# mynameisfiber/baton

Measured on NVIDIA H100. Metric: federated local samples/sec (whole box), ResNet-18 FedAvg, synthetic non-IID 32x32 shards, higher is better.
Workload: dtype bf16

## Files before the change

baton_b200/csrc/bindings.cpp:

```cpp
#include <ATen/cuda/CUDAContext.h>
#include <c10/cuda/CUDAGuard.h>
#include <torch/extension.h>

#include <optional>
#include <vector>

#include "launch.h"

namespace {

inline cudaStream_t cur_stream() { return at::cuda::getCurrentCUDAStream().stream(); }
inline void check(int rc, const char* what) {
  TORCH_CHECK(rc == 0, "baton_b200::", what, " failed with code ", rc,
              rc > 0 ? std::string(" (") + cudaGetErrorString(static_cast<cudaError_t>(rc)) + ")" : std::string());
}
inline const void* cptr(const at::Tensor& t) { return t.data_ptr(); }
inline void* ptr(at::Tensor& t) { return t.data_ptr(); }
template <class T>
inline T* opt_ptr(const std::optional<at::Tensor>& t) {
  return (t.has_value() && t->defined()) ? reinterpret_cast<T*>(t->data_ptr()) : nullptr;
}
#define CHECK_CUDA(x) TORCH_CHECK((x).is_cuda(), #x " must be a CUDA tensor")

inline std::optional<B200SgdEpilogue> sgd_epilogue(const std::optional<at::Tensor>& theta,
                                                   const std::optional<at::Tensor>& theta_bf16,
                                                   const std::optional<at::Tensor>& mom,
                                                   const std::optional<at::Tensor>& hyper, bool nesterov) {
  if (!hyper.has_value() || !hyper->defined()) return std::nullopt;
  TORCH_CHECK(theta.has_value() && theta->scalar_type() == at::kFloat && hyper->scalar_type() == at::kFloat &&
                  (!theta_bf16.has_value() || theta_bf16->scalar_type() == at::kBFloat16) &&
                  (!mom.has_value() || mom->scalar_type() == at::kFloat),
              "sgd epilogue: fp32 theta / momentum / hyper, bf16 shadow");
  return B200SgdEpilogue{theta->data_ptr<float>(), opt_ptr<void>(theta_bf16), opt_ptr<float>(mom),
                         hyper->data_ptr<float>(), nesterov ? 1 : 0};
}

extern "C" {
#define B200_TRACE_TUS(X) X(gemm_wgmma) X(gemm_fp8) X(quant) X(attention) X(im2col_tma) X(gemm_simt) X(fedavg) \
  X(elementwise) X(conv) X(norm) X(loss)
#define B200_DECL(tu) int b200_trace_set_##tu(unsigned long long* p);
B200_TRACE_TUS(B200_DECL)
#undef B200_DECL
}
bool trace_set(const std::optional<at::Tensor>& buf) {
  unsigned long long* p = nullptr;
  if (buf.has_value() && buf->defined()) {
    CHECK_CUDA(*buf);
    TORCH_CHECK(buf->scalar_type() == at::kLong && buf->is_contiguous() && buf->numel() >= 4, "trace buffer: int64 [2+2n]");
    p = reinterpret_cast<unsigned long long*>(buf->data_ptr());
  }
  int rc = 0;
#define B200_SET(tu) rc |= b200_trace_set_##tu(p);
  B200_TRACE_TUS(B200_SET)
#undef B200_SET
  return rc == 0;
}

bool gemm(const at::Tensor& a, const at::Tensor& b, at::Tensor d, const std::optional<at::Tensor>& bias, int64_t M,
          int64_t N, int64_t K, int64_t lda, int64_t ldb, int64_t ldd, bool a_mn, bool b_mn, int64_t act,
          int64_t split_k, bool accumulate, double alpha, const std::optional<at::Tensor>& flags, int64_t flag_epoch,
          int64_t flag_elem_off, int64_t flag_tile_elems, int64_t flag_bias_off, int64_t force_bn, bool simt,
          const std::optional<at::Tensor>& col_stats, const std::optional<at::Tensor>& flag_epoch_word,
          const std::optional<at::Tensor>& sgd_theta, const std::optional<at::Tensor>& sgd_theta_bf16,
          const std::optional<at::Tensor>& sgd_mom, const std::optional<at::Tensor>& sgd_hyper, bool sgd_nesterov) {
  CHECK_CUDA(a); CHECK_CUDA(b); CHECK_CUDA(d);
  TORCH_CHECK(a.scalar_type() == at::kBFloat16 && b.scalar_type() == at::kBFloat16, "gemm operands must be bf16");
  TORCH_CHECK(d.scalar_type() == at::kBFloat16 || d.scalar_type() == at::kFloat, "gemm output must be bf16/fp32");
  const c10::cuda::CUDAGuard guard(a.device());
  const int out_fp32 = d.scalar_type() == at::kFloat;
  const float* bp = opt_ptr<const float>(bias);
  TORCH_CHECK(!col_stats.has_value() || (!simt && col_stats->scalar_type() == at::kFloat && col_stats->numel() >= 2 * N),
              "col_stats needs the tensor-core path and a [2N] fp32 buffer");
  if (simt) {
    TORCH_CHECK(!sgd_hyper.has_value(), "the SIMT GEMM has no optimizer epilogue");
    check(b200_gemm_simt(cptr(a), cptr(b), ptr(d), bp, M, N, K, lda, ldb, ldd, a_mn, b_mn, out_fp32, act, accumulate,
                         static_cast<float>(alpha), cur_stream()),
          "gemm_simt");
    return true;
  }
  const std::optional<B200SgdEpilogue> sgd = sgd_epilogue(sgd_theta, sgd_theta_bf16, sgd_mom, sgd_hyper, sgd_nesterov);
  const int rc = b200_gemm_bf16(cptr(a), cptr(b), ptr(d), bp, M, N, K, lda, ldb, ldd, a_mn, b_mn, out_fp32, act, split_k,
                                accumulate, static_cast<float>(alpha), opt_ptr<const uint32_t>(flags),
                                static_cast<uint32_t>(flag_epoch), flag_elem_off, static_cast<int>(flag_tile_elems),
                                flag_bias_off, static_cast<int>(force_bn), opt_ptr<float>(col_stats),
                                opt_ptr<const uint32_t>(flag_epoch_word), sgd ? &*sgd : nullptr, cur_stream());
  if (rc == B200_SGD_EPILOGUE_DECLINED) return false;
  check(rc, "gemm_bf16");
  return true;
}

void gemm_batched(const at::Tensor& a, const at::Tensor& b, at::Tensor d, int64_t M, int64_t N, int64_t K, int64_t lda,
                  int64_t ldb, int64_t ldd, bool a_mn, bool b_mn, int64_t act, double alpha, int64_t n_outer,
                  int64_t n_inner, int64_t a_outer, int64_t a_inner, int64_t b_outer, int64_t b_inner, int64_t d_outer,
                  int64_t d_inner, bool accumulate) {
  CHECK_CUDA(a); CHECK_CUDA(b); CHECK_CUDA(d);
  TORCH_CHECK(a.scalar_type() == at::kBFloat16 && b.scalar_type() == at::kBFloat16, "gemm operands must be bf16");
  const c10::cuda::CUDAGuard guard(a.device());
  check(b200_gemm_bf16_batched(cptr(a), cptr(b), ptr(d), M, N, K, lda, ldb, ldd, a_mn, b_mn,
                               d.scalar_type() == at::kFloat, act, static_cast<float>(alpha), n_outer, n_inner, a_outer,
                               a_inner, b_outer, b_inner, d_outer, d_inner, accumulate, cur_stream()),
        "gemm_bf16_batched");
}

bool attention_fwd(const at::Tensor& qkv, at::Tensor out, at::Tensor probs, int64_t B, int64_t S, int64_t H, int64_t dh,
                   double scale) {
  CHECK_CUDA(qkv); CHECK_CUDA(out); CHECK_CUDA(probs);
  TORCH_CHECK(qkv.scalar_type() == at::kBFloat16 && out.scalar_type() == at::kBFloat16 &&
              probs.scalar_type() == at::kBFloat16 && qkv.is_contiguous() && out.is_contiguous() && probs.is_contiguous());
  const c10::cuda::CUDAGuard guard(qkv.device());
  const int rc = b200_attention_fwd(cptr(qkv), ptr(out), ptr(probs), static_cast<int>(B), static_cast<int>(S),
                                    static_cast<int>(H), static_cast<int>(dh), static_cast<float>(scale), cur_stream());
  if (rc == -2) return false;
  check(rc, "attention_fwd");
  return true;
}

bool im2col_tma_probe(const at::Tensor& x, at::Tensor col, int64_t kh, int64_t kw, int64_t stride, int64_t pad,
                      int64_t ho, int64_t wo) {
  CHECK_CUDA(x); CHECK_CUDA(col);
  TORCH_CHECK(x.scalar_type() == at::kBFloat16 && col.scalar_type() == at::kBFloat16 && x.dim() == 4 && x.is_contiguous() &&
              col.is_contiguous());
  const c10::cuda::CUDAGuard guard(x.device());
  const int rc = b200_im2col_tma_probe(cptr(x), ptr(col), static_cast<int>(x.size(0)), static_cast<int>(x.size(1)),
                                       static_cast<int>(x.size(2)), static_cast<int>(x.size(3)), static_cast<int>(kh),
                                       static_cast<int>(kw), static_cast<int>(stride), static_cast<int>(pad),
                                       static_cast<int>(ho), static_cast<int>(wo), cur_stream());
  if (rc == -2) return false;
  check(rc, "im2col_tma_probe");
  return true;
}

bool attention_bwd(const at::Tensor& qkv, const at::Tensor& dout, const at::Tensor& probs, at::Tensor dqkv, int64_t B,
                   int64_t S, int64_t H, int64_t dh, double scale) {
  CHECK_CUDA(qkv); CHECK_CUDA(dout); CHECK_CUDA(probs); CHECK_CUDA(dqkv);
  TORCH_CHECK(qkv.scalar_type() == at::kBFloat16 && dout.scalar_type() == at::kBFloat16 &&
              probs.scalar_type() == at::kBFloat16 && dqkv.scalar_type() == at::kBFloat16 && qkv.is_contiguous() &&
              dout.is_contiguous() && probs.is_contiguous() && dqkv.is_contiguous());
  const c10::cuda::CUDAGuard guard(qkv.device());
  const int rc = b200_attention_bwd(cptr(qkv), cptr(dout), cptr(probs), ptr(dqkv), static_cast<int>(B), static_cast<int>(S),
                                    static_cast<int>(H), static_cast<int>(dh), static_cast<float>(scale), cur_stream());
  if (rc == -2) return false;
  check(rc, "attention_bwd");
  return true;
}

bool conv_igemm_fwd(const at::Tensor& x, const at::Tensor& w, at::Tensor y, int64_t kh, int64_t kw, int64_t stride,
                    int64_t pad, int64_t ho, int64_t wo, int64_t cluster_k, int64_t force_bn,
                    const std::optional<at::Tensor>& col_stats) {
  CHECK_CUDA(x); CHECK_CUDA(w); CHECK_CUDA(y);
  TORCH_CHECK(x.scalar_type() == at::kBFloat16 && w.scalar_type() == at::kBFloat16 && y.scalar_type() == at::kBFloat16 &&
              x.dim() == 4 && x.is_contiguous() && w.is_contiguous() && y.is_contiguous());
  const c10::cuda::CUDAGuard guard(x.device());
  const int rc = b200_conv_igemm_fwd(cptr(x), cptr(w), ptr(y), static_cast<int>(x.size(0)), static_cast<int>(x.size(1)),
                                     static_cast<int>(x.size(2)), static_cast<int>(x.size(3)), static_cast<int>(w.size(0)),
                                     static_cast<int>(kh), static_cast<int>(kw), static_cast<int>(stride),
                                     static_cast<int>(pad), static_cast<int>(ho), static_cast<int>(wo),
                                     static_cast<int>(cluster_k), static_cast<int>(force_bn), opt_ptr<float>(col_stats),
                                     cur_stream());
  if (rc == -2) return false;
  check(rc, "conv_igemm_fwd");
  return true;
}
bool conv_igemm_dgrad(const at::Tensor& dy, const at::Tensor& w, at::Tensor dx, int64_t kh, int64_t kw, int64_t pad,
                      int64_t cluster_k, int64_t force_bn) {
  CHECK_CUDA(dy); CHECK_CUDA(w); CHECK_CUDA(dx);
  TORCH_CHECK(dy.scalar_type() == at::kBFloat16 && w.scalar_type() == at::kBFloat16 && dx.scalar_type() == at::kBFloat16 &&
              dy.dim() == 4 && dx.dim() == 4 && dy.is_contiguous() && w.is_contiguous() && dx.is_contiguous());
  const c10::cuda::CUDAGuard guard(dy.device());
  const int rc = b200_conv_igemm_dgrad(cptr(dy), cptr(w), ptr(dx), static_cast<int>(dx.size(0)), static_cast<int>(dx.size(1)),
                                       static_cast<int>(dx.size(2)), static_cast<int>(dx.size(3)), static_cast<int>(dy.size(3)),
                                       static_cast<int>(kh), static_cast<int>(kw), static_cast<int>(pad),
                                       static_cast<int>(dy.size(1)), static_cast<int>(dy.size(2)),
                                       static_cast<int>(cluster_k), static_cast<int>(force_bn), cur_stream());
  if (rc == -2) return false;
  check(rc, "conv_igemm_dgrad");
  return true;
}
bool conv_igemm_wgrad(const at::Tensor& dy, const at::Tensor& x, at::Tensor dw, int64_t cout, int64_t kh, int64_t kw,
                      int64_t stride, int64_t pad, int64_t ho, int64_t wo, int64_t split_k, int64_t force_bn,
                      const std::optional<at::Tensor>& sgd_theta, const std::optional<at::Tensor>& sgd_theta_bf16,
                      const std::optional<at::Tensor>& sgd_mom, const std::optional<at::Tensor>& sgd_hyper,
                      bool sgd_nesterov) {
  CHECK_CUDA(dy); CHECK_CUDA(x); CHECK_CUDA(dw);
  TORCH_CHECK(x.scalar_type() == at::kBFloat16 && dy.scalar_type() == at::kBFloat16 && dw.scalar_type() == at::kFloat &&
              x.dim() == 4 && x.is_contiguous() && dy.is_contiguous());
  const c10::cuda::CUDAGuard guard(x.device());
  const std::optional<B200SgdEpilogue> sgd = sgd_epilogue(sgd_theta, sgd_theta_bf16, sgd_mom, sgd_hyper, sgd_nesterov);
  const int rc = b200_conv_igemm_wgrad(cptr(dy), cptr(x), dw.data_ptr<float>(), static_cast<int>(x.size(0)),
                                       static_cast<int>(x.size(1)), static_cast<int>(x.size(2)), static_cast<int>(x.size(3)),
                                       static_cast<int>(cout), static_cast<int>(kh), static_cast<int>(kw),
                                       static_cast<int>(stride), static_cast<int>(pad), static_cast<int>(ho),
                                       static_cast<int>(wo), static_cast<int>(split_k), static_cast<int>(force_bn),
                                       sgd ? &*sgd : nullptr, cur_stream());
  if (rc == -2 || rc == B200_SGD_EPILOGUE_DECLINED) return false;
  check(rc, "conv_igemm_wgrad");
  return true;
}

void gemm_fp8(const at::Tensor& a, const at::Tensor& b, at::Tensor d, const std::optional<at::Tensor>& bias,
              const std::optional<at::Tensor>& sfa, const std::optional<at::Tensor>& sfb, int64_t M, int64_t N, int64_t K,
              int64_t lda, int64_t ldb, int64_t ldd, int64_t act, int64_t split_k, bool accumulate, double alpha) {
  CHECK_CUDA(a); CHECK_CUDA(b); CHECK_CUDA(d);
  TORCH_CHECK(a.element_size() == 1 && b.element_size() == 1, "gemm_fp8 operands must be 1-byte (e4m3)");
  const c10::cuda::CUDAGuard guard(a.device());
  check(b200_gemm_fp8(cptr(a), cptr(b), ptr(d), opt_ptr<const float>(bias), opt_ptr<const void>(sfa),
                      opt_ptr<const void>(sfb), M, N, K, lda, ldb, ldd, d.scalar_type() == at::kFloat, act, split_k,
                      accumulate, static_cast<float>(alpha), cur_stream()),
        "gemm_fp8");
}
void quant_mx_rows(const at::Tensor& x, at::Tensor q, at::Tensor sf, int64_t R, int64_t C, int64_t ld_in, int64_t Cp) {
  CHECK_CUDA(x);
  const c10::cuda::CUDAGuard guard(x.device());
  check(b200_quant_mx_rows(x.data_ptr(), q.data_ptr(), sf.data_ptr(), R, C, ld_in, Cp, cur_stream()), "quant_mx_rows");
}
void quant_mx_cols(const at::Tensor& x, at::Tensor q, at::Tensor sf, int64_t R, int64_t C, int64_t ld_in, int64_t Rp) {
  CHECK_CUDA(x);
  const c10::cuda::CUDAGuard guard(x.device());
  check(b200_quant_mx_cols(x.data_ptr(), q.data_ptr(), sf.data_ptr(), R, C, ld_in, Rp, cur_stream()), "quant_mx_cols");
}
void dequant_mx(const at::Tensor& q, const at::Tensor& sf, at::Tensor out, int64_t R, int64_t C, int64_t Cp) {
  CHECK_CUDA(q);
  const c10::cuda::CUDAGuard guard(q.device());
  check(b200_dequant_mx(q.data_ptr(), sf.data_ptr(), out.data_ptr<float>(), R, C, Cp, cur_stream()), "dequant_mx");
}

void fused_sgd(at::Tensor w, at::Tensor g, const std::optional<at::Tensor>& mom, const std::optional<at::Tensor>& wb,
               const at::Tensor& hyper, bool zero_grad, bool nesterov, const std::optional<at::Tensor>& wire_slot,
               const std::optional<at::Tensor>& pack_global, const std::optional<at::Tensor>& pack_scale, int64_t n_pack,
               bool wire_fp32) {
  CHECK_CUDA(w);
  TORCH_CHECK(w.scalar_type() == at::kFloat && g.scalar_type() == at::kFloat && hyper.scalar_type() == at::kFloat);
  TORCH_CHECK(w.is_contiguous() && g.is_contiguous() && w.numel() == g.numel());
  const c10::cuda::CUDAGuard guard(w.device());
  check(b200_fused_sgd(w.data_ptr<float>(), g.data_ptr<float>(), opt_ptr<float>(mom), opt_ptr<void>(wb), w.numel(),
                       hyper.data_ptr<float>(), zero_grad, nesterov,
                       reinterpret_cast<const unsigned long long*>(opt_ptr<const int64_t>(wire_slot)),
                       opt_ptr<const float>(pack_global), opt_ptr<const float>(pack_scale), n_pack, wire_fp32, cur_stream()),
        "fused_sgd");
}

void fused_sgd_segments(at::Tensor w, at::Tensor g, const std::optional<at::Tensor>& mom,
                        const std::optional<at::Tensor>& wb, const at::Tensor& segments, const at::Tensor& hyper,
                        bool nesterov) {
  CHECK_CUDA(w); CHECK_CUDA(segments);
  TORCH_CHECK(w.scalar_type() == at::kFloat && g.scalar_type() == at::kFloat && hyper.scalar_type() == at::kFloat);
  TORCH_CHECK(segments.scalar_type() == at::kLong && segments.dim() == 2 && segments.size(1) == 3 &&
              segments.is_contiguous(), "segments: contiguous int64 [n, 3]");
  const c10::cuda::CUDAGuard guard(w.device());
  check(b200_fused_sgd_segments(w.data_ptr<float>(), g.data_ptr<float>(), opt_ptr<float>(mom), opt_ptr<void>(wb),
                                reinterpret_cast<const long long*>(segments.data_ptr<int64_t>()),
                                static_cast<int>(segments.size(0)), hyper.data_ptr<float>(), nesterov, cur_stream()),
        "fused_sgd_segments");
}

void fold_client(at::Tensor acc, at::Tensor theta, const at::Tensor& global_w, const std::optional<at::Tensor>& wb,
                 const std::optional<at::Tensor>& mom, double nk, int64_t mode, bool reset) {
  CHECK_CUDA(acc);
  TORCH_CHECK(acc.scalar_type() == at::kFloat && theta.scalar_type() == at::kFloat && global_w.scalar_type() == at::kFloat);
  TORCH_CHECK(acc.numel() == theta.numel() && theta.numel() == global_w.numel());
  const c10::cuda::CUDAGuard guard(acc.device());
  check(b200_fold_client(acc.data_ptr<float>(), theta.data_ptr<float>(), global_w.data_ptr<float>(), opt_ptr<void>(wb),
                         opt_ptr<float>(mom), mom.has_value() && mom->defined() ? mom->numel() : 0, theta.numel(),
                         static_cast<float>(nk), static_cast<int>(mode), reset, cur_stream()),
        "fold_client");
}

void weighted_sum(at::Tensor dst, const std::vector<at::Tensor>& srcs, const std::vector<double>& weights) {
  CHECK_CUDA(dst);
  TORCH_CHECK(srcs.size() == weights.size() && !srcs.empty() && srcs.size() <= B200_MAX_RANKS);
  TORCH_CHECK(dst.is_contiguous());
  const c10::cuda::CUDAGuard guard(dst.device());
  std::vector<const void*> ps;
  std::vector<float> ws;
  for (size_t i = 0; i < srcs.size(); ++i) {
    TORCH_CHECK(srcs[i].is_cuda() && srcs[i].is_contiguous() && srcs[i].scalar_type() == dst.scalar_type() &&
                srcs[i].numel() == dst.numel());
    ps.push_back(srcs[i].data_ptr());
    ws.push_back(static_cast<float>(weights[i]));
  }
  const int dt = dst.scalar_type() == at::kBFloat16 ? 1 : 0;
  TORCH_CHECK(dt == 1 || dst.scalar_type() == at::kFloat, "weighted_sum supports fp32/bf16");
  check(b200_weighted_sum(dst.data_ptr(), ps.data(), ws.data(), static_cast<int>(ps.size()), dst.numel(), dt,
                          cur_stream()),
        "weighted_sum");
}

void cast(const at::Tensor& src, at::Tensor dst) {
  CHECK_CUDA(src);
  TORCH_CHECK(src.is_contiguous() && dst.is_contiguous() && src.numel() == dst.numel());
  const c10::cuda::CUDAGuard guard(src.device());
  if (src.scalar_type() == at::kFloat && dst.scalar_type() == at::kBFloat16)
    check(b200_cast_f32_bf16(src.data_ptr<float>(), dst.data_ptr(), src.numel(), cur_stream()), "cast");
  else if (src.scalar_type() == at::kBFloat16 && dst.scalar_type() == at::kFloat)
    check(b200_cast_bf16_f32(src.data_ptr(), dst.data_ptr<float>(), src.numel(), cur_stream()), "cast");
  else
    TORCH_CHECK(false, "cast: unsupported dtype pair");
}

void gather_rows(const at::Tensor& src, const at::Tensor& idx, at::Tensor dst) {
  CHECK_CUDA(src);
  TORCH_CHECK(idx.scalar_type() == at::kLong && src.is_contiguous() && dst.is_contiguous());
  const c10::cuda::CUDAGuard guard(src.device());
  const int64_t n = idx.numel();
  if (src.scalar_type() == at::kLong && src.dim() == 1) {
    check(b200_gather_rows_i64(src.data_ptr<int64_t>() ? reinterpret_cast<const long long*>(src.data_ptr<int64_t>()) : nullptr,
                               reinterpret_cast<const long long*>(idx.data_ptr<int64_t>()),
                               reinterpret_cast<long long*>(dst.data_ptr<int64_t>()), n, cur_stream()),
          "gather_i64");
    return;
  }
  const int64_t row_bytes = src.numel() / src.size(0) * src.element_size();
  check(b200_gather_rows(src.data_ptr(), reinterpret_cast<const long long*>(idx.data_ptr<int64_t>()), dst.data_ptr(), n,
                         row_bytes, cur_stream()),
        "gather_rows");
}

void colsum(const at::Tensor& x, at::Tensor out, int64_t rows, int64_t cols, bool accumulate) {
  CHECK_CUDA(x);
  const c10::cuda::CUDAGuard guard(x.device());
  check(b200_colsum(x.data_ptr(), out.data_ptr<float>(), rows, cols, accumulate, cur_stream()), "colsum");
}
void add_bf16(const at::Tensor& a, const at::Tensor& b, at::Tensor o, bool relu) {
  CHECK_CUDA(a);
  const c10::cuda::CUDAGuard guard(a.device());
  check(b200_add_bf16(a.data_ptr(), b.data_ptr(), o.data_ptr(), a.numel(), relu, cur_stream()), "add_bf16");
}
void relu_bwd(const at::Tensor& y, const at::Tensor& dy, at::Tensor dx) {
  CHECK_CUDA(y);
// ... 157 lines not shown
                      opt_ptr<float>(rvar), save_mean.data_ptr<float>(), save_rstd.data_ptr<float>(),
                      opt_ptr<long long>(nbt), rows, C,
                      static_cast<float>(eps), static_cast<float>(momentum), relu, training, cur_stream()),
        "bn_apply");
}
void bn_bwd_reduce(const at::Tensor& x, const at::Tensor& y, const at::Tensor& dy, const at::Tensor& mean,
                   const at::Tensor& rstd, at::Tensor sums, int64_t rows, int64_t C, bool relu) {
  CHECK_CUDA(x);
  const c10::cuda::CUDAGuard guard(x.device());
  check(b200_bn_bwd_reduce(x.data_ptr(), y.data_ptr(), dy.data_ptr(), mean.data_ptr<float>(), rstd.data_ptr<float>(),
                           sums.data_ptr<float>(), rows, C, relu, cur_stream()),
        "bn_bwd_reduce");
}
void bn_bwd_apply(const at::Tensor& x, const at::Tensor& y, const at::Tensor& dy, at::Tensor dx,
                  const std::optional<at::Tensor>& dres, const std::optional<at::Tensor>& gamma, const at::Tensor& mean,
                  const at::Tensor& rstd, at::Tensor sums, const std::optional<at::Tensor>& dgamma,
                  const std::optional<at::Tensor>& dbeta, int64_t rows, int64_t C, bool relu) {
  CHECK_CUDA(x);
  const c10::cuda::CUDAGuard guard(x.device());
  check(b200_bn_bwd_apply(x.data_ptr(), y.data_ptr(), dy.data_ptr(), dx.data_ptr(), opt_ptr<void>(dres),
                          opt_ptr<const float>(gamma), mean.data_ptr<float>(), rstd.data_ptr<float>(),
                          sums.data_ptr<float>(), opt_ptr<float>(dgamma), opt_ptr<float>(dbeta), rows, C, relu,
                          cur_stream()),
        "bn_bwd_apply");
}
bool bn_relu_maxpool(const at::Tensor& z, at::Tensor p, at::Tensor arg, at::Tensor sums,
                     const std::optional<at::Tensor>& gamma, const std::optional<at::Tensor>& beta,
                     const std::optional<at::Tensor>& rmean, const std::optional<at::Tensor>& rvar, at::Tensor save_mean,
                     at::Tensor save_rstd, const std::optional<at::Tensor>& nbt, int64_t N, int64_t H, int64_t W, int64_t C,
                     int64_t k, int64_t stride, int64_t pad, int64_t Ho, int64_t Wo, double eps, double momentum) {
  CHECK_CUDA(z);
  const c10::cuda::CUDAGuard guard(z.device());
  const int rc = b200_bn_relu_maxpool(z.data_ptr(), p.data_ptr(), arg.data_ptr(), sums.data_ptr<float>(),
                                      opt_ptr<const float>(gamma), opt_ptr<const float>(beta), opt_ptr<float>(rmean),
                                      opt_ptr<float>(rvar), save_mean.data_ptr<float>(), save_rstd.data_ptr<float>(),
                                      opt_ptr<long long>(nbt), static_cast<int>(N), static_cast<int>(H), static_cast<int>(W),
                                      static_cast<int>(C), static_cast<int>(k), static_cast<int>(stride),
                                      static_cast<int>(pad), static_cast<int>(Ho), static_cast<int>(Wo),
                                      static_cast<float>(eps), static_cast<float>(momentum), cur_stream());
  if (rc == -2) return false;
  check(rc, "bn_relu_maxpool");
  return true;
}
bool bn_maxpool_bwd(const at::Tensor& z, const at::Tensor& p, const at::Tensor& arg, const at::Tensor& dy_a,
                    const std::optional<at::Tensor>& dy_b, at::Tensor dz, const std::optional<at::Tensor>& gamma,
                    const at::Tensor& mean, const at::Tensor& rstd, at::Tensor sums, const std::optional<at::Tensor>& dgamma,
                    const std::optional<at::Tensor>& dbeta, int64_t N, int64_t H, int64_t W, int64_t C, int64_t k,
                    int64_t stride, int64_t pad, int64_t Ho, int64_t Wo) {
  CHECK_CUDA(z);
  const c10::cuda::CUDAGuard guard(z.device());
  const int rc = b200_bn_maxpool_bwd(z.data_ptr(), p.data_ptr(), arg.data_ptr(), dy_a.data_ptr(), opt_ptr<const void>(dy_b),
                                     dz.data_ptr(), opt_ptr<const float>(gamma), mean.data_ptr<float>(),
                                     rstd.data_ptr<float>(), sums.data_ptr<float>(), opt_ptr<float>(dgamma),
                                     opt_ptr<float>(dbeta), static_cast<int>(N), static_cast<int>(H), static_cast<int>(W),
                                     static_cast<int>(C), static_cast<int>(k), static_cast<int>(stride),
                                     static_cast<int>(pad), static_cast<int>(Ho), static_cast<int>(Wo), cur_stream());
  if (rc == -2) return false;
  check(rc, "bn_maxpool_bwd");
  return true;
}
bool bn_bwd_cluster(const at::Tensor& x, const at::Tensor& y, const at::Tensor& dy_a, const std::optional<at::Tensor>& dy_b,
                    at::Tensor dx, const std::optional<at::Tensor>& dres, const std::optional<at::Tensor>& gamma,
                    const at::Tensor& mean, const at::Tensor& rstd, const std::optional<at::Tensor>& dgamma,
                    const std::optional<at::Tensor>& dbeta, int64_t rows, int64_t C, bool relu, int64_t max_cluster) {
  CHECK_CUDA(x);
  const c10::cuda::CUDAGuard guard(x.device());
  const int rc = b200_bn_bwd_cluster(x.data_ptr(), y.data_ptr(), dy_a.data_ptr(), opt_ptr<const void>(dy_b), dx.data_ptr(),
                                     opt_ptr<void>(dres), opt_ptr<const float>(gamma), mean.data_ptr<float>(),
                                     rstd.data_ptr<float>(), opt_ptr<float>(dgamma), opt_ptr<float>(dbeta), rows, C, relu,
                                     static_cast<int>(max_cluster), cur_stream());
  if (rc == -2) return false;
  check(rc, "bn_bwd_cluster");
  return true;
}
void layernorm_fwd(const at::Tensor& x, const std::optional<at::Tensor>& res, at::Tensor y, const at::Tensor& gamma,
                   const at::Tensor& beta, at::Tensor mean, at::Tensor rstd, int64_t rows, int64_t C, double eps) {
  CHECK_CUDA(x);
  const c10::cuda::CUDAGuard guard(x.device());
  check(b200_layernorm_fwd(x.data_ptr(), opt_ptr<const void>(res), y.data_ptr(), gamma.data_ptr<float>(),
                           beta.data_ptr<float>(), mean.data_ptr<float>(), rstd.data_ptr<float>(), rows, C,
                           static_cast<float>(eps), cur_stream()),
        "layernorm_fwd");
}
void layernorm_bwd(const at::Tensor& x, const at::Tensor& dy, at::Tensor dx, const at::Tensor& gamma,
                   const at::Tensor& mean, const at::Tensor& rstd, at::Tensor dgamma, at::Tensor dbeta, int64_t rows,
                   int64_t C) {
  CHECK_CUDA(x);
  const c10::cuda::CUDAGuard guard(x.device());
  check(b200_layernorm_bwd(x.data_ptr(), dy.data_ptr(), dx.data_ptr(), gamma.data_ptr<float>(), mean.data_ptr<float>(),
                           rstd.data_ptr<float>(), dgamma.data_ptr<float>(), dbeta.data_ptr<float>(), rows, C,
                           cur_stream()),
        "layernorm_bwd");
}
void softmax_fwd(const at::Tensor& x, at::Tensor y, int64_t rows, int64_t C, double scale) {
  CHECK_CUDA(x);
  const c10::cuda::CUDAGuard guard(x.device());
  check(b200_softmax_fwd(x.data_ptr(), y.data_ptr(), rows, C, static_cast<float>(scale), cur_stream()), "softmax_fwd");
}
void softmax_bwd(const at::Tensor& y, const at::Tensor& dy, at::Tensor dx, int64_t rows, int64_t C, double scale) {
  CHECK_CUDA(y);
  const c10::cuda::CUDAGuard guard(y.device());
  check(b200_softmax_bwd(y.data_ptr(), dy.data_ptr(), dx.data_ptr(), rows, C, static_cast<float>(scale), cur_stream()),
        "softmax_bwd");
}

void softmax_xent(const at::Tensor& logits, const at::Tensor& target, const std::optional<at::Tensor>& dlogits,
                  at::Tensor loss_acc, int64_t rows, int64_t C, int64_t ld, double grad_scale) {
  CHECK_CUDA(logits);
  TORCH_CHECK(target.scalar_type() == at::kLong && loss_acc.scalar_type() == at::kFloat && loss_acc.numel() >= 2);
  const c10::cuda::CUDAGuard guard(logits.device());
  const int in32 = logits.scalar_type() == at::kFloat;
  const int out32 = dlogits.has_value() && dlogits->defined() && dlogits->scalar_type() == at::kFloat;
  check(b200_softmax_xent(logits.data_ptr(), in32, reinterpret_cast<const long long*>(target.data_ptr<int64_t>()),
                          opt_ptr<void>(dlogits), out32, loss_acc.data_ptr<float>(), rows, C, ld,
                          static_cast<float>(grad_scale), cur_stream()),
        "softmax_xent");
}
bool linear_xent_head(const at::Tensor& x, const at::Tensor& w, const std::optional<at::Tensor>& bias, const at::Tensor& target,
                      const std::optional<at::Tensor>& dx, at::Tensor dw, const std::optional<at::Tensor>& db,
                      at::Tensor loss_acc, const std::optional<at::Tensor>& logits_out, double grad_scale) {
  CHECK_CUDA(x);
  TORCH_CHECK(x.scalar_type() == at::kBFloat16 && w.scalar_type() == at::kBFloat16 && x.dim() == 2 && w.dim() == 2 &&
              x.is_contiguous() && w.is_contiguous() && x.size(1) == w.size(1));
  TORCH_CHECK(target.scalar_type() == at::kLong && dw.scalar_type() == at::kFloat && dw.is_contiguous() &&
              dw.numel() == w.numel() && loss_acc.scalar_type() == at::kFloat && loss_acc.numel() >= 2);
  const c10::cuda::CUDAGuard guard(x.device());
  const int rc = b200_linear_xent_head(x.data_ptr(), w.data_ptr(), opt_ptr<const float>(bias),
                                       reinterpret_cast<const long long*>(target.data_ptr<int64_t>()), opt_ptr<void>(dx),
                                       dw.data_ptr<float>(), opt_ptr<float>(db), loss_acc.data_ptr<float>(),
                                       opt_ptr<float>(logits_out), static_cast<int>(x.size(0)), static_cast<int>(x.size(1)),
                                       static_cast<int>(w.size(0)), static_cast<float>(grad_scale), cur_stream());
  if (rc == -2) return false;
  check(rc, "linear_xent_head");
  return true;
}
void mse(const at::Tensor& pred, const at::Tensor& target, const std::optional<at::Tensor>& dpred, at::Tensor loss_acc,
         double grad_scale) {
  CHECK_CUDA(pred);
  TORCH_CHECK(target.scalar_type() == at::kFloat && target.numel() == pred.numel());
  const c10::cuda::CUDAGuard guard(pred.device());
  const int in32 = pred.scalar_type() == at::kFloat;
  const int out32 = dpred.has_value() && dpred->defined() && dpred->scalar_type() == at::kFloat;
  check(b200_mse(pred.data_ptr(), in32, target.data_ptr<float>(), opt_ptr<void>(dpred), out32,
                 loss_acc.data_ptr<float>(), pred.numel(), static_cast<float>(grad_scale), cur_stream()),
        "mse");
}

}

PYBIND11_MODULE(TORCH_EXTENSION_NAME, m) {
  m.doc() = "baton_b200 sm_90a kernels";
  m.attr("MAX_RANKS") = B200_MAX_RANKS;
  m.def("gemm", &gemm);
  m.def("trace_set", &trace_set);
  m.def("attention_fwd", &attention_fwd);
  m.def("attention_bwd", &attention_bwd);
  m.def("bn_bwd_cluster", &bn_bwd_cluster);
  m.def("im2col_tma_probe", &im2col_tma_probe);
  m.def("conv_igemm_fwd", &conv_igemm_fwd);
  m.def("conv_igemm_wgrad", &conv_igemm_wgrad);
  m.def("conv_igemm_dgrad", &conv_igemm_dgrad);
  m.def("gemm_batched", &gemm_batched);
  m.def("gemm_fp8", &gemm_fp8);
  m.def("quant_mx_rows", &quant_mx_rows);
  m.def("quant_mx_cols", &quant_mx_cols);
  m.def("dequant_mx", &dequant_mx);
  m.def("fused_sgd", &fused_sgd);
  m.def("fused_sgd_segments", &fused_sgd_segments);
  m.def("weighted_sum", &weighted_sum);
  m.def("fold_client", &fold_client);
  m.def("cast", &cast);
  m.def("gather_rows", &gather_rows);
  m.def("colsum", &colsum);
  m.def("add_bf16", &add_bf16);
  m.def("relu_bwd", &relu_bwd);
  m.def("gelu", &gelu);
  m.def("gelu_bwd", &gelu_bwd);
  m.def("pad_rows", &pad_rows);
  m.def("embedding_bwd", &embedding_bwd);
  m.def("fedavg_allreduce", &fedavg_allreduce);
  m.def("flag_barrier", &flag_barrier);
  m.def("im2col", &im2col);
  m.def("col2im", &col2im);
  m.def("maxpool", &maxpool);
  m.def("maxpool_bwd", &maxpool_bwd);
  m.def("avgpool", &avgpool);
  m.def("avgpool_bwd", &avgpool_bwd);
  m.def("bn_stats", &bn_stats);
  m.def("bn_apply", &bn_apply);
  m.def("bn_bwd_reduce", &bn_bwd_reduce);
  m.def("bn_bwd_apply", &bn_bwd_apply);
  m.def("bn_relu_maxpool", &bn_relu_maxpool);
  m.def("bn_maxpool_bwd", &bn_maxpool_bwd);
  m.def("layernorm_fwd", &layernorm_fwd);
  m.def("layernorm_bwd", &layernorm_bwd);
  m.def("softmax_fwd", &softmax_fwd);
  m.def("softmax_bwd", &softmax_bwd);
  m.def("softmax_xent", &softmax_xent);
  m.def("mse", &mse);
  m.def("linear_xent_head", &linear_xent_head);
}
```

baton_b200/csrc/gemm_wgmma.cu:

```cuda
#define B200_TU_TAG 1
#include "ptx.cuh"
#include "launch.h"
#include "pdl.cuh"
#include "sgd.cuh"

namespace b200 {

constexpr int BM = 128;
constexpr int BK = 64;
constexpr int WG_K = 16;
constexpr int GEMM_THREADS = 384;
constexpr int CONSUMER_WARPS = 8;
constexpr int CONSUMER_THREADS = 32 * CONSUMER_WARPS;
constexpr int MAX_STAGES = 8;

struct GemmParams {
  int M, N, K;
  void* D;
  long long ldd;
  const float* bias;
  int out_fp32;
  int act;
  float* col_stats;
  int a_mn, b_mn;
  int k_tiles_per_split;
  int atomic_out;
  int cluster_k;
  int stages;
  const uint32_t* tile_flags;
  uint32_t flag_epoch;
  long long flag_elem_off;
  int flag_tile_elems;
  long long flag_bias_off;
  long long ldb;
  float alpha;
  int batched, batch_inner;
  int batch_count;
  long long d_outer, d_inner;
  int conv_ho, conv_wo;
  int conv_stride, conv_pad;
  int conv_kw;
  int conv_cin;
  int conv_taps;
  int conv_ncol;
  const uint32_t* flag_epoch_ptr;
  const float* sgd_hyper = nullptr;
  float* sgd_theta = nullptr;
  __nv_bfloat16* sgd_wb = nullptr;
  float* sgd_mom = nullptr;
  int sgd_nesterov = 0;
};

__device__ __forceinline__ void wait_arrival_flags(const uint32_t* flags, long long e0, long long e1, int granule,
                                                   uint32_t need) {
  for (long long t = e0 / granule; t <= e1 / granule; ++t) {
    unsigned long long spins = 0;
    while (static_cast<int32_t>(ld_acquire_sys(flags + t) - need) < 0) {
      if (++spins > (1ull << 26)) break;
    }
  }
}

template <int BN>
struct SmemLayout {
  static constexpr int A_BYTES = BM * BK * 2;
  static constexpr int B_BYTES = BN * BK * 2;
  static constexpr int STAGE_BYTES = A_BYTES + B_BYTES;
  static constexpr int PART_PITCH = BN + 4;
  static constexpr int PART_BYTES = BM * PART_PITCH * 4;
};

__device__ __forceinline__ float apply_act(float v, int act) {
  if (act == 1) return fmaxf(v, 0.f);
  if (act == 2) {
    const float k0 = 0.7978845608028654f, k1 = 0.044715f;
    float t = tanhf(k0 * (v + k1 * v * v * v));
    return 0.5f * v * (1.f + t);
  }
  return v;
}

__device__ __forceinline__ uint32_t cluster_ctarank() {
  uint32_t r;
  asm volatile("mov.u32 %0, %%cluster_ctarank;" : "=r"(r));
  return r;
}
__device__ __forceinline__ void cluster_sync_all() {
  asm volatile("barrier.cluster.arrive.release.aligned;" ::: "memory");
  asm volatile("barrier.cluster.wait.acquire.aligned;" ::: "memory");
}
__device__ __forceinline__ float4 ld_dsmem_f4(uint32_t local_smem_addr, uint32_t cta_rank) {
  uint32_t remote;
  asm volatile("mapa.shared::cluster.u32 %0, %1, %2;" : "=r"(remote) : "r"(local_smem_addr), "r"(cta_rank));
  float4 v;
  asm volatile("ld.shared::cluster.v4.f32 {%0, %1, %2, %3}, [%4];"
               : "=f"(v.x), "=f"(v.y), "=f"(v.z), "=f"(v.w)
               : "r"(remote)
               : "memory");
  return v;
}

#define COLSUM_STEP(OFF, HALF)                                                  \
  {                                                                             \
    const bool upper = (lane & (OFF)) != 0;                                     \
    _Pragma("unroll") for (int i = 0; i < (HALF); ++i) {                        \
      const float keep = upper ? t[i + (HALF)] : t[i];                          \
      const float send = upper ? t[i] : t[i + (HALF)];                          \
      t[i] = keep + __shfl_xor_sync(0xffffffffu, send, (OFF));                  \
    }                                                                           \
  }
__device__ __forceinline__ float warp_colsum32(float (&t)[32]) {
  const uint32_t lane = lane_id();
  COLSUM_STEP(16, 16) COLSUM_STEP(8, 8) COLSUM_STEP(4, 4) COLSUM_STEP(2, 2) COLSUM_STEP(1, 1)
  return t[0];
}
#undef COLSUM_STEP
__device__ __forceinline__ void accumulate_col_stats(const GemmParams& p, int col0, const float (&v)[32]) {
  float s[32], q[32];
#pragma unroll
  for (int j = 0; j < 32; ++j) {
    const float r = __bfloat162float(__float2bfloat16_rn(v[j]));
    s[j] = r;
    q[j] = r * r;
  }
  const float cs = warp_colsum32(s), cq = warp_colsum32(q);
  const int col = col0 + static_cast<int>(lane_id());
  if (col < p.N) {
    atomicAdd(p.col_stats + col, cs);
    atomicAdd(p.col_stats + p.N + col, cq);
  }
}

__device__ __forceinline__ void stage_col_stats(float* sbuf, int BNv, int c, const float (&v)[32]) {
  float s[32], q[32];
#pragma unroll
  for (int j = 0; j < 32; ++j) {
    const float r = __bfloat162float(__float2bfloat16_rn(v[j]));
    s[j] = r;
    q[j] = r * r;
  }
  const float cs = warp_colsum32(s), cq = warp_colsum32(q);
  const int lane = static_cast<int>(lane_id());
  sbuf[c + lane] = cs;
  sbuf[BNv + c + lane] = cq;
}

template <int NV, int ACT, bool BIAS>
__device__ __forceinline__ void transform_chunk_t(const GemmParams& p, int col0, float (&v)[NV]) {
  float b[NV];
  if (BIAS) {
    if (col0 + NV <= p.N && ((reinterpret_cast<uintptr_t>(p.bias + col0) & 15) == 0)) {
#pragma unroll
      for (int j = 0; j < NV; j += 4) {
        const float4 t = __ldg(reinterpret_cast<const float4*>(p.bias + col0 + j));
        b[j] = t.x; b[j + 1] = t.y; b[j + 2] = t.z; b[j + 3] = t.w;
      }
    } else {
#pragma unroll
      for (int j = 0; j < NV; ++j) b[j] = (col0 + j) < p.N ? __ldg(p.bias + col0 + j) : 0.f;
    }
  }
  const float alpha = p.alpha;
#pragma unroll
  for (int j = 0; j < NV; ++j) {
    float x = v[j] * alpha;
    if (BIAS) x += b[j];
    if (ACT == 1) x = fmaxf(x, 0.f);
    if (ACT == 2) {
      const float k0 = 0.7978845608028654f, k1 = 0.044715f;
      x = 0.5f * x * (1.f + tanhf(k0 * (x + k1 * x * x * x)));
    }
    v[j] = x;
  }
}
template <int NV>
__device__ __forceinline__ void transform_chunk(const GemmParams& p, int col0, float (&v)[NV]) {
  if (p.bias == nullptr) {
    if (p.act == 0) transform_chunk_t<NV, 0, false>(p, col0, v);
    else if (p.act == 1) transform_chunk_t<NV, 1, false>(p, col0, v);
    else transform_chunk_t<NV, 2, false>(p, col0, v);
  } else {
    if (p.act == 0) transform_chunk_t<NV, 0, true>(p, col0, v);
    else if (p.act == 1) transform_chunk_t<NV, 1, true>(p, col0, v);
    else transform_chunk_t<NV, 2, true>(p, col0, v);
  }
}

template <int NV>
__device__ __forceinline__ void store_row_chunk(const GemmParams& p, int row, int col0, float (&v)[NV], bool vec_ok,
                                                size_t d_off = 0) {
  transform_chunk<NV>(p, col0, v);
  const bool full = (col0 + NV <= p.N);
  if (p.out_fp32) {
    float* d = reinterpret_cast<float*>(p.D) + d_off + static_cast<size_t>(row) * p.ldd + col0;
    if (p.atomic_out) {
      if (full && vec_ok) {
#pragma unroll
        for (int j = 0; j < NV; j += 4)
          asm volatile("red.global.add.v4.f32 [%0], {%1, %2, %3, %4};" ::"l"(d + j), "f"(v[j]), "f"(v[j + 1]),
                       "f"(v[j + 2]), "f"(v[j + 3])
                       : "memory");
      } else {
        _Pragma("unroll") for (int j = 0; j < NV; ++j) if (col0 + j < p.N) atomicAdd(d + j, v[j]);
      }
    } else if (full && vec_ok) {
#pragma unroll
      for (int j = 0; j < NV; j += 4) *reinterpret_cast<float4*>(d + j) = make_float4(v[j], v[j + 1], v[j + 2], v[j + 3]);
    } else {
      _Pragma("unroll") for (int j = 0; j < NV; ++j) if (col0 + j < p.N) d[j] = v[j];
    }
  } else {
    __nv_bfloat16* d = reinterpret_cast<__nv_bfloat16*>(p.D) + d_off + static_cast<size_t>(row) * p.ldd + col0;
    if (full && vec_ok) {
#pragma unroll
      for (int j = 0; j < NV; j += 8) {
        uint4 o;
        o.x = pack_bf16x2(v[j], v[j + 1]);
        o.y = pack_bf16x2(v[j + 2], v[j + 3]);
        o.z = pack_bf16x2(v[j + 4], v[j + 5]);
        o.w = pack_bf16x2(v[j + 6], v[j + 7]);
        *reinterpret_cast<uint4*>(d + j) = o;
      }
    } else {
      _Pragma("unroll") for (int j = 0; j < NV; ++j) if (col0 + j < p.N) d[j] = __float2bfloat16_rn(v[j]);
    }
  }
}

__device__ __forceinline__ void sgd_epilogue_chunk(const GemmParams& p, size_t e, int col0, const float (&v)[32],
                                                   bool vec) {
  const SgdHyper h = load_sgd_hyper(p.sgd_hyper);
  float* w = p.sgd_theta + e;
  float* m = p.sgd_mom != nullptr ? p.sgd_mom + e : nullptr;
  __nv_bfloat16* wb = p.sgd_wb != nullptr ? p.sgd_wb + e : nullptr;
  const bool nest = p.sgd_nesterov != 0;
  if (vec && col0 + 32 <= p.N) {
#pragma unroll
    for (int j = 0; j < 32; j += 4) {
      float4 mv = m != nullptr ? *reinterpret_cast<const float4*>(m + j) : make_float4(0.f, 0.f, 0.f, 0.f);
      const float4 gv = make_float4(__fadd_rn(0.f, v[j]), __fadd_rn(0.f, v[j + 1]), __fadd_rn(0.f, v[j + 2]),
                                    __fadd_rn(0.f, v[j + 3]));
      const float4 wv = sgd_update4(h, *reinterpret_cast<const float4*>(w + j), gv, mv, m != nullptr, nest);
      *reinterpret_cast<float4*>(w + j) = wv;
      if (m != nullptr) *reinterpret_cast<float4*>(m + j) = mv;
      if (wb != nullptr) *reinterpret_cast<uint2*>(wb + j) = make_uint2(pack_bf16x2(wv.x, wv.y), pack_bf16x2(wv.z, wv.w));
    }
  } else {
#pragma unroll
    for (int j = 0; j < 32; ++j) {
      if (col0 + j < p.N) {
        float mv = m != nullptr ? m[j] : 0.f;
        const float wv = sgd_update(h, w[j], __fadd_rn(0.f, v[j]), mv, m != nullptr, nest);
// ... 279 lines not shown
#pragma unroll
      for (int j = 0; j < 32; ++j) v[j] = __uint_as_float(r[j]);
      if (p.col_stats != nullptr) accumulate_col_stats(p, col0, v);
      if (row >= p.M) continue;
      store_row_chunk<32>(p, row, col0, v, vec_ok, d_off);
    }
    return;
  }
  const int W = 128 / elt;
  uint8_t* srow = stage + lane * EPI_PITCH;
#pragma unroll 1
  for (int c0 = half * W; c0 < BN; c0 += 2 * W) {
    if (n0 + c0 >= p.N) break;
    for (int cc = 0; cc < W; cc += 32) {
      uint32_t r[32];
      acc_ld_row32(arow + c0 + cc, r);
      const int col0 = n0 + c0 + cc;
      float v[32];
#pragma unroll
      for (int j = 0; j < 32; ++j) v[j] = __uint_as_float(r[j]);
      transform_chunk<32>(p, col0, v);
      if (p.col_stats != nullptr) accumulate_col_stats(p, col0, v);
      if (p.out_fp32) {
#pragma unroll
        for (int j = 0; j < 32; j += 4)
          *reinterpret_cast<float4*>(srow + (cc + j) * 4) = make_float4(v[j], v[j + 1], v[j + 2], v[j + 3]);
      } else {
#pragma unroll
        for (int j = 0; j < 32; j += 8)
          *reinterpret_cast<uint4*>(srow + (cc + j) * 2) =
              make_uint4(pack_bf16x2(v[j], v[j + 1]), pack_bf16x2(v[j + 2], v[j + 3]), pack_bf16x2(v[j + 4], v[j + 5]),
                         pack_bf16x2(v[j + 6], v[j + 7]));
      }
    }
    __syncwarp();
    const int per16 = 16 / elt;
#pragma unroll
    for (int it = 0; it < 8; ++it) {
      const int idx = it * 32 + lane;
      const int r = idx >> 3, ch = idx & 7;
      const int grow = m0 + q * 32 + r;
      const int col = n0 + c0 + ch * per16;
      if (grow < p.M && col < p.N) {
        const uint4 val = *reinterpret_cast<const uint4*>(stage + r * EPI_PITCH + ch * 16);
        *reinterpret_cast<uint4*>(reinterpret_cast<uint8_t*>(p.D) +
                                  (d_off + static_cast<size_t>(grow) * p.ldd + col) * elt) = val;
      }
    }
    __syncwarp();
  }
}

template <int BN, int STAGES>
__global__ void __launch_bounds__(GEMM_THREADS, 1)
gemm_bf16_persistent_kernel(const __grid_constant__ CUtensorMap tmA, const __grid_constant__ CUtensorMap tmB,
                            const GemmParams p) {
  using L = SmemLayout<BN>;
  extern __shared__ __align__(1024) uint8_t smem_raw[];
  uint8_t* smem = reinterpret_cast<uint8_t*>((reinterpret_cast<uintptr_t>(smem_raw) + 1023) & ~uintptr_t(1023));
  float* acc_tile = reinterpret_cast<float*>(smem + STAGES * L::STAGE_BYTES);
  uint64_t* full_bar = reinterpret_cast<uint64_t*>(smem + STAGES * L::STAGE_BYTES + L::PART_BYTES);
  uint64_t* empty_bar = full_bar + STAGES;
  uint8_t* epi_stage = reinterpret_cast<uint8_t*>(empty_bar + STAGES);

  griddep_launch_dependents();
  const int warp = threadIdx.x >> 5;
  const int tiles_m = (p.M + BM - 1) / BM;
  const int tiles_n = (p.N + BN - 1) / BN;
  const int tiles_per_z = tiles_m * tiles_n;
  const int num_tiles = tiles_per_z * (p.batched ? p.batch_count : 1);
  const int num_kt = (p.K + BK - 1) / BK;

  if (warp == 0 && elect_one()) {
    tma_prefetch_desc(&tmA);
    tma_prefetch_desc(&tmB);
    for (int s = 0; s < STAGES; ++s) {
      mbar_init(&full_bar[s], 1);
      mbar_init(&empty_bar[s], CONSUMER_WARPS);
    }
    fence_barrier_init();
  }
  __syncthreads();
  griddep_wait();

  if (warp == 0) {
    if (elect_one()) {
      int s = 0;
      uint32_t ph = 0;
      for (int tile = blockIdx.x; tile < num_tiles; tile += gridDim.x) {
        const int z = tile / tiles_per_z, rem = tile - z * tiles_per_z;
        const int m0 = (rem % tiles_m) * BM, n0 = (rem / tiles_m) * BN;
        const int zo = p.batched ? z / p.batch_inner : 0, zi = p.batched ? z % p.batch_inner : 0;
        for (int kt = 0; kt < num_kt; ++kt) {
          mbar_wait(&empty_bar[s], ph ^ 1);
          uint8_t* sa = smem + s * L::STAGE_BYTES;
          uint8_t* sb = sa + L::A_BYTES;
          const int k0 = kt * BK;
          mbar_expect_tx(&full_bar[s], L::STAGE_BYTES);
          if (p.batched) {
            if (!p.a_mn) {
              tma_load_4d(sa, &tmA, &full_bar[s], k0, m0, zi, zo);
            } else {
#pragma unroll
              for (int j = 0; j < BM / 64; ++j) tma_load_4d(sa + j * 8192, &tmA, &full_bar[s], m0 + j * 64, k0, zi, zo);
            }
            if (!p.b_mn) {
              tma_load_4d(sb, &tmB, &full_bar[s], k0, n0, zi, zo);
            } else {
#pragma unroll
              for (int j = 0; j < BN / 64; ++j) tma_load_4d(sb + j * 8192, &tmB, &full_bar[s], n0 + j * 64, k0, zi, zo);
            }
          } else {
            if (!p.a_mn) {
              tma_load_2d(sa, &tmA, &full_bar[s], k0, m0);
            } else {
#pragma unroll
              for (int j = 0; j < BM / 64; ++j) tma_load_2d(sa + j * 8192, &tmA, &full_bar[s], m0 + j * 64, k0);
            }
            if (!p.b_mn) {
              tma_load_2d(sb, &tmB, &full_bar[s], k0, n0);
            } else {
#pragma unroll
              for (int j = 0; j < BN / 64; ++j) tma_load_2d(sb + j * 8192, &tmB, &full_bar[s], n0 + j * 64, k0);
            }
          }
          if (++s == STAGES) { s = 0; ph ^= 1; }
        }
      }
    }
  } else if (warp >= 4) {
    const int ew = warp - 4;
    const size_t elt = p.out_fp32 ? 4 : 2;
    const bool vec_ok = ((reinterpret_cast<uintptr_t>(p.D) & 15) == 0) && ((p.ldd * elt) % 16 == 0);
    int s = 0;
    uint32_t ph = 0;
    float acc[BN / 2];
    for (int tile = blockIdx.x; tile < num_tiles; tile += gridDim.x) {
      const int z = tile / tiles_per_z, rem = tile - z * tiles_per_z;
      const int m0 = (rem % tiles_m) * BM, n0 = (rem / tiles_m) * BN;
      size_t d_off = 0;
      if (p.batched)
        d_off = static_cast<size_t>(z / p.batch_inner) * p.d_outer + static_cast<size_t>(z % p.batch_inner) * p.d_inner;
      consume_ktiles<BN>(acc, smem, STAGES, full_bar, empty_bar, s, ph, num_kt, p.a_mn, p.b_mn, ew >> 2);
      named_bar_sync(1, CONSUMER_THREADS);
      wg_store_acc<BN>(acc, acc_tile, L::PART_PITCH, 64 * (ew >> 2));
      named_bar_sync(1, CONSUMER_THREADS);
      epilogue_tile<BN>(p, acc_tile, ew & 3, ew >> 2, m0, n0, epi_stage + ew * EPI_WARP_BYTES,
                        vec_ok && ((d_off * elt) & 15) == 0, d_off);
    }
  }
}


template <int BN, bool CLUSTER, int CONV = 0>
__global__ void __launch_bounds__(GEMM_THREADS, 1)
gemm_bf16_splitk_kernel(const __grid_constant__ CUtensorMap tmA, const __grid_constant__ CUtensorMap tmB,
                        const GemmParams p) {
  using L = SmemLayout<BN>;
  extern __shared__ __align__(1024) uint8_t smem_raw[];
  uint8_t* smem = reinterpret_cast<uint8_t*>((reinterpret_cast<uintptr_t>(smem_raw) + 1023) & ~uintptr_t(1023));
  const int STAGES = p.stages;
  const int ring_bytes = STAGES * L::STAGE_BYTES;
  const int data_bytes = L::PART_BYTES > ring_bytes ? L::PART_BYTES : ring_bytes;
  uint64_t* full_bar = reinterpret_cast<uint64_t*>(smem + data_bytes);
  uint64_t* empty_bar = full_bar + MAX_STAGES;
  float* cstat = reinterpret_cast<float*>(empty_bar + MAX_STAGES);

  griddep_launch_dependents();
  const int warp = threadIdx.x >> 5;
  const int m0 = blockIdx.y * BM;
  const int n0 = blockIdx.x * BN;
  const int k_tiles_total = (p.K + BK - 1) / BK;
  const int kt_begin = blockIdx.z * p.k_tiles_per_split;
  int kt_end = kt_begin + p.k_tiles_per_split;
  if (kt_end > k_tiles_total) kt_end = k_tiles_total;
  const int num_kt = kt_end - kt_begin;

  if (warp == 0 && elect_one()) {
    tma_prefetch_desc(&tmA);
    tma_prefetch_desc(&tmB);
    for (int s = 0; s < STAGES; ++s) {
      mbar_init(&full_bar[s], 1);
      mbar_init(&empty_bar[s], CONSUMER_WARPS);
    }
    fence_barrier_init();
  }
  __syncthreads();
  griddep_wait();

  if (warp == 0) {
    if (elect_one()) {
      if (p.tile_flags != nullptr) {
        const int rows_here = (p.N - n0) < BN ? (p.N - n0) : BN;
        const uint32_t need = p.flag_epoch_ptr != nullptr ? *reinterpret_cast<const volatile uint32_t*>(p.flag_epoch_ptr)
                                                          : p.flag_epoch;
        wait_arrival_flags(p.tile_flags, p.flag_elem_off + static_cast<long long>(n0) * p.ldb,
                           p.flag_elem_off + static_cast<long long>(n0 + rows_here) * p.ldb - 1, p.flag_tile_elems, need);
        if (p.flag_bias_off >= 0)
          wait_arrival_flags(p.tile_flags, p.flag_bias_off + n0, p.flag_bias_off + n0 + rows_here - 1,
                             p.flag_tile_elems, need);
        fence_proxy_async_all();
      }
      int s = 0;
      uint32_t ph = 0;
      for (int i = 0; i < num_kt; ++i) {
        mbar_wait(&empty_bar[s], ph ^ 1);
        uint8_t* sa = smem + s * L::STAGE_BYTES;
        uint8_t* sb = sa + L::A_BYTES;
        const int k0 = (kt_begin + i) * BK;
        mbar_expect_tx(&full_bar[s], L::STAGE_BYTES);
        if constexpr (CONV == 1 || CONV == 3) {
          const int kt = kt_begin + i;
          const int cblocks = p.conv_cin >> 6;
          const int tap = kt / cblocks, cb = kt - tap * cblocks;
          const int fr = tap / p.conv_kw, fs = tap - fr * p.conv_kw;
          const int q0 = m0 % p.conv_wo, t0 = m0 / p.conv_wo;
          tma_load_im2col_4d(sa, &tmA, &full_bar[s], cb * 64, q0 * p.conv_stride - p.conv_pad,
                             (t0 % p.conv_ho) * p.conv_stride - p.conv_pad, t0 / p.conv_ho, fs, fr);
        } else if (!p.a_mn) {
          tma_load_2d(sa, &tmA, &full_bar[s], k0, m0);
        } else {
#pragma unroll
          for (int j = 0; j < BM / 64; ++j)
            tma_load_2d(sa + j * 8192, &tmA, &full_bar[s], m0 + j * 64, k0);
        }
        if constexpr (CONV == 3) {
          const int kt = kt_begin + i;
          const int cblocks = p.conv_cin >> 6;
          const int tap = kt / cblocks, cb = kt - tap * cblocks;
          const int wcol = (p.conv_taps - 1 - tap) * p.conv_ncol + n0;
#pragma unroll
          for (int j = 0; j < BN / 64; ++j) tma_load_2d(sb + j * 8192, &tmB, &full_bar[s], wcol + j * 64, cb * 64);
        } else if (!p.b_mn) {
          tma_load_2d(sb, &tmB, &full_bar[s], k0, n0);
        } else {
#pragma unroll
          for (int j = 0; j < BN / 64; ++j) tma_load_2d(sb + j * 8192, &tmB, &full_bar[s], n0 + j * 64, k0);
        }
        if (++s == STAGES) { s = 0; ph ^= 1; }
      }
    }
  } else if (warp >= 4) {
    const int ew = warp - 4;
    float acc[BN / 2];
    int s = 0;
    uint32_t ph = 0;
    consume_ktiles<BN>(acc, smem, STAGES, full_bar, empty_bar, s, ph, num_kt, p.a_mn, p.b_mn, ew >> 2);
    named_bar_sync(1, CONSUMER_THREADS);
    float* part = reinterpret_cast<float*>(smem);
    wg_store_acc<BN>(acc, part, L::PART_PITCH, 64 * (ew >> 2));
    if constexpr (!CLUSTER) {
      named_bar_sync(1, CONSUMER_THREADS);
      const int q = ew & 3;
      constexpr int NCHUNK = BN / 32;
      const int c_begin = (ew < 4 ? 0 : (NCHUNK + 1) / 2) * 32, c_end = (ew < 4 ? (NCHUNK + 1) / 2 : NCHUNK) * 32;
      const int lrow = q * 32 + static_cast<int>(lane_id());
      const int row = m0 + lrow;
      const size_t elt = p.out_fp32 ? 4 : 2;
      const bool vec_ok = ((reinterpret_cast<uintptr_t>(p.D) & 15) == 0) && ((p.ldd * elt) % 16 == 0);
#pragma unroll 1
      for (int c = c_begin; c < c_end; c += 32) {
        const int col0 = n0 + c;
        if (row >= p.M || col0 >= p.N) continue;
        uint32_t r[32];
        acc_ld_row32(part + lrow * L::PART_PITCH + c, r);
        float v[32];
#pragma unroll
        for (int j = 0; j < 32; ++j) v[j] = __uint_as_float(r[j]);
        store_row_chunk<32>(p, row, col0, v, vec_ok);
      }
    }
  }

  if constexpr (CLUSTER) {
    const int S = p.cluster_k;
    cluster_sync_all();
    if (warp >= 4 && warp < 8) {
      const uint32_t me = cluster_ctarank();
      const int rows_per = BM / S;
      constexpr int CG = BN / 8;
      const int t = threadIdx.x - 128;
      const size_t elt = p.out_fp32 ? 4 : 2;
      const bool vec_ok = ((reinterpret_cast<uintptr_t>(p.D) & 15) == 0) && ((p.ldd * elt) % 16 == 0);
      const bool want_stats = p.col_stats != nullptr;
      float cs[8] = {0.f, 0.f, 0.f, 0.f, 0.f, 0.f, 0.f, 0.f}, cq[8] = {0.f, 0.f, 0.f, 0.f, 0.f, 0.f, 0.f, 0.f};
      for (int item = t; item < rows_per * CG; item += 128) {
        const int lrow = static_cast<int>(me) * rows_per + item / CG;
        const int c = (item % CG) * 8;
        const uint32_t laddr = smem_u32(smem) + static_cast<uint32_t>((lrow * L::PART_PITCH + c) * 4);
        float v[8] = {0.f, 0.f, 0.f, 0.f, 0.f, 0.f, 0.f, 0.f};
        for (int r = 0; r < S; ++r) {
          const float4 a = ld_dsmem_f4(laddr, r), b = ld_dsmem_f4(laddr + 16, r);
          v[0] += a.x; v[1] += a.y; v[2] += a.z; v[3] += a.w;
          v[4] += b.x; v[5] += b.y; v[6] += b.z; v[7] += b.w;
        }
        const int row = m0 + lrow, col0 = n0 + c;
        if (want_stats) {
#pragma unroll
          for (int j = 0; j < 8; ++j) {
            const float rnd = __bfloat162float(__float2bfloat16_rn(v[j]));
            cs[j] += rnd;
            cq[j] = fmaf(rnd, rnd, cq[j]);
          }
        }
        if (row < p.M && col0 < p.N) store_row_chunk<8>(p, row, col0, v, vec_ok);
      }
      if (want_stats) {
#pragma unroll
        for (int j = 0; j < 8; ++j) {
#pragma unroll
          for (int o = CG; o < 32; o <<= 1) {
            cs[j] += __shfl_xor_sync(0xffffffffu, cs[j], o);
            cq[j] += __shfl_xor_sync(0xffffffffu, cq[j], o);
          }
        }
        const int wq = t >> 5, ln = t & 31;
        if (ln < CG) {
#pragma unroll
          for (int j = 0; j < 8; ++j) {
            cstat[wq * 2 * BN + ln * 8 + j] = cs[j];
            cstat[wq * 2 * BN + BN + ln * 8 + j] = cq[j];
          }
        }
        named_bar_sync(2, 128);
        for (int i = t; i < 2 * BN; i += 128) {
          const int col = i < BN ? i : i - BN;
          if (n0 + col < p.N) {
            const float v = cstat[i] + cstat[2 * BN + i] + cstat[4 * BN + i] + cstat[6 * BN + i];
            atomicAdd(p.col_stats + (i < BN ? 0 : p.N) + n0 + col, v);
          }
        }
      }
    }
    cluster_sync_all();
  }
}


typedef CUresult (*EncodeTiledFn)(CUtensorMap*, CUtensorMapDataType, cuuint32_t, void*, const cuuint64_t*,
                                  const cuuint64_t*, const cuuint32_t*, const cuuint32_t*, CUtensorMapInterleave,
                                  CUtensorMapSwizzle, CUtensorMapL2promotion, CUtensorMapFloatOOBfill);

static EncodeTiledFn get_encode_fn() {
  static thread_local bool ctx_bound = false;
  if (!ctx_bound) {
    cudaFree(nullptr);
    ctx_bound = true;
  }
  static EncodeTiledFn fn = nullptr;
  if (fn == nullptr) {
    void* ptr = nullptr;
    cudaDriverEntryPointQueryResult qres;
    cudaError_t e = cudaGetDriverEntryPoint("cuTensorMapEncodeTiled", &ptr, cudaEnableDefault, &qres);
    if (e != cudaSuccess || qres != cudaDriverEntryPointSuccess || ptr == nullptr) return nullptr;
    fn = reinterpret_cast<EncodeTiledFn>(ptr);
  }
  return fn;
}

static int make_map(CUtensorMap* map, const void* base, long long rows, long long cols, long long ld, int box_cols,
                    int box_rows) {
  EncodeTiledFn fn = get_encode_fn();
  if (fn == nullptr) return -1;
  cuuint64_t gdim[2] = {static_cast<cuuint64_t>(cols), static_cast<cuuint64_t>(rows)};
  cuuint64_t gstr[1] = {static_cast<cuuint64_t>(ld) * 2};
  cuuint32_t box[2] = {static_cast<cuuint32_t>(box_cols), static_cast<cuuint32_t>(box_rows)};
  cuuint32_t estr[2] = {1, 1};
  CUresult r = fn(map, CU_TENSOR_MAP_DATA_TYPE_BFLOAT16, 2, const_cast<void*>(base), gdim, gstr, box, estr,
                  CU_TENSOR_MAP_INTERLEAVE_NONE, CU_TENSOR_MAP_SWIZZLE_128B, CU_TENSOR_MAP_L2_PROMOTION_L2_256B,
                  CU_TENSOR_MAP_FLOAT_OOB_FILL_NONE);
  return r == CUDA_SUCCESS ? 0 : static_cast<int>(r);
}

static int make_map4(CUtensorMap* map, const void* base, long long rows, long long cols, long long ld, long long inner,
                     long long s_inner, long long outer, long long s_outer, int box_cols, int box_rows) {
  EncodeTiledFn fn = get_encode_fn();
  if (fn == nullptr) return -1;
  cuuint64_t gdim[4] = {static_cast<cuuint64_t>(cols), static_cast<cuuint64_t>(rows), static_cast<cuuint64_t>(inner),
                        static_cast<cuuint64_t>(outer)};
  cuuint64_t gstr[3] = {static_cast<cuuint64_t>(ld) * 2, static_cast<cuuint64_t>(s_inner) * 2,
                        static_cast<cuuint64_t>(s_outer) * 2};
  cuuint32_t box[4] = {static_cast<cuuint32_t>(box_cols), static_cast<cuuint32_t>(box_rows), 1, 1};
  cuuint32_t estr[4] = {1, 1, 1, 1};
  CUresult r = fn(map, CU_TENSOR_MAP_DATA_TYPE_BFLOAT16, 4, const_cast<void*>(base), gdim, gstr, box, estr,
                  CU_TENSOR_MAP_INTERLEAVE_NONE, CU_TENSOR_MAP_SWIZZLE_128B, CU_TENSOR_MAP_L2_PROMOTION_L2_256B,
                  CU_TENSOR_MAP_FLOAT_OOB_FILL_NONE);
  return r == CUDA_SUCCESS ? 0 : static_cast<int>(r);
}

static int clamp_bn(int bn) { return bn > 128 ? 128 : bn; }

static void set_sgd_epilogue(GemmParams& p, const B200SgdEpilogue& s) {
  p.sgd_hyper = s.hyper; p.sgd_theta = s.theta; p.sgd_wb = reinterpret_cast<__nv_bfloat16*>(s.theta_bf16);
  p.sgd_mom = s.mom; p.sgd_nesterov = s.nesterov;
}

template <int BN, int STAGES, int CONV = 0, bool SGD = false>
static int launch_fixed(const CUtensorMap& ta, const CUtensorMap& tb, const GemmParams& p, dim3 grid,
                      cudaStream_t stream) {
  constexpr int smem = STAGES * SmemLayout<BN>::STAGE_BYTES + 2 * STAGES * 8 + 8 * BN * 4 + 1024;
  static bool configured = false;
  if (!configured) {
    cudaError_t e = cudaFuncSetAttribute(gemm_bf16_fixed_kernel<BN, STAGES, CONV, SGD>,
                                         cudaFuncAttributeMaxDynamicSharedMemorySize, smem);
    if (e != cudaSuccess) return static_cast<int>(e);
    configured = true;
  }
  cudaError_t le = launch_pdl(gemm_bf16_fixed_kernel<BN, STAGES, CONV, SGD>, grid, GEMM_THREADS, smem, stream, ta, tb, p);
  if (le != cudaSuccess) return static_cast<int>(le);
  return static_cast<int>(cudaGetLastError());
}

template <int BN, int STAGES>
static int launch_persistent(const CUtensorMap& ta, const CUtensorMap& tb, const GemmParams& p, int num_tiles,
                             cudaStream_t stream) {
  constexpr int smem = STAGES * SmemLayout<BN>::STAGE_BYTES + SmemLayout<BN>::PART_BYTES + 2 * STAGES * 8 +
                       CONSUMER_WARPS * EPI_WARP_BYTES + 1024;
  static_assert(smem <= 227 * 1024, "persistent GEMM exceeds the 227 KB of shared memory a block may use");
  static bool configured = false;
  if (!configured) {
    cudaError_t e = cudaFuncSetAttribute(gemm_bf16_persistent_kernel<BN, STAGES>,
                                         cudaFuncAttributeMaxDynamicSharedMemorySize, smem);
    if (e != cudaSuccess) return static_cast<int>(e);
    configured = true;
  }
  const int grid = num_tiles < device_sm_count() ? num_tiles : device_sm_count();
  cudaError_t le = launch_pdl(gemm_bf16_persistent_kernel<BN, STAGES>, dim3(grid), GEMM_THREADS, smem, stream, ta, tb, p);
  if (le != cudaSuccess) return static_cast<int>(le);
  return static_cast<int>(cudaGetLastError());
}

template <int BN, int CONV = 0>
static int launch_cfg(const CUtensorMap& ta, const CUtensorMap& tb, const GemmParams& p, dim3 grid,
                      cudaStream_t stream) {
  using L = SmemLayout<BN>;
  constexpr int max_stages = BN == 128 ? 6 : 8;
  constexpr int max_smem = max_stages * L::STAGE_BYTES + 2 * MAX_STAGES * 8 + 8 * BN * 4 + 1024;
  static bool configured = false;
  if (!configured) {
    const int cap = max_smem > L::PART_BYTES + 4096 ? max_smem : L::PART_BYTES + 4096;
    cudaError_t e = cudaFuncSetAttribute(gemm_bf16_splitk_kernel<BN, false, CONV>,
                                         cudaFuncAttributeMaxDynamicSharedMemorySize, cap);
    if (e == cudaSuccess)
      e = cudaFuncSetAttribute(gemm_bf16_splitk_kernel<BN, true, CONV>, cudaFuncAttributeMaxDynamicSharedMemorySize, cap);
    if (e != cudaSuccess) return static_cast<int>(e);
    configured = true;
  }
  int ring = p.stages * L::STAGE_BYTES;
  if (L::PART_BYTES > ring) ring = L::PART_BYTES;
  int smem = ring + 2 * MAX_STAGES * 8 + 8 * BN * 4 + 1024;
  constexpr int max_ctas = 2;
  const int ctas_here = p.atomic_out ? 1 : max_ctas;
  const int floor_smem = (227 * 1024) / (ctas_here + 1) + 1024;
  if (smem < floor_smem && floor_smem <= max_smem) smem = floor_smem;
  cudaLaunchConfig_t cfg = {};
  cfg.gridDim = grid;
  cfg.blockDim = dim3(GEMM_THREADS);
  cfg.dynamicSmemBytes = smem;
  cfg.stream = stream;
  cudaLaunchAttribute attr[2];
  int na = 0;
  if (pdl_enabled()) {
    attr[na].id = cudaLaunchAttributeProgrammaticStreamSerialization;
    attr[na].val.programmaticStreamSerializationAllowed = 1;
    ++na;
  }
  if (p.cluster_k > 1) {
    attr[na].id = cudaLaunchAttributeClusterDimension;
    attr[na].val.clusterDim.x = 1;
    attr[na].val.clusterDim.y = 1;
    attr[na].val.clusterDim.z = p.cluster_k;
    ++na;
  }
  cfg.attrs = attr;
  cfg.numAttrs = na;
  cudaError_t le = p.cluster_k > 1 ? cudaLaunchKernelEx(&cfg, gemm_bf16_splitk_kernel<BN, true, CONV>, ta, tb, p)
                                   : cudaLaunchKernelEx(&cfg, gemm_bf16_splitk_kernel<BN, false, CONV>, ta, tb, p);
  if (le != cudaSuccess) return static_cast<int>(le);
  return static_cast<int>(cudaGetLastError());
}

}

extern "C" int b200_encode_map2_bf16(void* map, const void* base, long long rows, long long cols, long long ld,
                                     int box_cols, int box_rows) {
  return b200::make_map(reinterpret_cast<CUtensorMap*>(map), base, rows, cols, ld, box_cols, box_rows);
}
extern "C" int b200_encode_map4_bf16(void* map, const void* base, long long rows, long long cols, long long ld,
                                     long long inner, long long s_inner, long long outer, long long s_outer,
                                     int box_cols, int box_rows) {
  return b200::make_map4(reinterpret_cast<CUtensorMap*>(map), base, rows, cols, ld, inner, s_inner, outer, s_outer,
                         box_cols, box_rows);
}

extern "C" int b200_gemm_bf16(const void* a, const void* b, void* d, const float* bias, int M, int N, int K,
                              long long lda, long long ldb, long long ldd, int a_mn, int b_mn, int out_fp32, int act,
                              int split_k, int accumulate, float alpha, const uint32_t* tile_flags,
                              uint32_t flag_epoch, long long flag_elem_off, int flag_tile_elems,
                              long long flag_bias_off, int force_bn, float* col_stats, const uint32_t* flag_epoch_ptr,
                              const B200SgdEpilogue* sgd, cudaStream_t stream) {
  using namespace b200;
  if (M <= 0 || N <= 0 || K <= 0) return 0;
  if (sgd != nullptr && (!accumulate || !out_fp32 || !a_mn || !b_mn || bias != nullptr || act != 0 || alpha != 1.0f ||
                         col_stats != nullptr || tile_flags != nullptr))
    return B200_SGD_EPILOGUE_DECLINED;
  if (col_stats != nullptr && (split_k > 1 || bias != nullptr || act != 0 || alpha != 1.0f || accumulate)) return -3;
  if ((lda % 8) || (ldb % 8) || (reinterpret_cast<uintptr_t>(a) & 15) || (reinterpret_cast<uintptr_t>(b) & 15))
    return -2;
  const int bn = clamp_bn(force_bn > 0 ? force_bn : (N > 64 ? 128 : 64));
  if (tile_flags != nullptr && (b_mn || flag_tile_elems <= 0)) return -4;
  CUtensorMap ta, tb;
  int rc;
  if (!a_mn)
    rc = make_map(&ta, a, M, K, lda, BK, BM);
  else
    rc = make_map(&ta, a, K, M, lda, 64, BK);
  if (rc) return rc;
  if (!b_mn)
    rc = make_map(&tb, b, N, K, ldb, BK, bn);
  else
    rc = make_map(&tb, b, K, N, ldb, 64, BK);
  if (rc) return rc;

  const int k_tiles = (K + BK - 1) / BK;
  int cluster_k = 1;
  if (split_k < 0) {
    cluster_k = -split_k;
    if (cluster_k != 2 && cluster_k != 4 && cluster_k != 8) return -5;
    while (cluster_k > 1 && (cluster_k - 1) * ((k_tiles + cluster_k - 1) / cluster_k) >= k_tiles) cluster_k >>= 1;
    split_k = cluster_k;
  }
  if (split_k < 1) split_k = 1;
  if (split_k > k_tiles) split_k = k_tiles;
  int per = (k_tiles + split_k - 1) / split_k;
  if (cluster_k == 1) split_k = (k_tiles + per - 1) / per;
  GemmParams p;
  p.M = M; p.N = N; p.K = K; p.D = d; p.ldd = ldd; p.bias = bias; p.out_fp32 = out_fp32; p.act = act;
  p.a_mn = a_mn; p.b_mn = b_mn; p.k_tiles_per_split = per;
  p.cluster_k = cluster_k;
  p.atomic_out = (accumulate || (split_k > 1 && cluster_k == 1)) ? 1 : 0;
  p.col_stats = col_stats;
  p.tile_flags = tile_flags; p.flag_epoch = flag_epoch; p.alpha = alpha;
  p.flag_elem_off = flag_elem_off; p.flag_tile_elems = flag_tile_elems; p.ldb = ldb;
  p.flag_bias_off = (tile_flags != nullptr && bias != nullptr) ? flag_bias_off : -1;
  p.flag_epoch_ptr = tile_flags != nullptr ? flag_epoch_ptr : nullptr;
  p.batched = 0; p.batch_inner = 1; p.batch_count = 1; p.d_outer = 0; p.d_inner = 0;
  if (p.atomic_out && (!out_fp32 || bias != nullptr || act != 0)) return -3;
  const int max_stages = bn == 128 ? 6 : 8;
  p.stages = per < max_stages ? (per < 2 ? 2 : per) : max_stages;
  dim3 grid((N + bn - 1) / bn, (M + BM - 1) / BM, split_k);
  const int num_tiles = static_cast<int>(grid.x * grid.y);
  const bool persistent = split_k == 1 && tile_flags == nullptr && num_tiles >= device_sm_count() && bn == 128;
  if (sgd != nullptr) {
    if (split_k != 1 || cluster_k != 1 || persistent) return B200_SGD_EPILOGUE_DECLINED;
    set_sgd_epilogue(p, *sgd);
  }
  if (cluster_k > 1) {
    if (bn == 128) return launch_cfg<128>(ta, tb, p, grid, stream);
    return launch_cfg<64>(ta, tb, p, grid, stream);
  }
  if (persistent) return launch_persistent<128, 3>(ta, tb, p, num_tiles, stream);
  const bool shallow = per <= 4 && !p.batched;
  if (sgd != nullptr) {
    if (bn == 128)
      return shallow ? launch_fixed<128, 3, 0, true>(ta, tb, p, grid, stream) : launch_fixed<128, 6, 0, true>(ta, tb, p, grid, stream);
    return shallow ? launch_fixed<64, 4, 0, true>(ta, tb, p, grid, stream) : launch_fixed<64, 8, 0, true>(ta, tb, p, grid, stream);
  }
  if (bn == 128) return shallow ? launch_fixed<128, 3>(ta, tb, p, grid, stream) : launch_fixed<128, 6>(ta, tb, p, grid, stream);
  return shallow ? launch_fixed<64, 4>(ta, tb, p, grid, stream) : launch_fixed<64, 8>(ta, tb, p, grid, stream);
}

extern "C" int b200_gemm_bf16_batched(const void* a, const void* b, void* d, int M, int N, int K, long long lda,
                                      long long ldb, long long ldd, int a_mn, int b_mn, int out_fp32, int act,
                                      float alpha, int n_outer, int n_inner, long long a_outer, long long a_inner,
                                      long long b_outer, long long b_inner, long long d_outer, long long d_inner,
                                      int accumulate, cudaStream_t stream) {
  using namespace b200;
  if (M <= 0 || N <= 0 || K <= 0 || n_outer <= 0 || n_inner <= 0) return 0;
  if ((lda % 8) || (ldb % 8) || (a_outer % 8) || (a_inner % 8) || (b_outer % 8) || (b_inner % 8) ||
      (reinterpret_cast<uintptr_t>(a) & 15) || (reinterpret_cast<uintptr_t>(b) & 15))
    return -2;
  auto fix = [](long long s) { return s > 0 ? s : 8; };
  const int bn = N > 64 ? 128 : 64;
  CUtensorMap ta, tb;
  int rc;
  if (!a_mn)
    rc = make_map4(&ta, a, M, K, lda, n_inner, fix(a_inner), n_outer, fix(a_outer), BK, BM);
  else
    rc = make_map4(&ta, a, K, M, lda, n_inner, fix(a_inner), n_outer, fix(a_outer), 64, BK);
  if (rc) return rc;
  if (!b_mn)
    rc = make_map4(&tb, b, N, K, ldb, n_inner, fix(b_inner), n_outer, fix(b_outer), BK, bn);
  else
    rc = make_map4(&tb, b, K, N, ldb, n_inner, fix(b_inner), n_outer, fix(b_outer), 64, BK);
  if (rc) return rc;
  GemmParams p;
  p.M = M; p.N = N; p.K = K; p.D = d; p.ldd = ldd; p.bias = nullptr; p.out_fp32 = out_fp32; p.act = act;
  p.a_mn = a_mn; p.b_mn = b_mn; p.k_tiles_per_split = (K + BK - 1) / BK; p.cluster_k = 1;
  p.atomic_out = accumulate ? 1 : 0;
  p.col_stats = nullptr;
  p.tile_flags = nullptr; p.flag_epoch = 0; p.alpha = alpha; p.flag_elem_off = 0; p.flag_tile_elems = 0;
  p.ldb = ldb; p.flag_bias_off = -1; p.flag_epoch_ptr = nullptr; p.stages = 4;
  p.batched = 1; p.batch_inner = n_inner; p.d_outer = d_outer; p.d_inner = d_inner;
  if (p.atomic_out && !out_fp32) return -3;
  dim3 grid((N + bn - 1) / bn, (M + BM - 1) / BM, n_outer * n_inner);
  p.batch_count = n_outer * n_inner;
  const long long total_tiles = static_cast<long long>(grid.x) * grid.y * grid.z;
  if (total_tiles >= 2 * device_sm_count() && total_tiles < (1ll << 30)) {
    const int nt = static_cast<int>(total_tiles);
    if (bn == 128) return launch_persistent<128, 3>(ta, tb, p, nt, stream);
    return launch_persistent<64, 5>(ta, tb, p, nt, stream);
  }
  if (bn == 128) return launch_fixed<128, 6>(ta, tb, p, grid, stream);
  return launch_fixed<64, 8>(ta, tb, p, grid, stream);
}

extern "C" int b200_encode_map_im2col_bf16(void* map, const void* x, int N, int H, int W, int C, int KH, int KW,
                                            int stride, int pad, int channels, int pixels);

extern "C" int b200_conv_igemm_fwd(const void* x, const void* w, void* y, int N, int H, int W, int Cin, int Cout, int KH,
                                   int KW, int stride, int pad, int Ho, int Wo, int cluster_k, int force_bn,
                                   float* col_stats, cudaStream_t stream) {
  using namespace b200;
  const long long M = static_cast<long long>(N) * Ho * Wo;
  const int K = KH * KW * Cin;
  if (M <= 0 || Cout <= 0) return 0;
  if (Cin % 64 != 0 || Cout % 8 != 0 || M > (1ll << 30) || (reinterpret_cast<uintptr_t>(x) & 15) ||
      (reinterpret_cast<uintptr_t>(w) & 15) || (reinterpret_cast<uintptr_t>(y) & 15))
    return -2;
  const int bn = clamp_bn(force_bn > 0 ? force_bn : (Cout > 64 ? 128 : 64));
  CUtensorMap ta, tb;
  int rc = b200_encode_map_im2col_bf16(&ta, x, N, H, W, Cin, KH, KW, stride, pad, 64, BM);
  if (rc) return rc;
  rc = make_map(&tb, w, Cout, K, K, BK, bn);
  if (rc) return rc;
  const int k_tiles = K / BK;
  if (cluster_k != 1 && cluster_k != 2 && cluster_k != 4 && cluster_k != 8) return -5;
  while (cluster_k > 1 && (cluster_k - 1) * ((k_tiles + cluster_k - 1) / cluster_k) >= k_tiles) cluster_k >>= 1;
  const int per = (k_tiles + cluster_k - 1) / cluster_k;
  GemmParams p;
  p.M = static_cast<int>(M); p.N = Cout; p.K = K; p.D = y; p.ldd = Cout; p.bias = nullptr; p.out_fp32 = 0; p.act = 0;
  p.a_mn = 0; p.b_mn = 0; p.k_tiles_per_split = per; p.cluster_k = cluster_k; p.atomic_out = 0;
  p.col_stats = col_stats;
  p.tile_flags = nullptr; p.flag_epoch = 0; p.alpha = 1.0f; p.flag_elem_off = 0; p.flag_tile_elems = 0; p.ldb = K;
  p.flag_bias_off = -1; p.flag_epoch_ptr = nullptr;
  p.batched = 0; p.batch_inner = 1; p.batch_count = 1; p.d_outer = 0; p.d_inner = 0;
  const int max_stages = bn == 128 ? 6 : 8;
  p.stages = per < max_stages ? (per < 2 ? 2 : per) : max_stages;
  p.conv_ho = Ho; p.conv_wo = Wo; p.conv_stride = stride; p.conv_pad = pad; p.conv_kw = KW; p.conv_cin = Cin;
  p.conv_taps = KH * KW; p.conv_ncol = Cin;
  dim3 grid((Cout + bn - 1) / bn, static_cast<unsigned>((M + BM - 1) / BM), cluster_k);
  if (cluster_k > 1) {
    if (bn == 128) return launch_cfg<128, 1>(ta, tb, p, grid, stream);
    return launch_cfg<64, 1>(ta, tb, p, grid, stream);
  }
  const bool shallow = per <= 4;
  if (bn == 128) return shallow ? launch_fixed<128, 3, 1>(ta, tb, p, grid, stream) : launch_fixed<128, 6, 1>(ta, tb, p, grid, stream);
  return shallow ? launch_fixed<64, 4, 1>(ta, tb, p, grid, stream) : launch_fixed<64, 8, 1>(ta, tb, p, grid, stream);
}

extern "C" int b200_conv_igemm_dgrad(const void* dy, const void* w, void* dx, int N, int H, int W, int Cin, int Cout,
                                     int KH, int KW, int pad, int Ho, int Wo, int cluster_k, int force_bn,
                                     cudaStream_t stream) {
  using namespace b200;
  const long long M = static_cast<long long>(N) * H * W;
  const int K = KH * KW * Cout;
  if (M <= 0 || Cin <= 0) return 0;
  const int padp = KH - 1 - pad, padq = KW - 1 - pad;
  if (Cout % 64 != 0 || Cin % 64 != 0 || M > (1ll << 30) || padp < 0 || padq < 0 || padp != padq ||
      Ho + 2 * padp - (KH - 1) != H || Wo + 2 * padq - (KW - 1) != W || (reinterpret_cast<uintptr_t>(dy) & 15) ||
      (reinterpret_cast<uintptr_t>(w) & 15) || (reinterpret_cast<uintptr_t>(dx) & 15))
    return -2;
  const int bn = clamp_bn(force_bn > 0 ? force_bn : (Cin > 64 ? 128 : 64));
  CUtensorMap ta, tb;
  int rc = b200_encode_map_im2col_bf16(&ta, dy, N, Ho, Wo, Cout, KH, KW, 1, padp, 64, BM);
  if (rc) return rc;
  rc = make_map(&tb, w, Cout, static_cast<long long>(KH) * KW * Cin, static_cast<long long>(KH) * KW * Cin, 64, BK);
  if (rc) return rc;
  const int k_tiles = K / BK;
  if (cluster_k != 1 && cluster_k != 2 && cluster_k != 4 && cluster_k != 8) return -5;
  while (cluster_k > 1 && (cluster_k - 1) * ((k_tiles + cluster_k - 1) / cluster_k) >= k_tiles) cluster_k >>= 1;
  const int per = (k_tiles + cluster_k - 1) / cluster_k;
  GemmParams p;
  p.M = static_cast<int>(M); p.N = Cin; p.K = K; p.D = dx; p.ldd = Cin; p.bias = nullptr; p.out_fp32 = 0; p.act = 0;
  p.a_mn = 0; p.b_mn = 1; p.k_tiles_per_split = per; p.cluster_k = cluster_k; p.atomic_out = 0;
  p.col_stats = nullptr;
  p.tile_flags = nullptr; p.flag_epoch = 0; p.alpha = 1.0f; p.flag_elem_off = 0; p.flag_tile_elems = 0;
  p.ldb = static_cast<long long>(KH) * KW * Cin;
  p.flag_bias_off = -1; p.flag_epoch_ptr = nullptr;
  p.batched = 0; p.batch_inner = 1; p.batch_count = 1; p.d_outer = 0; p.d_inner = 0;
  const int max_stages = bn == 128 ? 6 : 8;
  p.stages = per < max_stages ? (per < 2 ? 2 : per) : max_stages;
  p.conv_ho = H; p.conv_wo = W; p.conv_stride = 1; p.conv_pad = padp; p.conv_kw = KW; p.conv_cin = Cout;
  p.conv_taps = KH * KW; p.conv_ncol = Cin;
  dim3 grid((Cin + bn - 1) / bn, static_cast<unsigned>((M + BM - 1) / BM), cluster_k);
  if (cluster_k > 1) {
    if (bn == 128) return launch_cfg<128, 3>(ta, tb, p, grid, stream);
    return launch_cfg<64, 3>(ta, tb, p, grid, stream);
  }
  if (bn == 128) return launch_fixed<128, 6, 3>(ta, tb, p, grid, stream);
  return launch_fixed<64, 8, 3>(ta, tb, p, grid, stream);
}

extern "C" int b200_conv_igemm_wgrad(const void* dy, const void* x, float* dw, int N, int H, int W, int Cin, int Cout,
                                     int KH, int KW, int stride, int pad, int Ho, int Wo, int split_k, int force_bn,
                                     const B200SgdEpilogue* sgd, cudaStream_t stream) {
  using namespace b200;
  const long long Mp = static_cast<long long>(N) * Ho * Wo;
  const int Kc = KH * KW * Cin;
  if (Mp <= 0 || Cout <= 0) return 0;
  if (Cin % 64 != 0 || Cout % 8 != 0 || Mp > (1ll << 30) || (reinterpret_cast<uintptr_t>(x) & 15) ||
      (reinterpret_cast<uintptr_t>(dy) & 15) || (reinterpret_cast<uintptr_t>(dw) & 15))
    return -2;
  const int bn = clamp_bn(force_bn > 0 ? force_bn : (Kc > 64 ? 128 : 64));
  CUtensorMap ta, tb;
  int rc = make_map(&ta, dy, Mp, Cout, Cout, 64, BK);
  if (rc) return rc;
  rc = b200_encode_map_im2col_bf16(&tb, x, N, H, W, Cin, KH, KW, stride, pad, 64, 64);
  if (rc) return rc;
  const int k_tiles = static_cast<int>((Mp + BK - 1) / BK);
  if (split_k < 1) split_k = 1;
  if (split_k > k_tiles) split_k = k_tiles;
  const int per = (k_tiles + split_k - 1) / split_k;
  split_k = (k_tiles + per - 1) / per;
  if (sgd != nullptr && split_k != 1) return B200_SGD_EPILOGUE_DECLINED;
  GemmParams p;
  if (sgd != nullptr) set_sgd_epilogue(p, *sgd);
  p.M = Cout; p.N = Kc; p.K = static_cast<int>(Mp); p.D = dw; p.ldd = Kc; p.bias = nullptr; p.out_fp32 = 1; p.act = 0;
  p.a_mn = 1; p.b_mn = 1; p.k_tiles_per_split = per; p.cluster_k = 1; p.atomic_out = 1;
  p.col_stats = nullptr;
  p.tile_flags = nullptr; p.flag_epoch = 0; p.alpha = 1.0f; p.flag_elem_off = 0; p.flag_tile_elems = 0; p.ldb = Kc;
  p.flag_bias_off = -1; p.flag_epoch_ptr = nullptr;
  p.batched = 0; p.batch_inner = 1; p.batch_count = 1; p.d_outer = 0; p.d_inner = 0;
  p.stages = 4;
  p.conv_ho = Ho; p.conv_wo = Wo; p.conv_stride = stride; p.conv_pad = pad; p.conv_kw = KW; p.conv_cin = Cin;
  p.conv_taps = KH * KW; p.conv_ncol = Cin;
  dim3 grid((Kc + bn - 1) / bn, (Cout + BM - 1) / BM, split_k);
  if (sgd != nullptr) {
    if (bn == 128) return launch_fixed<128, 6, 2, true>(ta, tb, p, grid, stream);
    return launch_fixed<64, 8, 2, true>(ta, tb, p, grid, stream);
  }
  if (bn == 128) return launch_fixed<128, 6, 2>(ta, tb, p, grid, stream);
  return launch_fixed<64, 8, 2>(ta, tb, p, grid, stream);
}

B200_TRACE_REGISTER(gemm_wgmma)
```

baton_b200/csrc/launch.h:

```cpp
#pragma once
#include <cuda_runtime.h>
#include <stdint.h>

#define B200_MAX_RANKS 16

extern "C" {

struct B200SgdEpilogue {
  float* theta;
  void* theta_bf16;
  float* mom;
  const float* hyper;
  int nesterov;
};
#define B200_SGD_EPILOGUE_DECLINED (-6)

int b200_gemm_bf16(const void* a, const void* b, void* d, const float* bias, int M, int N, int K, long long lda,
                   long long ldb, long long ldd, int a_mn, int b_mn, int out_fp32, int act, int split_k, int accumulate,
                   float alpha, const uint32_t* tile_flags, uint32_t flag_epoch, long long flag_elem_off, int flag_tile_elems,
                   long long flag_bias_off, int force_bn, float* col_stats, const uint32_t* flag_epoch_ptr,
                   const B200SgdEpilogue* sgd, cudaStream_t stream);
int b200_gemm_bf16_batched(const void* a, const void* b, void* d, int M, int N, int K, long long lda, long long ldb,
                           long long ldd, int a_mn, int b_mn, int out_fp32, int act, float alpha, int n_outer,
                           int n_inner, long long a_outer, long long a_inner, long long b_outer, long long b_inner,
                           long long d_outer, long long d_inner, int accumulate, cudaStream_t stream);
int b200_attention_fwd(const void* qkv, void* out, void* probs, int B, int S, int H, int dh, float scale,
                       cudaStream_t stream);
int b200_attention_bwd(const void* qkv, const void* dout, const void* probs, void* dqkv, int B, int S, int H, int dh,
                       float scale, cudaStream_t stream);
int b200_conv_igemm_fwd(const void* x, const void* w, void* y, int N, int H, int W, int Cin, int Cout, int KH, int KW,
                        int stride, int pad, int Ho, int Wo, int cluster_k, int force_bn, float* col_stats,
                        cudaStream_t stream);
int b200_conv_igemm_dgrad(const void* dy, const void* w, void* dx, int N, int H, int W, int Cin, int Cout, int KH, int KW,
                          int pad, int Ho, int Wo, int cluster_k, int force_bn, cudaStream_t stream);
int b200_conv_igemm_wgrad(const void* dy, const void* x, float* dw, int N, int H, int W, int Cin, int Cout, int KH, int KW,
                          int stride, int pad, int Ho, int Wo, int split_k, int force_bn, const B200SgdEpilogue* sgd,
                          cudaStream_t stream);
int b200_im2col_tma_probe(const void* x, void* col, int N, int H, int W, int C, int KH, int KW, int stride, int pad,
                          int Ho, int Wo, cudaStream_t stream);
int b200_gemm_fp8(const void* a, const void* b, void* d, const float* bias, const void* sfa, const void* sfb, int M, int N,
                  int K, long long lda, long long ldb, long long ldd, int out_fp32, int act, int split_k, int accumulate,
                  float alpha, cudaStream_t stream);
int b200_quant_mx_rows(const void* x, void* q, void* sf, long long R, int C, long long ld_in, int Cp, cudaStream_t stream);
int b200_quant_mx_cols(const void* x, void* q, void* sf, long long R, int C, long long ld_in, long long Rp,
                       cudaStream_t stream);
int b200_dequant_mx(const void* q, const void* sf, float* out, long long R, int C, int Cp, cudaStream_t stream);
int b200_gemm_simt(const void* a, const void* b, void* d, const float* bias, int M, int N, int K, long long lda,
                   long long ldb, long long ldd, int a_mn, int b_mn, int out_fp32, int act, int accumulate,
                   float alpha, cudaStream_t stream);

int b200_fused_sgd(float* w, float* g, float* mom, void* w_bf16, long long n, const float* hyper, int zero_grad,
                   int nesterov, const unsigned long long* wire_slot, const float* pack_global,
                   const float* pack_scale, long long n_pack, int wire_fp32, cudaStream_t stream);
int b200_fused_sgd_segments(float* w, float* g, float* mom, void* w_bf16, const long long* segments, int n_seg,
                            const float* hyper, int nesterov, cudaStream_t stream);
int b200_fold_client(float* acc, float* theta, const float* global_w, void* w_bf16, float* mom, long long n_mom, long long n,
                     float nk, int mode, int reset, cudaStream_t stream);
int b200_weighted_sum(void* dst, const void* const* srcs, const float* weights, int n_src, long long n, int dtype,
                      cudaStream_t stream);
int b200_cast_f32_bf16(const float* src, void* dst, long long n, cudaStream_t stream);
int b200_cast_bf16_f32(const void* src, float* dst, long long n, cudaStream_t stream);
int b200_gather_rows(const void* src, const long long* idx, void* dst, long long n_rows, long long row_bytes,
                     cudaStream_t stream);
int b200_gather_rows_i64(const long long* src, const long long* idx, long long* dst, long long n,
                         cudaStream_t stream);
int b200_colsum(const void* x, float* out, long long rows, int cols, int accumulate, cudaStream_t stream);
int b200_add_bf16(const void* a, const void* b, void* out, long long n, int relu, cudaStream_t stream);
int b200_relu_bwd_bf16(const void* y, const void* dy, void* dx, long long n, cudaStream_t stream);
int b200_gelu_bf16(const void* x, void* y, long long n, cudaStream_t stream);
int b200_gelu_bwd_bf16(const void* x, const void* dy, void* dx, long long n, cudaStream_t stream);
int b200_embedding_bwd(const void* dy, const long long* idx, float* grad, long long n_rows, int width,
                       cudaStream_t stream);
int b200_pad_rows_bf16(const void* src, void* dst, long long rows, int k, int kp, const uint32_t* flags,
                       const uint32_t* epoch_word, long long elem_off, int granule, cudaStream_t stream);

struct FedAvgArgs {
  void* wire[B200_MAX_RANKS];
  unsigned long long* pads[B200_MAX_RANKS];
  void* wire_mc;
  float* theta;
  float* global_w;
  void* theta_bf16;
  float* momentum;
  long long n_momentum;
  long long* int_local;
  long long* int_wire[B200_MAX_RANKS];
  float* loss_local;
  float* loss_wire[B200_MAX_RANKS];
  float* loss_out;
  int n_loss;
  float n_samples[B200_MAX_RANKS];
  int counts_from_flags;
  float nvls_prescale;
  uint32_t alive_mask;
  int rank, world;
  long long n;
  int n_int;
  int wire_kind;
  int delta;
  int use_nvls;
  uint32_t epoch;
  uint32_t* tile_flags;
  uint32_t flag_value;
  int tile_elems;
  int prepacked;
  int timeout_log2;
  int* status;
  unsigned long long* phase_ns;
};
int b200_fedavg_allreduce(const FedAvgArgs* args, int n_ctas, cudaStream_t stream);
int b200_flag_barrier(unsigned long long* const* pads, int rank, int world, uint32_t alive_mask, uint32_t epoch,
                      int slot, cudaStream_t stream);

int b200_im2col_nhwc(const void* x, void* col, int N, int H, int W, int C, int KH, int KW, int stride, int pad,
                     int Ho, int Wo, int kp, cudaStream_t stream);
int b200_col2im_nhwc(const void* col, void* dx, int N, int H, int W, int C, int KH, int KW, int stride, int pad,
                     int Ho, int Wo, int kp, cudaStream_t stream);
int b200_maxpool_nhwc(const void* x, void* y, int* argmax, int N, int H, int W, int C, int k, int stride, int pad,
                      int Ho, int Wo, int arg_u8, cudaStream_t stream);
int b200_maxpool_bwd_nhwc(const void* dy, const void* dy_b, const int* argmax, void* dx, int N, int H, int W, int C, int Ho,
                          int Wo, int k, int stride, int pad, int arg_u8, cudaStream_t stream);
int b200_avgpool_nhwc(const void* x, void* y, int N, int HW, int C, cudaStream_t stream);
int b200_avgpool_bwd_nhwc(const void* dy, void* dx, int N, int HW, int C, cudaStream_t stream);

int b200_bn_stats(const void* x, float* sums, long long rows, int C, cudaStream_t stream);
int b200_bn_apply(const void* x, const void* residual, void* y, float* sums, const float* gamma, const float* beta,
                  float* running_mean, float* running_var, float* save_mean, float* save_rstd, long long* nbt,
                  long long rows, int C, float eps, float momentum, int relu, int training, cudaStream_t stream);
int b200_bn_bwd_reduce(const void* x, const void* y, const void* dy, const float* save_mean, const float* save_rstd,
                       float* sums, long long rows, int C, int relu, cudaStream_t stream);
int b200_bn_bwd_apply(const void* x, const void* y, const void* dy, void* dx, void* dres, const float* gamma,
                      const float* save_mean, const float* save_rstd, float* sums, float* dgamma, float* dbeta,
                      long long rows, int C, int relu, cudaStream_t stream);
int b200_bn_relu_maxpool(const void* z, void* p, void* argmax, const float* sums, const float* gamma, const float* beta,
                         float* running_mean, float* running_var, float* save_mean, float* save_rstd, long long* nbt, int N,
                         int H, int W, int C, int k, int stride, int pad, int Ho, int Wo, float eps, float momentum,
                         cudaStream_t stream);
int b200_bn_maxpool_bwd(const void* z, const void* p, const void* argmax, const void* dy_a, const void* dy_b, void* dz,
                        const float* gamma, const float* save_mean, const float* save_rstd, float* sums, float* dgamma,
                        float* dbeta, int N, int H, int W, int C, int k, int stride, int pad, int Ho, int Wo,
                        cudaStream_t stream);
int b200_bn_bwd_cluster(const void* x, const void* y, const void* dy_a, const void* dy_b, void* dx, void* dres,
                        const float* gamma, const float* save_mean, const float* save_rstd, float* dgamma, float* dbeta,
                        long long rows, int C, int relu, int max_cluster, cudaStream_t stream);
int b200_layernorm_fwd(const void* x, const void* residual, void* y, const float* gamma, const float* beta,
                       float* mean, float* rstd, long long rows, int C, float eps, cudaStream_t stream);
int b200_layernorm_bwd(const void* x, const void* dy, void* dx, const float* gamma, const float* mean,
                       const float* rstd, float* dgamma, float* dbeta, long long rows, int C, cudaStream_t stream);
int b200_softmax_fwd(const void* x, void* y, long long rows, int C, float scale, cudaStream_t stream);
int b200_softmax_bwd(const void* y, const void* dy, void* dx, long long rows, int C, float scale,
                     cudaStream_t stream);

int b200_softmax_xent(const void* logits, int logits_fp32, const long long* target, void* dlogits, int dl_fp32,
                      float* loss_acc, long long rows, int C, long long ld, float grad_scale, cudaStream_t stream);
int b200_linear_xent_head(const void* x, const void* w, const float* bias, const long long* target, void* dx, float* dw,
                          float* db, float* loss_acc, float* logits_out, int rows, int K, int NC, float grad_scale,
                          cudaStream_t stream);
int b200_mse(const void* pred, int pred_fp32, const float* target, void* dpred, int dp_fp32, float* loss_acc,
             long long n, float grad_scale, cudaStream_t stream);
}
```

baton_b200/models/resnet.py:

```python
from __future__ import annotations

from typing import List, Optional, Sequence, Type

import torch
from torch import nn

from ..ops import nn as bnn
from .base import FederatedModule


def _conv_bn_fwd(conv: "bnn.Conv2d", bn: "bnn.BatchNorm2d", x, residual=None, after_conv=None):
    cc, cb = bnn.Ctx(), bnn.Ctx()
    stats = conv._fusable_stats(x)
    z = bnn._ConvFn.forward(cc, x, conv.weight, conv._w_bf16(), conv.kernel_size, conv.kernel_size, conv.stride,
                            conv.padding, None, stats, conv.flags_cfg)
    if after_conv is not None:
        after_conv()
    y = bnn._BNFn.forward(cb, z, residual, bn.weight, bn.bias, bn.running_mean, bn.running_var, bn.num_batches_tracked,
                          bn.eps, bn.momentum, bn.relu, True, bn.workspace, None, stats is not None)
    return y, (cc, cb)


def _conv_bn_bwd(ctxs, dy_a, dy_b=None, needs_dx=True):
    cc, cb = ctxs
    cc.needs_dx = needs_dx
    out = bnn._BNFn.backward(cb, dy_a, dy_b)
    dz, dres = out[0], out[1]
    dx = bnn._ConvFn.backward(cc, dz)[0]
    return dx, dres




def _stem_fwd(conv, bn, pool, x, after_conv=None):
    stats = conv._fusable_stats(x)
    if (stats is None or bn.workspace is None or not bn.relu or not bn.training or bn.num_features % 8
            or bnn._grad_target(bn.weight) is None or bnn._grad_target(bn.bias) is None):
        return None
    cc = bnn.Ctx()
    z = bnn._ConvFn.forward(cc, x, conv.weight, conv._w_bf16(), conv.kernel_size, conv.kernel_size, conv.stride,
                            conv.padding, None, stats, conv.flags_cfg)
    if after_conv is not None:
        after_conv()
    c = bn.num_features
    out = bnn.F.bn_relu_maxpool(z, bn.workspace[: 2 * c], bnn._unwrap(bn.weight), bnn._unwrap(bn.bias), bn.running_mean,
                                bn.running_var, bn.num_batches_tracked, bn.eps, bn.momentum, pool.k, pool.stride, pool.pad)
    if out is None:
        raise RuntimeError("bn_relu_maxpool rejected a shape _stem_fwd accepted")
    p, arg, mean, rstd = out
    return p, cc, z, arg, mean, rstd


def _stem_bwd(saved, bn, pool, dy_a, dy_b=None):
    p, cc, z, arg, mean, rstd = saved
    c = bn.num_features
    gamma = bnn._unwrap(bn.weight)
    tg, tb = bnn._grad_target(gamma), bnn._grad_target(bnn._unwrap(bn.bias))
    dz = bnn.F.bn_maxpool_bwd(z, p, arg, dy_a.contiguous(), dy_b.contiguous() if dy_b is not None else None, gamma, mean,
                              rstd, bn.workspace[2 * c:], tg, tb, pool.k, pool.stride, pool.pad)
    if dz is None:
        raise RuntimeError("bn_maxpool_bwd rejected a shape bn_relu_maxpool accepted")
    cc.needs_dx = False
    bnn._ConvFn.backward(cc, dz)


class BasicBlock(nn.Module):
    expansion = 1

    def __init__(self, inplanes: int, planes: int, stride: int = 1, downsample: Optional[nn.Module] = None):
        super().__init__()
        self.conv1 = bnn.Conv2d(inplanes, planes, 3, stride, 1)
        self.bn1 = bnn.BatchNorm2d(planes, relu=True)
        self.conv2 = bnn.Conv2d(planes, planes, 3, 1, 1)
        self.bn2 = bnn.BatchNorm2d(planes, relu=True)
        self.downsample = downsample

    def forward(self, x):
        identity = x if self.downsample is None else self.downsample(x)
        out = self.bn1(self.conv1(x))
        return self.bn2(self.conv2(out), identity)

    units = (("conv1", "bn1"), ("conv2", "bn2"))


class Bottleneck(nn.Module):
    expansion = 4

    def __init__(self, inplanes: int, planes: int, stride: int = 1, downsample: Optional[nn.Module] = None):
        super().__init__()
        self.conv1 = bnn.Conv2d(inplanes, planes, 1, 1, 0)
        self.bn1 = bnn.BatchNorm2d(planes, relu=True)
        self.conv2 = bnn.Conv2d(planes, planes, 3, stride, 1)
        self.bn2 = bnn.BatchNorm2d(planes, relu=True)
        self.conv3 = bnn.Conv2d(planes, planes * 4, 1, 1, 0)
        self.bn3 = bnn.BatchNorm2d(planes * 4, relu=True)
        self.downsample = downsample

    def forward(self, x):
        identity = x if self.downsample is None else self.downsample(x)
        out = self.bn1(self.conv1(x))
        out = self.bn2(self.conv2(out))
        return self.bn3(self.conv3(out), identity)

    units = (("conv1", "bn1"), ("conv2", "bn2"), ("conv3", "bn3"))


class _Downsample(nn.Sequential):

    def __init__(self, inplanes: int, outplanes: int, stride: int):
        super().__init__(bnn.Conv2d(inplanes, outplanes, 1, stride, 0), bnn.BatchNorm2d(outplanes, relu=False))


class ResNet(FederatedModule):
    loss_kind = "ce"
    default_lr = 0.05
    default_batch_size = 128

    def __init__(self, block: Type[nn.Module], layers: Sequence[int], num_classes: int = 1000,
                 in_channels: int = 3, name: Optional[str] = None):
        super().__init__()
        if name:
            self.name = name
        self.inplanes = 64
        self.conv1 = bnn.Conv2d(in_channels, 64, 7, 2, 3)
        self.bn1 = bnn.BatchNorm2d(64, relu=True)
        self.maxpool = bnn.MaxPool2d(3, 2, 1)
        self.layer1 = self._make_layer(block, 64, layers[0], 1)
        self.layer2 = self._make_layer(block, 128, layers[1], 2)
        self.layer3 = self._make_layer(block, 256, layers[2], 2)
        self.layer4 = self._make_layer(block, 512, layers[3], 2)
        self.avgpool = bnn.GlobalAvgPool()
        self.fc = bnn.Linear(512 * block.expansion, num_classes, out_fp32=True)
        self.stats_workspace = None
        self.zeroes_own_workspace = True
        for m in self.modules():
            if isinstance(m, BasicBlock):
                nn.init.zeros_(m.bn2.weight)
            elif isinstance(m, Bottleneck):
                nn.init.zeros_(m.bn3.weight)

    def _make_layer(self, block, planes: int, blocks: int, stride: int) -> nn.Sequential:
        downsample = None
        if stride != 1 or self.inplanes != planes * block.expansion:
            downsample = _Downsample(self.inplanes, planes * block.expansion, stride)
        layers: List[nn.Module] = [block(self.inplanes, planes, stride, downsample)]
        self.inplanes = planes * block.expansion
        for _ in range(1, blocks):
            layers.append(block(self.inplanes, planes))
        return nn.Sequential(*layers)

    def set_precision(self, dtype: str = "bf16") -> "ResNet":
        assert dtype in ("bf16", "fp8")
        for m in self.modules():
            if isinstance(m, bnn.Conv2d):
                m.fp8 = dtype == "fp8"
        self.compute_dtype = dtype
        return self

    def forward(self, x):
        if self.stats_workspace is not None and self.training:
            self.stats_workspace.zero_()
        x = self.maxpool(self.bn1(self.conv1(x)))
        x = self.layer4(self.layer3(self.layer2(self.layer1(x))))
        return self.fc(self.avgpool(x))

    def _block_fwd(self, blk, x, tape):
        ds_ctx = None
        identity = x
        if blk.downsample is not None:
            with bnn.BRANCH.fork(x):
                identity, ds_ctx = _conv_bn_fwd(blk.downsample[0], blk.downsample[1], x)
        out = x
        ctxs = []
        n = len(blk.units)
        for i, (cn, bnn_) in enumerate(blk.units):
            last = i == n - 1
            if last:
                bnn.BRANCH.join()
            out, c = _conv_bn_fwd(getattr(blk, cn), getattr(blk, bnn_), out, identity if last else None)
            ctxs.append(c)
        tape.append((ctxs, ds_ctx))
        return out

    def _block_bwd(self, entry, pieces):
        ctxs, ds_ctx = entry
        d, dres = _conv_bn_bwd(ctxs[-1], pieces[0], pieces[1] if len(pieces) > 1 else None)
        dx_ds = None
        if ds_ctx is not None:
            with bnn.BRANCH.fork(dres):
                dx_ds, _ = _conv_bn_bwd(ds_ctx, dres)
        for c in reversed(ctxs[:-1]):
            d, _ = _conv_bn_bwd(c, d)
        if ds_ctx is not None:
            bnn.BRANCH.join()
            return [d, dx_ds]
        return [d, dres]

    def explicit_step(self, x, target, loss_acc=None, after_first_gemm=None):
        F = bnn.F
        if self.stats_workspace is not None:
            self.stats_workspace.zero_()
        stem = cp = None
        fused_stem = _stem_fwd(self.conv1, self.bn1, self.maxpool, x, after_first_gemm)
        if fused_stem is not None:
            h = fused_stem[0]
        else:
            h, stem = _conv_bn_fwd(self.conv1, self.bn1, x, after_conv=after_first_gemm)
            cp = bnn.Ctx()
            h = bnn._MaxPoolFn.forward(cp, h, self.maxpool.k, self.maxpool.stride, self.maxpool.pad)
        tape = []
        for layer in (self.layer1, self.layer2, self.layer3, self.layer4):
            for blk in layer:
                h = self._block_fwd(blk, h, tape)
        ca = None
        if h.shape[1] == 1 and h.shape[2] == 1:
            feat = h.reshape(h.shape[0], h.shape[3])
        else:
            ca = bnn.Ctx()
            feat = bnn._AvgPoolFn.forward(ca, h)
        fc = self.fc
        head = None
        tw, tb = bnn._grad_target(fc.weight), bnn._grad_target(fc.bias)
        if fc.out_features <= 32 and tw is not None and (fc.bias is None or tb is not None) and fc.act == 0:
            head = F.linear_xent_head(feat.contiguous(), bnn._shadow(fc, "weight", fc.weight), fc.bias, target, tw, tb,
                                      acc=loss_acc)
        if head is not None:
            stats, d, _ = head
        else:
            cl = bnn.Ctx()
            logits = bnn._LinearFn.forward(cl, feat, fc.weight, fc.bias, bnn._shadow(fc, "weight", fc.weight), fc.act,
                                           fc.out_fp32, None, None)
            cl.needs_dx = True
            stats, dlogits = F.softmax_xent(logits.contiguous(), target, want_grad=True, acc=loss_acc)
            d = bnn._LinearFn.backward(cl, dlogits)[0]
        d = d.reshape(h.shape) if ca is None else bnn._AvgPoolFn.backward(ca, d)
        pieces = [d]
        for bi in range(len(tape) - 1, -1, -1):
            pieces = self._block_bwd(tape[bi], pieces)
        if fused_stem is not None:
            _stem_bwd(fused_stem, self.bn1, self.maxpool, pieces[0], pieces[1] if len(pieces) > 1 else None)
        else:
            d = bnn._MaxPoolFn.backward(cp, pieces[0], pieces[1] if len(pieces) > 1 else None)[0]
            _conv_bn_bwd(stem, d, needs_dx=False)
        bnn.WGRAD.join()
        return stats

    def build_workspace(self, device) -> torch.Tensor:
        bns = [m for m in self.modules() if isinstance(m, bnn.BatchNorm2d)]
        total = sum(4 * m.num_features for m in bns)
        ws = torch.zeros(total, dtype=torch.float32, device=device)
        off = 0
        for m in bns:
            m.workspace = ws[off: off + 4 * m.num_features]
            off += 4 * m.num_features
        self.stats_workspace = ws
        for parent in self.modules():
            for conv_name, bn_name in (("conv1", "bn1"), ("conv2", "bn2"), ("conv3", "bn3")):
                conv, bn = getattr(parent, conv_name, None), getattr(parent, bn_name, None)
                if isinstance(conv, bnn.Conv2d) and isinstance(bn, bnn.BatchNorm2d):
                    conv.bn_ws = bn.workspace
            if isinstance(parent, _Downsample):
                parent[0].bn_ws = parent[1].workspace
        return ws


def resnet18(num_classes: int = 10, **kw) -> ResNet:
    kw.setdefault("name", "resnet18")
    return ResNet(BasicBlock, [2, 2, 2, 2], num_classes=num_classes, **kw)


def resnet50(num_classes: int = 1000, **kw) -> ResNet:
    kw.setdefault("name", "resnet50")
    return ResNet(Bottleneck, [3, 4, 6, 3], num_classes=num_classes, **kw)
```

baton_b200/ops/functional.py:

```python
from __future__ import annotations

from typing import List, Optional, Sequence, Tuple

import torch

from ._ext import load

BF16 = torch.bfloat16
NUM_SMS = 132


def _pitch(t: torch.Tensor) -> int:
    assert t.dim() == 2 and (t.stride(1) == 1 or t.shape[1] == 1), "GEMM operand must have unit inner stride"
    return t.stride(0) if t.shape[0] > 1 else max(t.stride(0), t.shape[1])


def _tma_ok(t: torch.Tensor) -> bool:
    return t.dtype == BF16 and _pitch(t) % 8 == 0 and t.data_ptr() % 16 == 0


def pick_bn(M: int, N: int) -> int:
    m_tiles = (M + 127) // 128
    if N >= 128 and m_tiles * ((N + 127) // 128) >= NUM_SMS:
        return 128
    if N > 128 and m_tiles * ((N + 127) // 128) >= NUM_SMS // 2:
        return 128
    return 64


_WGRAD_MAX_CTAS = 64
_CLUSTER_MIN_KT = 4


def pick_split_k(M: int, N: int, K: int, bn: int) -> int:
    tiles = ((M + 127) // 128) * ((N + bn - 1) // bn)
    k_tiles = (K + 63) // 64
    if tiles >= NUM_SMS // 2 or k_tiles < 8:
        return 1
    return max(1, min(k_tiles // 4, max(1, _WGRAD_MAX_CTAS // tiles)))


def pick_cluster_k(M: int, N: int, K: int, bn: int) -> int:
    tiles = ((M + 127) // 128) * ((N + bn - 1) // bn)
    k_tiles = (K + 63) // 64
    if k_tiles < 16:
        return 1
    best = 1
    for s in (2, 4, 8):
        cap = NUM_SMS // 2 if s == 8 else 128
        if tiles * s <= cap and k_tiles >= _CLUSTER_MIN_KT * s:
            best = s
    return best


def gemm(a: torch.Tensor, b: torch.Tensor, *, a_mn: bool = False, b_mn: bool = False,
         out: Optional[torch.Tensor] = None, out_dtype: torch.dtype = BF16, bias: Optional[torch.Tensor] = None,
         act: int = 0, accumulate: bool = False, alpha: float = 1.0, split_k: Optional[int] = None,
         n_valid: Optional[int] = None, flags: Optional[torch.Tensor] = None, flag_epoch: int = 0,
         flag_elem_off: int = 0, flag_tile_elems: int = 0, flag_bias_off: int = -1, force_bn: int = 0,
         force_simt: bool = False, col_stats: Optional[torch.Tensor] = None,
         flag_epoch_word: Optional[torch.Tensor] = None, sgd: Optional[dict] = None) -> Optional[torch.Tensor]:
    C = load()
    M, K = (a.shape[1], a.shape[0]) if a_mn else (a.shape[0], a.shape[1])
    N, Kb = (b.shape[1], b.shape[0]) if b_mn else (b.shape[0], b.shape[1])
    assert K == Kb, "GEMM reduction dims differ: {} vs {}".format(K, Kb)
    if n_valid is not None:
        N = min(N, n_valid)
    if out is None:
        out = torch.empty((M, N), dtype=out_dtype, device=a.device)
        if accumulate:
            out.zero_()
    ldd = out.stride(0) if out.dim() == 2 else N
    lda, ldb = _pitch(a), _pitch(b)
    use_simt = force_simt or not (_tma_ok(a) and _tma_ok(b))
    if use_simt and sgd is not None:
        return None
    if use_simt:
        assert col_stats is None, "fused column statistics need the tensor-core path"
        C.gemm(a, b, out, bias, M, N, K, lda, ldb, ldd, a_mn, b_mn, act, 1, accumulate, alpha, None, 0, 0, 0, -1, 0,
               True, None, None, None, None, None, None, False)
        return out
    bn = force_bn or pick_bn(M, N)
    if col_stats is not None:
        assert not accumulate and bias is None and act == 0 and alpha == 1.0
    if split_k is None:
        if accumulate and out.dtype == torch.float32:
            split_k = pick_split_k(M, N, K, bn)
        else:
            split_k = -pick_cluster_k(M, N, K, bn)
            if split_k == -1:
                split_k = 1
    if split_k > 1:
        assert out.dtype == torch.float32 and bias is None and act == 0
    if sgd is not None and split_k != 1:
        return None
    sg = sgd or {}
    if not C.gemm(a, b, out, bias, M, N, K, lda, ldb, ldd, a_mn, b_mn, act, split_k, accumulate, alpha, flags, flag_epoch,
                  flag_elem_off, flag_tile_elems, flag_bias_off, bn, False, col_stats, flag_epoch_word, sg.get("theta"),
                  sg.get("theta_bf16"), sg.get("momentum"), sg.get("hyper"), bool(sg.get("nesterov", False))):
        return None
    return out


def gemm_stats_fusable(M: int, N: int, K: int) -> bool:
    return K % 8 == 0


def fused_sgd(w: torch.Tensor, g: torch.Tensor, hyper: torch.Tensor, momentum_buf: Optional[torch.Tensor] = None,
              w_bf16: Optional[torch.Tensor] = None, zero_grad: bool = True, nesterov: bool = False,
              pack: Optional[dict] = None) -> None:
    pk = pack or {}
    load().fused_sgd(w, g, momentum_buf, w_bf16, hyper, zero_grad, nesterov, pk.get("wire_slot"),
                     pk.get("global_w"), pk.get("scale"), int(pk.get("n_pack", 0)), bool(pk.get("wire_fp32", False)))


def sgd_epilogue_args(theta: torch.Tensor, grad: torch.Tensor, grad_view: torch.Tensor, hyper: torch.Tensor,
                      momentum: Optional[torch.Tensor] = None, theta_bf16: Optional[torch.Tensor] = None,
                      nesterov: bool = False) -> dict:
    off = (grad_view.data_ptr() - grad.data_ptr()) // grad.element_size()
    assert 0 <= off < grad.numel(), "the GEMM output is not a view of the gradient arena"
    return {"theta": theta[off:], "theta_bf16": theta_bf16[off:] if theta_bf16 is not None else None,
            "momentum": momentum[off:] if momentum is not None else None, "hyper": hyper, "nesterov": nesterov}


SGD_CHUNK = 8192


def sgd_segments(n: int, fused: Sequence[Tuple[int, int, int, int]], nograd: Sequence[Tuple[int, int]],
                 chunk: int = SGD_CHUNK) -> List[Tuple[int, int, int]]:
    pieces = sorted((o + r * ld, o + r * ld + cols) for o, rows, cols, ld in fused for r in range(rows))
    free, pos = [], 0
    for s, e in pieces:
        if s < pos or e > n:
            raise ValueError("fused blocks overlap or leave the arena: [{}, {})".format(s, e))
        if s > pos:
            free.append((pos, s))
        pos = e
    if pos < n:
        free.append((pos, n))
    ng = sorted((o, o + l) for o, l in nograd)
    out = []
    for s, e in free:
        cuts = sorted({s, e} | {b for r in ng for b in r if s < b < e})
        for a, b in zip(cuts, cuts[1:]):
            kind = 1 if any(lo <= a and b <= hi for lo, hi in ng) else 0
            out.extend((c, min(chunk, b - c), kind) for c in range(a, b, chunk))
    return out


def fused_sgd_segments(w: torch.Tensor, g: torch.Tensor, hyper: torch.Tensor, segments: torch.Tensor,
                       momentum_buf: Optional[torch.Tensor] = None, w_bf16: Optional[torch.Tensor] = None,
                       nesterov: bool = False) -> None:
    load().fused_sgd_segments(w, g, momentum_buf, w_bf16, segments, hyper, nesterov)


def weighted_sum_(dst: torch.Tensor, srcs: Sequence[torch.Tensor], weights: Sequence[float]) -> torch.Tensor:
    C = load()
    flat_dst = dst.view(-1) if dst.is_contiguous() else None
    if flat_dst is None or dst.dtype not in (torch.float32, BF16) or len(srcs) > C.MAX_RANKS:
        acc = torch.zeros_like(dst, dtype=torch.float32)
        for s, w in zip(srcs, weights):
            acc.add_(s.to(device=dst.device, dtype=torch.float32), alpha=float(w))
        dst.copy_(acc.to(dst.dtype))
        return dst
    ss = [s.to(device=dst.device, dtype=dst.dtype).contiguous().view(-1) for s in srcs]
    C.weighted_sum(flat_dst, ss, [float(w) for w in weights])
    return dst


def fold_client(acc: torch.Tensor, theta: torch.Tensor, global_w: torch.Tensor, nk: float, *, first: bool = False,
                reset: bool = False, w_bf16: Optional[torch.Tensor] = None, momentum: Optional[torch.Tensor] = None) -> None:
    load().fold_client(acc, theta, global_w, w_bf16, momentum, float(nk), 1 if first else 0, reset)


def fold_finish(acc: torch.Tensor, theta: torch.Tensor, global_w: torch.Tensor, total: float) -> None:
    load().fold_client(acc, theta, global_w, None, None, 1.0 / float(total), 2, False)


def cast(src: torch.Tensor, dtype: torch.dtype, out: Optional[torch.Tensor] = None) -> torch.Tensor:
    if out is None:
        out = torch.empty(src.shape, dtype=dtype, device=src.device)
    load().cast(src.contiguous(), out)
    return out


def gather_rows(src: torch.Tensor, idx: torch.Tensor, out: Optional[torch.Tensor] = None) -> torch.Tensor:
    if out is None:
        out = torch.empty((idx.numel(),) + tuple(src.shape[1:]), dtype=src.dtype, device=src.device)
    load().gather_rows(src, idx, out)
    return out


def colsum_(x2d: torch.Tensor, out: torch.Tensor, accumulate: bool = True) -> torch.Tensor:
    load().colsum(x2d, out, x2d.shape[0], x2d.shape[1], accumulate)
    return out


def add(a: torch.Tensor, b: torch.Tensor, relu: bool = False) -> torch.Tensor:
    out = torch.empty_like(a)
    load().add_bf16(a, b, out, relu)
    return out


def relu_bwd(y: torch.Tensor, dy: torch.Tensor) -> torch.Tensor:
    dx = torch.empty_like(dy)
    load().relu_bwd(y, dy, dx)
    return dx


def gelu(x: torch.Tensor) -> torch.Tensor:
    y = torch.empty_like(x)
    load().gelu(x, y)
    return y


def gelu_bwd(x: torch.Tensor, dy: torch.Tensor) -> torch.Tensor:
    dx = torch.empty_like(x)
    load().gelu_bwd(x, dy, dx)
    return dx


def pad_rows(src2d: torch.Tensor, kp: int, out: Optional[torch.Tensor] = None, gate: Optional[dict] = None) -> torch.Tensor:
    rows, k = src2d.shape
    if out is None:
        out = torch.empty((rows, kp), dtype=BF16, device=src2d.device)
    g = gate or {}
    load().pad_rows(src2d, out, rows, k, kp, g.get("flags"), g.get("epoch_word"), int(g.get("elem_off", 0)),
                    int(g.get("tile_elems", 0)))
    return out


def conv_out_size(h: int, k: int, stride: int, pad: int) -> int:
    return (h + 2 * pad - k) // stride + 1


def round_up(x: int, m: int) -> int:
    return (x + m - 1) // m * m


def im2col(x: torch.Tensor, kh: int, kw: int, stride: int, pad: int) -> Tuple[torch.Tensor, int, int, int]:
    n, h, w, c = x.shape
    ho, wo = conv_out_size(h, kh, stride, pad), conv_out_size(w, kw, stride, pad)
    kp = round_up(kh * kw * c, 8)
    col = torch.empty((n * ho * wo, kp), dtype=BF16, device=x.device)
    load().im2col(x, col, n, h, w, c, kh, kw, stride, pad, ho, wo, kp)
    return col, ho, wo, kp


def conv_igemm_fwd(x: torch.Tensor, w2d: torch.Tensor, kh: int, kw: int, stride: int, pad: int,
                   col_stats: Optional[torch.Tensor] = None) -> Optional[torch.Tensor]:
    n, h, w, c = x.shape
    cout = w2d.shape[0]
    if c % 64 or w2d.shape[1] != kh * kw * c or not x.is_contiguous() or not w2d.is_contiguous():
        return None
    ho, wo = conv_out_size(h, kh, stride, pad), conv_out_size(w, kw, stride, pad)
    M, K = n * ho * wo, kh * kw * c
    bn = pick_bn(M, cout)
    y = torch.empty((M, cout), dtype=BF16, device=x.device)
    ok = load().conv_igemm_fwd(x, w2d, y, kh, kw, stride, pad, ho, wo, pick_cluster_k(M, cout, K, bn), bn, col_stats)
    return y if ok else None


def conv_igemm_dgrad(dy: torch.Tensor, w2d: torch.Tensor, in_shape, kh: int, kw: int, pad: int) -> Optional[torch.Tensor]:
    n, h, w, c = in_shape
    cout = dy.shape[-1]
    if c % 64 or cout % 64 or w2d.shape[1] != kh * kw * c or not dy.is_contiguous() or not w2d.is_contiguous():
        return None
    M, K = n * h * w, kh * kw * cout
    bn = pick_bn(M, c)
    dx = torch.empty((n, h, w, c), dtype=BF16, device=dy.device)
    ok = load().conv_igemm_dgrad(dy, w2d, dx, kh, kw, pad, pick_cluster_k(M, c, K, bn), bn)
    return dx if ok else None


def conv_igemm_wgrad_(dy2d: torch.Tensor, x: torch.Tensor, dw2d: torch.Tensor, kh: int, kw: int, stride: int,
                      pad: int, sgd: Optional[dict] = None) -> bool:
    n, h, w, c = x.shape
    cout = dy2d.shape[1]
    if c % 64 or not x.is_contiguous() or not dy2d.is_contiguous() or not dw2d.is_contiguous():
        return False
    ho, wo = conv_out_size(h, kh, stride, pad), conv_out_size(w, kw, stride, pad)
    M, K = n * ho * wo, kh * kw * c
    bn = pick_bn(cout, K)
    split_k = pick_split_k(cout, K, M, bn)
    if sgd is not None and split_k != 1:
        return False
    sg = sgd or {}
    return bool(load().conv_igemm_wgrad(dy2d, x, dw2d, cout, kh, kw, stride, pad, ho, wo, split_k, bn,
                                        sg.get("theta"), sg.get("theta_bf16"), sg.get("momentum"), sg.get("hyper"),
                                        bool(sg.get("nesterov", False))))


def col2im(col: torch.Tensor, shape: Tuple[int, int, int, int], kh: int, kw: int, stride: int, pad: int,
           ho: int, wo: int) -> torch.Tensor:
    n, h, w, c = shape
    dx = torch.empty(shape, dtype=BF16, device=col.device)
    load().col2im(col, dx, n, h, w, c, kh, kw, stride, pad, ho, wo, col.shape[1])
    return dx


def maxpool(x: torch.Tensor, k: int, stride: int, pad: int) -> Tuple[torch.Tensor, torch.Tensor]:
    n, h, w, c = x.shape
    ho, wo = conv_out_size(h, k, stride, pad), conv_out_size(w, k, stride, pad)
    y = torch.empty((n, ho, wo, c), dtype=BF16, device=x.device)
    arg = torch.empty((n, ho, wo, c), dtype=torch.uint8 if (c % 8 == 0 and k * k <= 255) else torch.int32, device=x.device)
    load().maxpool(x, y, arg, n, h, w, c, k, stride, pad, ho, wo)
    return y, arg


def maxpool_bwd(dy: torch.Tensor, arg: torch.Tensor, in_shape, k: int, stride: int, pad: int,
                dy_b: Optional[torch.Tensor] = None) -> torch.Tensor:
    n, h, w, c = in_shape
    if dy_b is not None and arg.dtype != torch.uint8:
        dy, dy_b = add(dy, dy_b), None
    dx = torch.empty(in_shape, dtype=BF16, device=dy.device)
    load().maxpool_bwd(dy, dy_b, arg, dx, n, h, w, c, dy.shape[1], dy.shape[2], k, stride, pad)
    return dx


def bn_relu_maxpool(z: torch.Tensor, sums: torch.Tensor, gamma, beta, rmean, rvar, nbt, eps: float, momentum: float,
                    k: int, stride: int, pad: int):
    n, h, w, c = z.shape
    if c % 8 or k * k > 255:
        return None
    ho, wo = conv_out_size(h, k, stride, pad), conv_out_size(w, k, stride, pad)
    p = torch.empty((n, ho, wo, c), dtype=BF16, device=z.device)
    arg = torch.empty((n, ho, wo, c), dtype=torch.uint8, device=z.device)
    mean = torch.empty(c, dtype=torch.float32, device=z.device)
    rstd = torch.empty(c, dtype=torch.float32, device=z.device)
    if not load().bn_relu_maxpool(z, p, arg, sums, gamma, beta, rmean, rvar, mean, rstd, nbt, n, h, w, c, k, stride, pad,
                                  ho, wo, eps, momentum):
        return None
    return p, arg, mean, rstd


def bn_maxpool_bwd(z: torch.Tensor, p: torch.Tensor, arg: torch.Tensor, dy_a: torch.Tensor, dy_b: Optional[torch.Tensor],
                   gamma, mean: torch.Tensor, rstd: torch.Tensor, sums_b: torch.Tensor, dgamma, dbeta, k: int, stride: int,
                   pad: int) -> Optional[torch.Tensor]:
    n, h, w, c = z.shape
    dz = torch.empty_like(z)
    if not load().bn_maxpool_bwd(z, p, arg, dy_a, dy_b, dz, gamma, mean, rstd, sums_b, dgamma, dbeta, n, h, w, c, k, stride,
                                 pad, p.shape[1], p.shape[2]):
        return None
    return dz


def avgpool(x: torch.Tensor) -> torch.Tensor:
    n, h, w, c = x.shape
    y = torch.empty((n, c), dtype=BF16, device=x.device)
    load().avgpool(x, y, n, h * w, c)
    return y


def avgpool_bwd(dy: torch.Tensor, in_shape) -> torch.Tensor:
    n, h, w, c = in_shape
    dx = torch.empty(in_shape, dtype=BF16, device=dy.device)
    load().avgpool_bwd(dy, dx, n, h * w, c)
    return dx


def softmax_xent(logits: torch.Tensor, target: torch.Tensor, want_grad: bool = True,
                 grad_dtype: Optional[torch.dtype] = None, acc: Optional[torch.Tensor] = None):
    rows, c = logits.shape
    if acc is None:
        acc = torch.zeros(2, dtype=torch.float32, device=logits.device)
    dl = torch.empty_like(logits, dtype=grad_dtype or logits.dtype) if want_grad else None
    load().softmax_xent(logits, target, dl, acc, rows, c, logits.stride(0), 1.0 / rows)
    return acc, dl


def linear_xent_head(x: torch.Tensor, w_bf16: torch.Tensor, bias: Optional[torch.Tensor], target: torch.Tensor,
                     dw: torch.Tensor, db: Optional[torch.Tensor], acc: Optional[torch.Tensor] = None,
                     want_dx: bool = True, want_logits: bool = False):
    rows, K = x.shape
    if acc is None:
        acc = torch.zeros(2, dtype=torch.float32, device=x.device)
    dx = torch.empty((rows, K), dtype=BF16, device=x.device) if want_dx else None
    logits = torch.empty((rows, w_bf16.shape[0]), dtype=torch.float32, device=x.device) if want_logits else None
    ok = load().linear_xent_head(x, w_bf16, bias, target, dx, dw, db, acc, logits, 1.0 / rows)
    return (acc, dx, logits) if ok else None


def mse(pred: torch.Tensor, target: torch.Tensor, want_grad: bool = True):
    acc = torch.zeros(2, dtype=torch.float32, device=pred.device)
    dp = torch.empty_like(pred) if want_grad else None
    load().mse(pred.contiguous(), target.contiguous().float(), dp, acc, 1.0 / pred.numel())
    return acc, dp


def gemm_batched(a: torch.Tensor, b: torch.Tensor, out: torch.Tensor, *, M: int, N: int, K: int, lda: int, ldb: int,
                 ldd: int, a_mn: bool, b_mn: bool, n_outer: int, n_inner: int, a_strides, b_strides, d_strides,
                 alpha: float = 1.0, act: int = 0, accumulate: bool = False) -> torch.Tensor:
    load().gemm_batched(a, b, out, M, N, K, lda, ldb, ldd, a_mn, b_mn, act, alpha, n_outer, n_inner,
                        a_strides[0], a_strides[1], b_strides[0], b_strides[1], d_strides[0], d_strides[1], accumulate)
    return out


def embedding_bwd_(dy2d: torch.Tensor, idx: torch.Tensor, grad_table: torch.Tensor) -> None:
    load().embedding_bwd(dy2d, idx, grad_table)


def _sf_bytes(rows: int, k: int) -> int:
    return ((rows + 127) // 128) * ((k + 127) // 128) * 512


def quant_mx_rows(x2d: torch.Tensor):
    R, C = x2d.shape
    Cp = round_up(C, 16)
    q = torch.empty((R, Cp), dtype=torch.uint8, device=x2d.device)
    sf = torch.empty(_sf_bytes(R, C), dtype=torch.uint8, device=x2d.device)
    load().quant_mx_rows(x2d, q, sf, R, C, x2d.stride(0), Cp)
    return q, sf


def quant_mx_cols(x2d: torch.Tensor):
    R, C = x2d.shape
    Rp = round_up(R, 16)
    q = torch.zeros((C, Rp), dtype=torch.uint8, device=x2d.device) if Rp != R else \
        torch.empty((C, Rp), dtype=torch.uint8, device=x2d.device)
    sf = torch.empty(_sf_bytes(C, R), dtype=torch.uint8, device=x2d.device)
    load().quant_mx_cols(x2d, q, sf, R, C, x2d.stride(0), Rp)
    return q, sf


def dequant_mx(q: torch.Tensor, sf: torch.Tensor, cols: int) -> torch.Tensor:
# ... 19 lines not shown
```

baton_b200/ops/nn.py:

```python
from __future__ import annotations

import contextlib
import math
from typing import Optional

import torch
from torch import nn
from torch.nn import functional as TF

from . import functional as F
from ._ext import load

BF16 = torch.bfloat16


class _P:
    __slots__ = ("p",)

    def __init__(self, p):
        self.p = p


def _unwrap(v):
    return v.p if isinstance(v, _P) else v
# ... 106 lines not shown
BRANCH = _Branch()


class _SgdEpilogue:

    def __init__(self):
        self.arena = None

    @contextlib.contextmanager
    def open(self, arena, hyper, nesterov):
        self.arena, self.hyper, self.nesterov = arena, hyper, nesterov
        self.fused, self.nograd = [], []
        try:
            yield self
        finally:
            self.arena = None

    @property
    def active(self):
        return self.arena is not None

    def args(self, out2d):
        a = self.arena
        if a is None:
            return None
        return F.sgd_epilogue_args(a.theta, a.grad, out2d, self.hyper, a.momentum, a.theta_bf16, self.nesterov)

    def record(self, out2d, nograd_of=None):
        off = (out2d.data_ptr() - self.arena.grad.data_ptr()) // 4
        self.fused.append((off, out2d.shape[0], out2d.shape[1], out2d.stride(0)))
        if nograd_of is not None:
            self.nograd.append(((nograd_of.data_ptr() - self.arena.grad.data_ptr()) // 4, nograd_of.numel()))


SGD_EPI = _SgdEpilogue()


def _wgrad(fn, out2d, nograd_of=None):
    sgd = SGD_EPI.args(out2d)
    if sgd is not None and fn(sgd):
        SGD_EPI.record(out2d, nograd_of)
    else:
        fn(None)


def _grad_target(p: Optional[torch.Tensor]):
    if p is None or p.grad is None or p.grad.dtype != torch.float32:
        return None
    return p.grad


def _shadow(module: nn.Module, name: str, param: torch.Tensor, as2d: bool = True) -> torch.Tensor:
    sh = getattr(module, name + "_bf16", None)
    if sh is not None:
        return sh
    if param.dim() == 4:
        src = param.detach().permute(0, 2, 3, 1).contiguous()
        return F.cast(src.view(param.shape[0], -1), BF16)
    return F.cast(param.detach().contiguous(), BF16)


class _LinearFn(torch.autograd.Function):
    @staticmethod
    def forward(ctx, x, weight, bias, w_bf16, act, out_fp32, flags_cfg, anchor):
        weight, bias = _unwrap(weight), _unwrap(bias)
        x2 = x.reshape(-1, x.shape[-1])
        kw = {}
        if flags_cfg is not None:
            kw = dict(flags=flags_cfg["flags"], flag_epoch=flags_cfg.get("epoch", 0), flag_elem_off=flags_cfg["elem_off"],
                      flag_tile_elems=flags_cfg["tile_elems"], flag_bias_off=flags_cfg.get("bias_off", -1),
                      force_bn=128, flag_epoch_word=flags_cfg.get("epoch_word"))
        y = F.gemm(x2, w_bf16, bias=bias, act=act if act != 2 else 0,
                   out_dtype=torch.float32 if out_fp32 else BF16, **kw)
        ctx.act = act
        pre = None
        if act == 2:
            pre = y
            y = F.gelu(pre)
        ctx.save_for_backward(x2, w_bf16, y if act == 1 else pre)
        ctx.weight, ctx.bias = weight, bias
        ctx.x_shape = x.shape
        ctx.needs_dx = x.requires_grad
        return y.view(*x.shape[:-1], w_bf16.shape[0])

    @staticmethod
    def backward(ctx, dy):
        x2, w_bf16, aux = ctx.saved_tensors
        dy2 = dy.reshape(-1, dy.shape[-1])
        if dy2.dtype != BF16:
            dy2 = F.cast(dy2.contiguous(), BF16)
        elif not dy2.is_contiguous():
            dy2 = dy2.contiguous()
        if ctx.act == 1:
            dy2 = F.relu_bwd(aux, dy2)
        elif ctx.act == 2:
            dy2 = F.gelu_bwd(aux, dy2)
        weight, bias = ctx.weight, ctx.bias
        gw = gb = None
        tgt = _grad_target(weight)
        if tgt is not None:
            out2d = tgt.view(weight.shape[0], -1)
            WGRAD.run(lambda: F.gemm(dy2, x2, a_mn=True, b_mn=True, out=out2d, accumulate=True), dy2, x2)
        else:
            gw = F.gemm(dy2, x2, a_mn=True, b_mn=True, out_dtype=torch.float32, accumulate=True).view_as(weight)
        if bias is not None:
            tb = _grad_target(bias)
            if tb is not None:
                F.colsum_(dy2, tb, accumulate=True)
            else:
                gb = F.colsum_(dy2, torch.zeros_like(bias, dtype=torch.float32), accumulate=True)
        dx = None
        if ctx.needs_dx:
            dx = F.gemm(dy2, w_bf16, b_mn=True).view(ctx.x_shape)
        return dx, gw, gb, None, None, None, None, None


class Linear(nn.Module):

    def __init__(self, in_features: int, out_features: int, bias: bool = True, act: Optional[str] = None,
                 out_fp32: bool = False):
        super().__init__()
        self.in_features, self.out_features = in_features, out_features
        self.act = {None: 0, "relu": 1, "gelu": 2}[act]
        self.out_fp32 = out_fp32
        self.weight = nn.Parameter(torch.empty(out_features, in_features))
        self.bias = nn.Parameter(torch.empty(out_features)) if bias else None
        self.flags_cfg = None
        self.reset_parameters()

    def reset_parameters(self):
        nn.init.kaiming_uniform_(self.weight, a=math.sqrt(5))
        if self.bias is not None:
            bound = 1 / math.sqrt(self.in_features)
            nn.init.uniform_(self.bias, -bound, bound)

    def forward(self, x):
        if not x.is_cuda:
            y = TF.linear(x, self.weight.to(x.dtype), None if self.bias is None else self.bias.to(x.dtype))
            return TF.relu(y) if self.act == 1 else (TF.gelu(y, approximate="tanh") if self.act == 2 else y)
        if x.dtype != BF16:
            x = F.cast(x.contiguous(), BF16)
        if getattr(self, "fp8", False) and self.act == 0 and self.bias is None and not self.out_fp32:
            y = matmul_fp8(x.reshape(-1, x.shape[-1]), self, _shadow(self, "weight", self.weight), self.in_features)
            return y.view(*x.shape[:-1], self.out_features)
        cfg = self.flags_cfg
        if cfg is not None and cfg.get("epoch_word") is None:
            self.flags_cfg = None
        return _LinearFn.apply(x, _wrap(self.weight, x), _wrap(self.bias, x), _shadow(self, "weight", self.weight),
                               self.act, self.out_fp32, cfg, _anchor(x, self.weight))


class _ConvFn(torch.autograd.Function):
    @staticmethod
    def forward(ctx, x, weight, w_bf16, kh, kw, stride, pad, anchor, stats=None, gate=None):
        weight = _unwrap(weight)
        n, h, w, c = x.shape
        cout = w_bf16.shape[0]
        ctx.center = (h == 1 and w == 1 and kh == kw and kh % 2 == 1 and pad == kh // 2 and c % 8 == 0 and kh > 1)
        if ctx.center:
            col, ho, wo, kp = x.view(n, c), 1, 1, c
            wc = w_bf16.view(cout, kh * kw, c)[:, (kh // 2) * kw + kw // 2, :]
            y = F.gemm(col, wc, col_stats=stats)
        else:
            y = None
            ctx.igemm = False
            if kh == 1 and kw == 1 and stride == 1 and pad == 0 and c % 8 == 0:
                col, ho, wo, kp = x.view(n * h * w, c), h, w, c
            elif c % 64 == 0:
                ho, wo, kp = F.conv_out_size(h, kh, stride, pad), F.conv_out_size(w, kw, stride, pad), kh * kw * c
                y = F.conv_igemm_fwd(x, w_bf16, kh, kw, stride, pad, col_stats=stats)
                col, ctx.igemm = x, y is not None
            if y is None:
                if not (kh == 1 and kw == 1 and stride == 1 and pad == 0 and c % 8 == 0):
                    col, ho, wo, kp = F.im2col(x, kh, kw, stride, pad)
                gk = {}
                if gate is not None:
                    gk = dict(flags=gate["flags"], flag_epoch_word=gate["epoch_word"], flag_elem_off=gate["elem_off"],
                              flag_tile_elems=gate["tile_elems"], force_bn=F.pick_bn(col.shape[0], w_bf16.shape[0]))
                y = F.gemm(col, w_bf16, col_stats=stats, **gk)
        ctx.save_for_backward(col, w_bf16)
        ctx.weight = weight
        ctx.geom = (n, h, w, c, kh, kw, stride, pad, ho, wo, kp)
        ctx.needs_dx = x.requires_grad
        return y.view(n, ho, wo, cout)

    @staticmethod
    def backward(ctx, dy):
        col, w_bf16 = ctx.saved_tensors
        n, h, w, c, kh, kw, stride, pad, ho, wo, kp = ctx.geom
        cout = w_bf16.shape[0]
        dy2 = dy.reshape(n * ho * wo, cout)
        if not dy2.is_contiguous():
            dy2 = dy2.contiguous()
        weight = ctx.weight
        k_true = kh * kw * c
        gw = None
        tgt = _grad_target(weight)
        if ctx.center:
            tap = (kh // 2) * kw + kw // 2
            if tgt is None:
                gw = torch.zeros((cout, kh, kw, c), dtype=torch.float32, device=dy.device)
                g2d = gw.view(cout, kh * kw, c)[:, tap, :]
                gw = gw.permute(0, 3, 1, 2)
            else:
                full = tgt.permute(0, 2, 3, 1).reshape(cout, kh * kw, c)
                assert full.data_ptr() == tgt.data_ptr(), "conv weight grad must be channels_last in the arena"
                g2d = full[:, tap, :]
            if tgt is None:
                F.gemm(dy2, col, a_mn=True, b_mn=True, out=g2d, accumulate=True)
            tok = WGRAD.mark(dy2)
            dx = None
            if ctx.needs_dx:
                wc = w_bf16.view(cout, kh * kw, c)[:, tap, :]
                dx = F.gemm(dy2, wc, b_mn=True).view(n, 1, 1, c)
            if tgt is not None:
                WGRAD.run(lambda: _wgrad(lambda sgd: F.gemm(dy2, col, a_mn=True, b_mn=True, out=g2d, accumulate=True,
                                                            sgd=sgd) is not None, g2d, nograd_of=tgt),
                          dy2, col, after=None if SGD_EPI.active else tok)
            return dx, gw, None, None, None, None, None, None, None, None
        igemm = getattr(ctx, "igemm", False)
        tok = WGRAD.mark(dy2)
        dx = None
        if ctx.needs_dx:
            if stride == 1 and kh == kw and kh > 1 and kp == k_true and w_bf16.shape[1] == k_true:
                dx = F.conv_igemm_dgrad(dy2.view(n, ho, wo, cout), w_bf16, (n, h, w, c), kh, kw, pad)
            if dx is None:
                dcol = F.gemm(dy2, w_bf16, b_mn=True)
                if kh == 1 and kw == 1 and stride == 1 and pad == 0 and c % 8 == 0:
                    dx = dcol.view(n, h, w, c)
                else:
                    dx = F.col2im(dcol, (n, h, w, c), kh, kw, stride, pad, ho, wo)
        if tgt is not None:
            out2d = tgt.permute(0, 2, 3, 1).reshape(cout, k_true) if tgt.dim() == 4 else tgt.view(cout, k_true)
            assert out2d.data_ptr() == tgt.data_ptr(), "conv weight grad must be channels_last in the arena"
            if igemm:
                WGRAD.run(lambda: _wgrad(lambda sgd: F.conv_igemm_wgrad_(dy2, col, out2d, kh, kw, stride, pad, sgd=sgd),
                                         out2d),
                          dy2, col, after=None if SGD_EPI.active else tok)
            else:
                WGRAD.run(lambda: F.gemm(dy2, col, a_mn=True, b_mn=True, out=out2d, accumulate=True, n_valid=k_true),
                          dy2, col, after=tok)
        elif igemm:
            g2 = torch.zeros((cout, k_true), dtype=torch.float32, device=dy.device)
            F.conv_igemm_wgrad_(dy2, col, g2, kh, kw, stride, pad)
            gw = g2.view(cout, kh, kw, c).permute(0, 3, 1, 2)
        else:
            g2 = F.gemm(dy2, col, a_mn=True, b_mn=True, out_dtype=torch.float32, accumulate=True, n_valid=k_true)
            gw = g2.view(cout, kh, kw, c).permute(0, 3, 1, 2)
        return dx, gw, None, None, None, None, None, None, None, None


class Conv2d(nn.Module):

    def __init__(self, in_channels: int, out_channels: int, kernel_size: int, stride: int = 1, padding: int = 0):
        super().__init__()
        self.in_channels, self.out_channels = in_channels, out_channels
        self.kernel_size, self.stride, self.padding = kernel_size, stride, padding
        w = torch.empty(out_channels, in_channels, kernel_size, kernel_size)
        nn.init.kaiming_normal_(w, mode="fan_out", nonlinearity="relu")
        self.weight = nn.Parameter(w.contiguous(memory_format=torch.channels_last))
        self.k_true = kernel_size * kernel_size * in_channels
        self.kp = F.round_up(self.k_true, 8)
        self.flags_cfg = None

    def _w_bf16(self):
        sh = getattr(self, "weight_bf16", None)
        if sh is None:
            sh = _shadow(self, "weight", self.weight)
        sh = sh.view(self.out_channels, self.k_true)
        if self.kp != self.k_true:
            sh = F.pad_rows(sh, self.kp, gate=self.flags_cfg)
        return sh

    def forward(self, x):
        if not x.is_cuda:
            y = TF.conv2d(x.permute(0, 3, 1, 2), self.weight.to(x.dtype), None, self.stride, self.padding)
            return y.permute(0, 2, 3, 1)
        if getattr(self, "fp8", False):
            return conv2d_fp8(x, self)
        stats = self._fusable_stats(x)
        y = _ConvFn.apply(x, _wrap(self.weight, x), self._w_bf16(), self.kernel_size, self.kernel_size,
                          self.stride, self.padding, _anchor(x, self.weight), stats, self.flags_cfg)
        if stats is not None:
            y._bn_stats_ws = stats
        return y

    def _fusable_stats(self, x):
        ws = getattr(self, "bn_ws", None)
        if ws is None or not self.training or not torch.is_grad_enabled():
            return None
        n, h, w, c = x.shape
        k, s_, p_ = self.kernel_size, self.stride, self.padding
        ho, wo = (h + 2 * p_ - k) // s_ + 1, (w + 2 * p_ - k) // s_ + 1
        centre = h == 1 and w == 1 and k % 2 == 1 and p_ == k // 2 and c % 8 == 0 and k > 1
        kdim = c if (centre or (k == 1 and c % 8 == 0)) else F.round_up(k * k * c, 8)
        cout = self.weight.shape[0]
        return ws[: 2 * cout] if F.gemm_stats_fusable(n * ho * wo, cout, kdim) else None


class _BNFn(torch.autograd.Function):
    @staticmethod
    def forward(ctx, x, residual, gamma, beta, rmean, rvar, nbt, eps, momentum, relu, training, ws, anchor,
                stats_ready=False):
        gamma, beta = _unwrap(gamma), _unwrap(beta)
        C_ = load()
        c = x.shape[-1]
        rows = x.numel() // c
        y = torch.empty_like(x)
        if ws is None:
            ws = torch.zeros(4 * c, dtype=torch.float32, device=x.device)
        sums_f, sums_b = ws[: 2 * c], ws[2 * c:]
        save_mean = torch.empty(c, dtype=torch.float32, device=x.device)
        save_rstd = torch.empty(c, dtype=torch.float32, device=x.device)
        if training and not stats_ready:
            C_.bn_stats(x, sums_f, rows, c)
        C_.bn_apply(x, residual, y, sums_f, gamma, beta, rmean, rvar, save_mean, save_rstd, nbt, rows, c, eps,
                    momentum, relu, training)
        ctx.save_for_backward(x, y, save_mean, save_rstd)
        ctx.gamma, ctx.beta, ctx.sums_b = gamma, beta, sums_b
        ctx.relu, ctx.has_res, ctx.rows, ctx.c = relu, residual is not None, rows, c
        return y

    @staticmethod
    def backward(ctx, dy, dy_b=None):
        C_ = load()
        x, y, mean, rstd = ctx.saved_tensors
        if not dy.is_contiguous():
            dy = dy.contiguous()
        gamma, beta = ctx.gamma, ctx.beta
        dx = torch.empty_like(x)
        dres = torch.empty_like(x) if ctx.has_res else None
        tg, tb = _grad_target(gamma), _grad_target(beta)
        gg = gb = None
        if tg is None:
            gg = tg = torch.zeros(ctx.c, dtype=torch.float32, device=x.device)
        if tb is None:
            gb = tb = torch.zeros(ctx.c, dtype=torch.float32, device=x.device)
        if not C_.bn_bwd_cluster(x, y, dy, dy_b, dx, dres, gamma, mean, rstd, tg, tb, ctx.rows, ctx.c, ctx.relu, 16):
            if dy_b is not None:
                dy = F.add(dy, dy_b.contiguous())
            C_.bn_bwd_reduce(x, y, dy, mean, rstd, ctx.sums_b, ctx.rows, ctx.c, ctx.relu)
            C_.bn_bwd_apply(x, y, dy, dx, dres, gamma, mean, rstd, ctx.sums_b, tg, tb, ctx.rows, ctx.c, ctx.relu)
        if ctx.has_res and dres is None:
            dres = dy
        return dx, dres, gg, gb, None, None, None, None, None, None, None, None, None, None


class BatchNorm2d(nn.Module):

    def __init__(self, num_features: int, eps: float = 1e-5, momentum: float = 0.1, relu: bool = False):
        super().__init__()
        self.num_features, self.eps, self.momentum, self.relu = num_features, eps, momentum, relu
        self.weight = nn.Parameter(torch.ones(num_features))
        self.bias = nn.Parameter(torch.zeros(num_features))
        self.register_buffer("running_mean", torch.zeros(num_features))
        self.register_buffer("running_var", torch.ones(num_features))
        self.register_buffer("num_batches_tracked", torch.tensor(0, dtype=torch.long))
        self.workspace = None

    def forward(self, x, residual=None):
        if not x.is_cuda:
            xn = x.permute(0, 3, 1, 2)
            y = TF.batch_norm(xn, self.running_mean, self.running_var, self.weight, self.bias, self.training,
                              self.momentum, self.eps).permute(0, 2, 3, 1)
            if self.training:
                self.num_batches_tracked += 1
            if residual is not None:
                y = y + residual
            return TF.relu(y) if self.relu else y
        ws = self.workspace
        if ws is None:
            ws = torch.zeros(4 * self.num_features, dtype=torch.float32, device=x.device)
        fused = getattr(x, "_bn_stats_ws", None)
        ready = (fused is not None and self.workspace is not None and self.training
                 and fused.data_ptr() == self.workspace.data_ptr())
        return _BNFn.apply(x, residual, _wrap(self.weight, x), _wrap(self.bias, x), self.running_mean,
                           self.running_var, self.num_batches_tracked if self.training else None, self.eps,
                           self.momentum, self.relu, self.training, ws, _anchor(x, self.weight), ready)


class _MaxPoolFn(torch.autograd.Function):
    @staticmethod
    def forward(ctx, x, k, stride, pad):
        y, arg = F.maxpool(x, k, stride, pad)
        ctx.save_for_backward(arg)
        ctx.cfg = (tuple(x.shape), k, stride, pad)
        return y

    @staticmethod
    def backward(ctx, dy, dy_b=None):
        (arg,) = ctx.saved_tensors
        shape, k, stride, pad = ctx.cfg
        return F.maxpool_bwd(dy.contiguous(), arg, shape, k, stride, pad, dy_b=dy_b), None, None, None


class MaxPool2d(nn.Module):
    def __init__(self, kernel_size: int = 3, stride: int = 2, padding: int = 1):
        super().__init__()
        self.k, self.stride, self.pad = kernel_size, stride, padding

    def forward(self, x):
        if not x.is_cuda:
            return TF.max_pool2d(x.permute(0, 3, 1, 2), self.k, self.stride, self.pad).permute(0, 2, 3, 1)
        return _MaxPoolFn.apply(x, self.k, self.stride, self.pad)


class _AvgPoolFn(torch.autograd.Function):
    @staticmethod
    def forward(ctx, x):
        ctx.shape = tuple(x.shape)
        return F.avgpool(x)

    @staticmethod
    def backward(ctx, dy):
        return F.avgpool_bwd(dy.contiguous(), ctx.shape)


class GlobalAvgPool(nn.Module):

    def forward(self, x):
        if x.shape[1] == 1 and x.shape[2] == 1:
            return x.reshape(x.shape[0], x.shape[3])
        if not x.is_cuda:
            return x.mean(dim=(1, 2))
        return _AvgPoolFn.apply(x)


class _LNFn(torch.autograd.Function):
    @staticmethod
    def forward(ctx, x, residual, gamma, beta, eps, anchor):
        gamma, beta = _unwrap(gamma), _unwrap(beta)
        C_ = load()
        c = x.shape[-1]
        rows = x.numel() // c
        y = torch.empty_like(x)
        mean = torch.empty(rows, dtype=torch.float32, device=x.device)
        rstd = torch.empty(rows, dtype=torch.float32, device=x.device)
        C_.layernorm_fwd(x, residual, y, gamma, beta, mean, rstd, rows, c, eps)
        pre = x if residual is None else F.add(x, residual)
        ctx.save_for_backward(pre, mean, rstd)
        ctx.gamma, ctx.beta, ctx.has_res, ctx.rows, ctx.c = gamma, beta, residual is not None, rows, c
        return y

    @staticmethod
    def backward(ctx, dy):
        C_ = load()
        pre, mean, rstd = ctx.saved_tensors
        dy = dy.contiguous()
        dx = torch.empty_like(pre)
        tg, tb = _grad_target(ctx.gamma), _grad_target(ctx.beta)
        gg = gb = None
        if tg is None:
            gg = tg = torch.zeros(ctx.c, dtype=torch.float32, device=dy.device)
        if tb is None:
            gb = tb = torch.zeros(ctx.c, dtype=torch.float32, device=dy.device)
        C_.layernorm_bwd(pre, dy, dx, ctx.gamma, mean, rstd, tg, tb, ctx.rows, ctx.c)
        return dx, (dx if ctx.has_res else None), gg, gb, None, None


class LayerNorm(nn.Module):

    def __init__(self, normalized_shape: int, eps: float = 1e-12):
        super().__init__()
        self.c, self.eps = normalized_shape, eps
        self.weight = nn.Parameter(torch.ones(normalized_shape))
        self.bias = nn.Parameter(torch.zeros(normalized_shape))

    def forward(self, x, residual=None):
        if not x.is_cuda:
            if residual is not None:
                x = x + residual
            return TF.layer_norm(x, (self.c,), self.weight.to(x.dtype), self.bias.to(x.dtype), self.eps)
        return _LNFn.apply(x.contiguous(), None if residual is None else residual.contiguous(),
                           _wrap(self.weight, x), _wrap(self.bias, x), self.eps, _anchor(x, self.weight))


class _SoftmaxFn(torch.autograd.Function):
    @staticmethod
    def forward(ctx, x, scale):
        c = x.shape[-1]
        y = torch.empty_like(x)
        load().softmax_fwd(x, y, x.numel() // c, c, scale)
        ctx.save_for_backward(y)
        ctx.scale = scale
        return y

    @staticmethod
    def backward(ctx, dy):
        (y,) = ctx.saved_tensors
        c = y.shape[-1]
        dx = torch.empty_like(y)
        load().softmax_bwd(y, dy.contiguous(), dx, y.numel() // c, c, ctx.scale)
        return dx, None


def softmax(x: torch.Tensor, scale: float = 1.0) -> torch.Tensor:
    if not x.is_cuda:
        return torch.softmax(x * scale, dim=-1)
# ... 220 lines not shown
```

Baseline: 194,100.

## Fuse BatchNorm forward and backward into conv/GEMM epilogues via cluster reduction

Adds a BatchNorm epilogue to the wgmma GEMM and implicit-GEMM conv kernels. Forward mode computes per-channel statistics across the cluster through distributed shared memory, then normalizes, applies residual and ReLU, and updates running stats. Backward mode applies the BN gradient, ReLU mask and dgamma/dbeta inside the dgrad kernel. The aim is to remove the separate BN reduce/apply kernels and the extra activation round-trips through global memory. In exchange it adds cluster syncs, register pressure, more Python plumbing, and fallback paths when the epilogue is declined.

```diff
diff --git a/baton_b200/csrc/bindings.cpp b/baton_b200/csrc/bindings.cpp
--- a/baton_b200/csrc/bindings.cpp
+++ b/baton_b200/csrc/bindings.cpp
@@ -33,6 +33,43 @@
               "sgd epilogue: fp32 theta / momentum / hyper, bf16 shadow");
   return B200SgdEpilogue{theta->data_ptr<float>(), opt_ptr<void>(theta_bf16), opt_ptr<float>(mom),
                          hyper->data_ptr<float>(), nesterov ? 1 : 0};
+}
+
+inline B200BnEpilogue bn_epilogue(const std::vector<std::optional<at::Tensor>>& t, const std::vector<double>& s) {
+  TORCH_CHECK(t.size() == 15 && s.size() == 4, "bn epilogue: 15 tensors and 4 scalars");
+  const int mode = static_cast<int>(s[0]);
+  TORCH_CHECK(mode == 1 || mode == 2, "bn epilogue: mode 1 (forward) or 2 (backward)");
+  for (size_t i : {0, 1, 2, 3, 6, 7, 13, 14})
+    TORCH_CHECK(!t[i].has_value() || (t[i]->scalar_type() == at::kFloat && t[i]->is_contiguous()),
+                "bn epilogue: fp32 per-channel tensors");
+  for (size_t i : {4, 5, 9, 10, 11, 12})
+    TORCH_CHECK(!t[i].has_value() || (t[i]->scalar_type() == at::kBFloat16 && t[i]->is_contiguous()),
+                "bn epilogue: bf16 activations");
+  TORCH_CHECK(t[2].has_value() && t[3].has_value(), "bn epilogue: mean / rstd");
+  TORCH_CHECK(mode == 1 ? t[5].has_value() : (t[9].has_value() && (s[1] == 0 || t[10].has_value())),
+              "bn epilogue: forward needs y, backward needs x (and y for the ReLU mask)");
+  TORCH_CHECK(!t[8].has_value() || t[8]->scalar_type() == at::kLong, "bn epilogue: num_batches_tracked is int64");
+  B200BnEpilogue e{};
+  e.mode = mode;
+  e.relu = s[1] != 0 ? 1 : 0;
+  e.eps = static_cast<float>(s[2]);
+  e.momentum = static_cast<float>(s[3]);
+  e.gamma = opt_ptr<const float>(t[0]);
+  e.beta = opt_ptr<const float>(t[1]);
+  e.mean = opt_ptr<float>(t[2]);
+  e.rstd = opt_ptr<float>(t[3]);
+  e.residual = opt_ptr<const void>(t[4]);
+  e.y = opt_ptr<void>(t[5]);
+  e.running_mean = opt_ptr<float>(t[6]);
+  e.running_var = opt_ptr<float>(t[7]);
+  e.nbt = opt_ptr<long long>(t[8]);
+  e.x = opt_ptr<const void>(t[9]);
+  e.y_in = opt_ptr<const void>(t[10]);
+  e.dy_b = opt_ptr<const void>(t[11]);
+  e.dres = opt_ptr<void>(t[12]);
+  e.dgamma = opt_ptr<float>(t[13]);
+  e.dbeta = opt_ptr<float>(t[14]);
+  return e;
 }
 
 extern "C" {
@@ -83,9 +120,25 @@
                                 accumulate, static_cast<float>(alpha), opt_ptr<const uint32_t>(flags),
                                 static_cast<uint32_t>(flag_epoch), flag_elem_off, static_cast<int>(flag_tile_elems),
                                 flag_bias_off, static_cast<int>(force_bn), opt_ptr<float>(col_stats),
-                                opt_ptr<const uint32_t>(flag_epoch_word), sgd ? &*sgd : nullptr, cur_stream());
+                                opt_ptr<const uint32_t>(flag_epoch_word), sgd ? &*sgd : nullptr, nullptr, cur_stream());
   if (rc == B200_SGD_EPILOGUE_DECLINED) return false;
   check(rc, "gemm_bf16");
+  return true;
+}
+
+bool gemm_bn(const at::Tensor& a, const at::Tensor& b, at::Tensor d, int64_t M, int64_t N, int64_t K, int64_t lda,
+             int64_t ldb, int64_t ldd, bool b_mn, int64_t split_k, int64_t force_bn,
+             const std::vector<std::optional<at::Tensor>>& bn_t, const std::vector<double>& bn_s) {
+  CHECK_CUDA(a); CHECK_CUDA(b); CHECK_CUDA(d);
+  TORCH_CHECK(a.scalar_type() == at::kBFloat16 && b.scalar_type() == at::kBFloat16 && d.scalar_type() == at::kBFloat16,
+              "gemm_bn: bf16 operands and output");
+  const c10::cuda::CUDAGuard guard(a.device());
+  const B200BnEpilogue e = bn_epilogue(bn_t, bn_s);
+  const int rc = b200_gemm_bf16(cptr(a), cptr(b), ptr(d), nullptr, M, N, K, lda, ldb, ldd, 0, b_mn, 0, 0, split_k, 0, 1.0f,
+                                nullptr, 0, 0, 0, -1, static_cast<int>(force_bn), nullptr, nullptr, nullptr, &e,
+                                cur_stream());
+  if (rc == B200_BN_EPILOGUE_DECLINED || rc == -2) return false;
+  check(rc, "gemm_bn");
   return true;
 }
 
@@ -156,9 +209,26 @@
                                      static_cast<int>(kh), static_cast<int>(kw), static_cast<int>(stride),
                                      static_cast<int>(pad), static_cast<int>(ho), static_cast<int>(wo),
                                      static_cast<int>(cluster_k), static_cast<int>(force_bn), opt_ptr<float>(col_stats),
-                                     cur_stream());
+                                     nullptr, cur_stream());
   if (rc == -2) return false;
   check(rc, "conv_igemm_fwd");
+  return true;
+}
+bool conv_igemm_fwd_bn(const at::Tensor& x, const at::Tensor& w, at::Tensor y, int64_t kh, int64_t kw, int64_t stride,
+                       int64_t pad, int64_t ho, int64_t wo, int64_t cluster_k, int64_t force_bn,
+                       const std::vector<std::optional<at::Tensor>>& bn_t, const std::vector<double>& bn_s) {
+  CHECK_CUDA(x); CHECK_CUDA(w); CHECK_CUDA(y);
+  TORCH_CHECK(x.scalar_type() == at::kBFloat16 && w.scalar_type() == at::kBFloat16 && y.scalar_type() == at::kBFloat16 &&
+              x.dim() == 4 && x.is_contiguous() && w.is_contiguous() && y.is_contiguous());
+  const c10::cuda::CUDAGuard guard(x.device());
+  const B200BnEpilogue e = bn_epilogue(bn_t, bn_s);
+  const int rc = b200_conv_igemm_fwd(cptr(x), cptr(w), ptr(y), static_cast<int>(x.size(0)), static_cast<int>(x.size(1)),
+                                     static_cast<int>(x.size(2)), static_cast<int>(x.size(3)), static_cast<int>(w.size(0)),
+                                     static_cast<int>(kh), static_cast<int>(kw), static_cast<int>(stride),
+                                     static_cast<int>(pad), static_cast<int>(ho), static_cast<int>(wo),
+                                     static_cast<int>(cluster_k), static_cast<int>(force_bn), nullptr, &e, cur_stream());
+  if (rc == -2 || rc == B200_BN_EPILOGUE_DECLINED) return false;
+  check(rc, "conv_igemm_fwd_bn");
   return true;
 }
 bool conv_igemm_dgrad(const at::Tensor& dy, const at::Tensor& w, at::Tensor dx, int64_t kh, int64_t kw, int64_t pad,
@@ -171,9 +241,26 @@
                                        static_cast<int>(dx.size(2)), static_cast<int>(dx.size(3)), static_cast<int>(dy.size(3)),
                                        static_cast<int>(kh), static_cast<int>(kw), static_cast<int>(pad),
                                        static_cast<int>(dy.size(1)), static_cast<int>(dy.size(2)),
-                                       static_cast<int>(cluster_k), static_cast<int>(force_bn), cur_stream());
+                                       static_cast<int>(cluster_k), static_cast<int>(force_bn), nullptr, cur_stream());
   if (rc == -2) return false;
   check(rc, "conv_igemm_dgrad");
+  return true;
+}
+bool conv_igemm_dgrad_bn(const at::Tensor& dy, const at::Tensor& w, at::Tensor dx, int64_t kh, int64_t kw, int64_t pad,
+                         int64_t cluster_k, int64_t force_bn, const std::vector<std::optional<at::Tensor>>& bn_t,
+                         const std::vector<double>& bn_s) {
+  CHECK_CUDA(dy); CHECK_CUDA(w); CHECK_CUDA(dx);
+  TORCH_CHECK(dy.scalar_type() == at::kBFloat16 && w.scalar_type() == at::kBFloat16 && dx.scalar_type() == at::kBFloat16 &&
+              dy.dim() == 4 && dx.dim() == 4 && dy.is_contiguous() && w.is_contiguous() && dx.is_contiguous());
+  const c10::cuda::CUDAGuard guard(dy.device());
+  const B200BnEpilogue e = bn_epilogue(bn_t, bn_s);
+  const int rc = b200_conv_igemm_dgrad(cptr(dy), cptr(w), ptr(dx), static_cast<int>(dx.size(0)), static_cast<int>(dx.size(1)),
+                                       static_cast<int>(dx.size(2)), static_cast<int>(dx.size(3)), static_cast<int>(dy.size(3)),
+                                       static_cast<int>(kh), static_cast<int>(kw), static_cast<int>(pad),
+                                       static_cast<int>(dy.size(1)), static_cast<int>(dy.size(2)),
+                                       static_cast<int>(cluster_k), static_cast<int>(force_bn), &e, cur_stream());
+  if (rc == -2 || rc == B200_BN_EPILOGUE_DECLINED) return false;
+  check(rc, "conv_igemm_dgrad_bn");
   return true;
 }
 bool conv_igemm_wgrad(const at::Tensor& dy, const at::Tensor& x, at::Tensor dw, int64_t cout, int64_t kh, int64_t kw,
@@ -637,6 +724,9 @@
   m.doc() = "baton_b200 sm_90a kernels";
   m.attr("MAX_RANKS") = B200_MAX_RANKS;
   m.def("gemm", &gemm);
+  m.def("gemm_bn", &gemm_bn);
+  m.def("conv_igemm_fwd_bn", &conv_igemm_fwd_bn);
+  m.def("conv_igemm_dgrad_bn", &conv_igemm_dgrad_bn);
   m.def("trace_set", &trace_set);
   m.def("attention_fwd", &attention_fwd);
   m.def("attention_bwd", &attention_bwd);
diff --git a/baton_b200/csrc/gemm_wgmma.cu b/baton_b200/csrc/gemm_wgmma.cu
--- a/baton_b200/csrc/gemm_wgmma.cu
+++ b/baton_b200/csrc/gemm_wgmma.cu
@@ -49,6 +49,8 @@
   __nv_bfloat16* sgd_wb = nullptr;
   float* sgd_mom = nullptr;
   int sgd_nesterov = 0;
+  B200BnEpilogue bn = {};
+  int bn_m_tiles = 1;
 };
 
 __device__ __forceinline__ void wait_arrival_flags(const uint32_t* flags, long long e0, long long e1, int granule,
@@ -89,6 +91,8 @@
   asm volatile("barrier.cluster.arrive.release.aligned;" ::: "memory");
   asm volatile("barrier.cluster.wait.acquire.aligned;" ::: "memory");
 }
+__device__ __forceinline__ void cluster_arrive_only() { asm volatile("barrier.cluster.arrive.release.aligned;" ::: "memory"); }
+__device__ __forceinline__ void cluster_wait_only() { asm volatile("barrier.cluster.wait.acquire.aligned;" ::: "memory"); }
 __device__ __forceinline__ float4 ld_dsmem_f4(uint32_t local_smem_addr, uint32_t cta_rank) {
   uint32_t remote;
   asm volatile("mapa.shared::cluster.u32 %0, %1, %2;" : "=r"(remote) : "r"(local_smem_addr), "r"(cta_rank));
@@ -98,6 +102,25 @@
                : "r"(remote)
                : "memory");
   return v;
+}
+__device__ __forceinline__ float ld_dsmem_f1(uint32_t local_smem_addr, uint32_t cta_rank) {
+  uint32_t remote;
+  asm volatile("mapa.shared::cluster.u32 %0, %1, %2;" : "=r"(remote) : "r"(local_smem_addr), "r"(cta_rank));
+  float v;
+  asm volatile("ld.shared::cluster.f32 %0, [%1];" : "=f"(v) : "r"(remote) : "memory");
+  return v;
+}
+__device__ __forceinline__ void unpack8_bf16(const uint4 u, float (&f)[8]) {
+  const uint32_t w[4] = {u.x, u.y, u.z, u.w};
+#pragma unroll
+  for (int j = 0; j < 4; ++j) {
+    const float2 t = unpack_bf16x2(w[j]);
+    f[2 * j] = t.x;
+    f[2 * j + 1] = t.y;
+  }
+}
+__device__ __forceinline__ uint4 pack8_bf16(const float (&f)[8]) {
+  return make_uint4(pack_bf16x2(f[0], f[1]), pack_bf16x2(f[2], f[3]), pack_bf16x2(f[4], f[5]), pack_bf16x2(f[6], f[7]));
 }
 
 #define COLSUM_STEP(OFF, HALF)                                                  \
@@ -683,7 +706,292 @@
 }
 
 
-template <int BN, bool CLUSTER, int CONV = 0>
+constexpr int BN_EPI_SMEM_FLOATS_PER_COL = 20;
+template <int BN, int EPI>
+struct BnEpiOperands {
+  static constexpr int ITEMS = BM * (BN / 8) / CONSUMER_THREADS;
+  uint4 ax[ITEMS], ay[ITEMS], ab[ITEMS];
+  float mu[8], rs[8], gm8[8];
+  float pc[4];
+};
+template <int BN>
+struct BnEpiOperands<BN, 0> {};
+
+template <int BN, int EPI>
+__device__ __forceinline__ void bn_epi_load(const GemmParams& p, BnEpiOperands<BN, EPI>& op, int m0, int n0) {
+  constexpr int CG = BN / 8;
+  constexpr int ITEMS = BnEpiOperands<BN, EPI>::ITEMS;
+  const B200BnEpilogue& e = p.bn;
+  const int t = static_cast<int>(threadIdx.x) - 128;
+  const int rows_per = BM / p.cluster_k;
+  const int zb = static_cast<int>(blockIdx.z);
+  const int col0 = n0 + (t & (CG - 1)) * 8;
+  const bool col_ok = col0 < p.N;
+  const bool lead = blockIdx.y == 0 && zb == 0;
+  const auto bf = [](const void* base, size_t off) {
+    return *reinterpret_cast<const uint4*>(reinterpret_cast<const __nv_bfloat16*>(base) + off);
+  };
+#pragma unroll
+  for (int i = 0; i < ITEMS; ++i) {
+    const int item = t + i * CONSUMER_THREADS;
+    const int row = m0 + zb * rows_per + item / CG;
+    const size_t off = static_cast<size_t>(row) * p.ldd + col0;
+    op.ax[i] = op.ay[i] = op.ab[i] = make_uint4(0u, 0u, 0u, 0u);
+    if (item < rows_per * CG && row < p.M && col_ok) {
+      if (EPI == 1) {
+        if (e.residual != nullptr) op.ax[i] = bf(e.residual, off);
+      } else {
+        op.ax[i] = bf(e.x, off);
+        if (e.relu) op.ay[i] = bf(e.y_in, off);
+        if (e.dy_b != nullptr) op.ab[i] = bf(e.dy_b, off);
+      }
+    }
+  }
+  if (EPI == 2) {
+#pragma unroll
+    for (int j = 0; j < 8; ++j) {
+      op.mu[j] = col_ok ? e.mean[col0 + j] : 0.f;
+      op.rs[j] = col_ok ? e.rstd[col0 + j] : 0.f;
+      op.gm8[j] = (col_ok && e.gamma != nullptr) ? e.gamma[col0 + j] : 1.f;
+    }
+  }
+  op.pc[0] = op.pc[1] = op.pc[2] = op.pc[3] = 0.f;
+  const int col = n0 + t;
+  if (t < BN && col < p.N) {
+    if (EPI == 1) {
+      op.pc[0] = e.gamma != nullptr ? e.gamma[col] : 1.f;
+      op.pc[1] = e.beta != nullptr ? e.beta[col] : 0.f;
+      if (lead && e.running_mean != nullptr) {
+        op.pc[2] = e.running_mean[col];
+        op.pc[3] = e.running_var[col];
+      }
+    } else if (lead) {
+      op.pc[0] = e.dbeta != nullptr ? e.dbeta[col] : 0.f;
+      op.pc[1] = e.dgamma != nullptr ? e.dgamma[col] : 0.f;
+    }
+  }
+}
+
+template <int BN, int EPI>
+__device__ __forceinline__ void bn_cluster_epilogue(const GemmParams& p, const BnEpiOperands<BN, EPI>& op, float* cstat,
+                                                    int m0, int n0, int warp, uint8_t* smem) {
+  using L = SmemLayout<BN>;
+  constexpr int CG = BN / 8;
+  constexpr int ITEMS = BM * CG / CONSUMER_THREADS;
+  constexpr int DS_BATCH = 4, MAX_NR = 16;
+  const B200BnEpilogue& e = p.bn;
+  const int S = p.cluster_k, MT = p.bn_m_tiles, NR = MT * S;
+  const int yb = static_cast<int>(blockIdx.y), zb = static_cast<int>(blockIdx.z);
+  float* wpart = cstat;
+  float* cpart = cstat + 16 * BN;
+  float* coef = cpart + 2 * BN;
+  const bool worker = warp >= 4;
+  const int t = static_cast<int>(threadIdx.x) - 128;
+  const int rows_per = BM / S;
+  const int n_items = rows_per * CG;
+  const int cl = (t & (CG - 1)) * 8;
+  const int col0 = n0 + cl;
+  const bool col_ok = col0 < p.N;
+  const auto& ax = op.ax;
+  const auto& ay = op.ay;
+  const auto& ab = op.ab;
+  const auto& mu = op.mu;
+  const auto& rs = op.rs;
+  const auto& pc = op.pc;
+  size_t off[ITEMS];
+  bool ok[ITEMS];
+  const bool lead = yb == 0 && zb == 0;
+#pragma unroll
+  for (int i = 0; i < ITEMS; ++i) {
+    const int item = t + i * CONSUMER_THREADS;
+    const int row = m0 + zb * rows_per + item / CG;
+    ok[i] = worker && item < n_items && row < p.M && col_ok;
+    off[i] = static_cast<size_t>(row) * p.ldd + col0;
+  }
+  if (threadIdx.x == 128) TRACE_POINT();
+  cluster_sync_all();
+  if (threadIdx.x == 128) TRACE_POINT();
+  float g[ITEMS][8];
+  if (worker) {
+    float cs[8] = {0.f, 0.f, 0.f, 0.f, 0.f, 0.f, 0.f, 0.f}, cq[8] = {0.f, 0.f, 0.f, 0.f, 0.f, 0.f, 0.f, 0.f};
+#pragma unroll
+    for (int i = 0; i < ITEMS; ++i) {
+#pragma unroll
+      for (int j = 0; j < 8; ++j) g[i][j] = 0.f;
+      const int item = t + i * CONSUMER_THREADS;
+      if (item >= n_items) continue;
+      const int lrow = zb * rows_per + item / CG;
+      float v[8] = {0.f, 0.f, 0.f, 0.f, 0.f, 0.f, 0.f, 0.f};
+      if (S == 1) {
+        const float4* sp = reinterpret_cast<const float4*>(reinterpret_cast<const float*>(smem) + lrow * L::PART_PITCH + cl);
+        const float4 a = sp[0], b = sp[1];
+        v[0] += a.x; v[1] += a.y; v[2] += a.z; v[3] += a.w;
+        v[4] += b.x; v[5] += b.y; v[6] += b.z; v[7] += b.w;
+#pragma unroll
+        for (int j = 0; j < 8; ++j) g[i][j] = v[j];
+        continue;
+      }
+      const uint32_t laddr = smem_u32(smem) + static_cast<uint32_t>((lrow * L::PART_PITCH + cl) * 4);
+      for (int r0 = 0; r0 < S; r0 += DS_BATCH) {
+        float4 pa[DS_BATCH], pb[DS_BATCH];
+#pragma unroll
+        for (int r = 0; r < DS_BATCH; ++r) {
+          if (r0 + r < S) {
+            const uint32_t rank = static_cast<uint32_t>(yb + (r0 + r) * MT);
+            pa[r] = ld_dsmem_f4(laddr, rank);
+            pb[r] = ld_dsmem_f4(laddr + 16, rank);
+          }
+        }
+#pragma unroll
+        for (int r = 0; r < DS_BATCH; ++r) {
+          if (r0 + r < S) {
+            v[0] += pa[r].x; v[1] += pa[r].y; v[2] += pa[r].z; v[3] += pa[r].w;
+            v[4] += pb[r].x; v[5] += pb[r].y; v[6] += pb[r].z; v[7] += pb[r].w;
+          }
+        }
+      }
+#pragma unroll
+      for (int j = 0; j < 8; ++j) g[i][j] = v[j];
+    }
+#pragma unroll
+    for (int i = 0; i < ITEMS; ++i) {
+      if (!ok[i]) {
+#pragma unroll
+        for (int j = 0; j < 8; ++j) g[i][j] = 0.f;
+        continue;
+      }
+#pragma unroll
+      for (int j = 0; j < 8; ++j) g[i][j] = __bfloat162float(__float2bfloat16_rn(g[i][j]));
+      if (EPI == 1) {
+        *reinterpret_cast<uint4*>(reinterpret_cast<__nv_bfloat16*>(p.D) + off[i]) = pack8_bf16(g[i]);
+#pragma unroll
+        for (int j = 0; j < 8; ++j) {
+          cs[j] += g[i][j];
+          cq[j] = fmaf(g[i][j], g[i][j], cq[j]);
+        }
+      } else {
+        float xf[8], yv[8], d[8];
+        unpack8_bf16(ax[i], xf);
+        unpack8_bf16(ay[i], yv);
+        unpack8_bf16(ab[i], d);
+#pragma unroll
+        for (int j = 0; j < 8; ++j) {
+          if (e.dy_b != nullptr) g[i][j] += d[j];
+          if (e.relu && !(yv[j] > 0.f)) g[i][j] = 0.f;
+          cs[j] += g[i][j];
+          cq[j] = fmaf(g[i][j], (xf[j] - mu[j]) * rs[j], cq[j]);
+        }
+        if (e.dres != nullptr) *reinterpret_cast<uint4*>(reinterpret_cast<__nv_bfloat16*>(e.dres) + off[i]) = pack8_bf16(g[i]);
+      }
+    }
+#pragma unroll
+    for (int j = 0; j < 8; ++j) {
+#pragma unroll
+      for (int o = CG; o < 32; o <<= 1) {
+        cs[j] += __shfl_xor_sync(0xffffffffu, cs[j], o);
+        cq[j] += __shfl_xor_sync(0xffffffffu, cq[j], o);
+      }
+    }
+    const int wq = t >> 5, ln = t & 31;
+    if (ln < CG) {
+#pragma unroll
+      for (int j = 0; j < 8; ++j) {
+        wpart[wq * 2 * BN + ln * 8 + j] = cs[j];
+        wpart[wq * 2 * BN + BN + ln * 8 + j] = cq[j];
+      }
+    }
+    named_bar_sync(1, CONSUMER_THREADS);
+    for (int i = t; i < 2 * BN; i += CONSUMER_THREADS) {
+      float s = 0.f;
+#pragma unroll
+      for (int w = 0; w < CONSUMER_WARPS; ++w) s += wpart[w * 2 * BN + i];
+      cpart[i] = s;
+    }
+    if (t == 0) TRACE_POINT();
+  }
+  cluster_sync_all();
+  if (threadIdx.x == 128) TRACE_POINT();
+  if (worker) {
+    float* tot = wpart;
+    for (int i = t; i < 2 * BN; i += CONSUMER_THREADS) {
+      const uint32_t a = smem_u32(cpart + i);
+      float l[MAX_NR];
+#pragma unroll
+      for (int r = 0; r < MAX_NR; ++r)
+        if (r < NR) l[r] = ld_dsmem_f1(a, static_cast<uint32_t>(r));
+      float s = 0.f;
+#pragma unroll
+      for (int r = 0; r < MAX_NR; ++r)
+        if (r < NR) s += l[r];
+      tot[i] = s;
+    }
+    named_bar_sync(1, CONSUMER_THREADS);
+    const float inv_rows = 1.f / static_cast<float>(p.M);
+    const int col = n0 + t;
+    if (t < BN && col < p.N) {
+      const float s = tot[t], q = tot[BN + t];
+      if (EPI == 1) {
+        const float mean = s * inv_rows;
+        const float var = fmaxf(q * inv_rows - mean * mean, 0.f);
+        const float rstd = rsqrtf(var + e.eps);
+        coef[t] = pc[0] * rstd;
+        coef[BN + t] = pc[1] - mean * pc[0] * rstd;
+        if (lead) {
+          e.mean[col] = mean;
+          e.rstd[col] = rstd;
+          if (e.running_mean != nullptr) {
+            const float rows = static_cast<float>(p.M);
+            const float unbiased = p.M > 1 ? var * rows / static_cast<float>(p.M - 1) : var;
+            e.running_mean[col] = (1.f - e.momentum) * pc[2] + e.momentum * mean;
+            e.running_var[col] = (1.f - e.momentum) * pc[3] + e.momentum * unbiased;
+          }
+        }
+      } else {
+        coef[t] = s * inv_rows;
+        coef[BN + t] = q * inv_rows;
+        if (lead) {
+          if (e.dbeta != nullptr) e.dbeta[col] = pc[0] + s;
+          if (e.dgamma != nullptr) e.dgamma[col] = pc[1] + q;
+        }
+      }
+    }
+    if (EPI == 1 && lead && blockIdx.x == 0 && t == 0 && e.nbt != nullptr) *e.nbt += 1;
+    named_bar_sync(1, CONSUMER_THREADS);
+    if (t == 0) TRACE_POINT();
+  }
+  cluster_arrive_only();
+  if (worker && col_ok) {
+    float ka[8], kb[8], gr[8];
+#pragma unroll
+    for (int j = 0; j < 8; ++j) {
+      ka[j] = coef[cl + j];
+      kb[j] = coef[BN + cl + j];
+      if (EPI == 2) gr[j] = op.gm8[j] * rs[j];
+    }
+#pragma unroll
+    for (int i = 0; i < ITEMS; ++i) {
+      if (!ok[i]) continue;
+      float o[8], a[8];
+      unpack8_bf16(ax[i], a);
+      if (EPI == 1) {
+#pragma unroll
+        for (int j = 0; j < 8; ++j) {
+          o[j] = fmaf(g[i][j], ka[j], kb[j]) + a[j];
+          if (e.relu) o[j] = fmaxf(o[j], 0.f);
+        }
+        *reinterpret_cast<uint4*>(reinterpret_cast<__nv_bfloat16*>(e.y) + off[i]) = pack8_bf16(o);
+      } else {
+#pragma unroll
+        for (int j = 0; j < 8; ++j) o[j] = gr[j] * (g[i][j] - ka[j] - (a[j] - mu[j]) * rs[j] * kb[j]);
+        *reinterpret_cast<uint4*>(reinterpret_cast<__nv_bfloat16*>(p.D) + off[i]) = pack8_bf16(o);
+      }
+    }
+  }
+  if (threadIdx.x == 128) TRACE_POINT();
+  cluster_wait_only();
+}
+
+template <int BN, bool CLUSTER, int CONV = 0, int EPI = 0>
 __global__ void __launch_bounds__(GEMM_THREADS, 1)
 gemm_bf16_splitk_kernel(const __grid_constant__ CUtensorMap tmA, const __grid_constant__ CUtensorMap tmB,
                         const GemmParams p) {
@@ -718,6 +1026,7 @@
   }
   __syncthreads();
   griddep_wait();
+  BnEpiOperands<BN, EPI> bn_op;
 
   if (warp == 0) {
     if (elect_one()) {
@@ -773,6 +1082,7 @@
     }
   } else if (warp >= 4) {
     const int ew = warp - 4;
+    if constexpr (EPI != 0) bn_epi_load<BN, EPI>(p, bn_op, m0, n0);
     float acc[BN / 2];
     int s = 0;
     uint32_t ph = 0;
@@ -803,7 +1113,9 @@
     }
   }
 
-  if constexpr (CLUSTER) {
+  if constexpr (EPI != 0) {
+    bn_cluster_epilogue<BN, EPI>(p, bn_op, cstat, m0, n0, warp, smem);
+  } else if constexpr (CLUSTER) {
     const int S = p.cluster_k;
     cluster_sync_all();
     if (warp >= 4 && warp < 8) {
@@ -1011,6 +1323,65 @@
   return static_cast<int>(cudaGetLastError());
 }
 
+template <int CONV, int EPI>
+static int launch_bn_epi(const CUtensorMap& ta, const CUtensorMap& tb, GemmParams& p, int bn, dim3 grid,
+                         cudaStream_t stream) {
+  using L = SmemLayout<64>;
+  constexpr int max_smem = 8 * L::STAGE_BYTES + 2 * MAX_STAGES * 8 + BN_EPI_SMEM_FLOATS_PER_COL * 64 * 4 + 1024;
+  const int m_tiles = static_cast<int>(grid.y);
+  const int csize = m_tiles * p.cluster_k;
+  if (bn != 64 || p.N % 8 != 0 || p.ldd % 8 != 0 || (reinterpret_cast<uintptr_t>(p.D) & 15) || csize > 16)
+    return B200_BN_EPILOGUE_DECLINED;
+  static int np16 = -1;
+  if (np16 < 0) {
+    cudaError_t e = cudaFuncSetAttribute(gemm_bf16_splitk_kernel<64, true, CONV, EPI>,
+                                         cudaFuncAttributeMaxDynamicSharedMemorySize, max_smem);
+    if (e != cudaSuccess) return static_cast<int>(e);
+    np16 = cudaFuncSetAttribute(gemm_bf16_splitk_kernel<64, true, CONV, EPI>,
+                                cudaFuncAttributeNonPortableClusterSizeAllowed, 1) == cudaSuccess;
+    cudaGetLastError();
+  }
+  if (csize > 8 && !np16) return B200_BN_EPILOGUE_DECLINED;
+  p.bn_m_tiles = m_tiles;
+  int ring = p.stages * L::STAGE_BYTES;
+  if (L::PART_BYTES > ring) ring = L::PART_BYTES;
+  int smem = ring + 2 * MAX_STAGES * 8 + BN_EPI_SMEM_FLOATS_PER_COL * 64 * 4 + 1024;
+  const int floor_smem = (227 * 1024) / 3 + 1024;
+  if (smem < floor_smem) smem = floor_smem;
+  cudaLaunchConfig_t cfg = {};
+  cfg.gridDim = grid;
+  cfg.blockDim = dim3(GEMM_THREADS);
+  cfg.dynamicSmemBytes = smem;
+  cfg.stream = stream;
+  cudaLaunchAttribute attr[2];
+  int na = 0;
+  if (pdl_enabled()) {
+    attr[na].id = cudaLaunchAttributeProgrammaticStreamSerialization;
+    attr[na].val.programmaticStreamSerializationAllowed = 1;
+    ++na;
+  }
+  attr[na].id = cudaLaunchAttributeClusterDimension;
+  attr[na].val.clusterDim.x = 1;
+  attr[na].val.clusterDim.y = static_cast<unsigned>(m_tiles);
+  attr[na].val.clusterDim.z = static_cast<unsigned>(p.cluster_k);
+  ++na;
+  cfg.attrs = attr;
+  cfg.numAttrs = na;
+  cudaError_t le = cudaLaunchKernelEx(&cfg, gemm_bf16_splitk_kernel<64, true, CONV, EPI>, ta, tb, p);
+  if (le != cudaSuccess) return static_cast<int>(le);
+  return static_cast<int>(cudaGetLastError());
+}
+template <int CONV>
+static int launch_bn(const CUtensorMap& ta, const CUtensorMap& tb, GemmParams& p, const B200BnEpilogue& bn_epi, int bn,
+                     dim3 grid, cudaStream_t stream) {
+  p.bn = bn_epi;
+  if constexpr (CONV != 3)
+    if (bn_epi.mode == 1) return launch_bn_epi<CONV, 1>(ta, tb, p, bn, grid, stream);
+  if constexpr (CONV != 1)
+    if (bn_epi.mode == 2) return launch_bn_epi<CONV, 2>(ta, tb, p, bn, grid, stream);
+  return B200_BN_EPILOGUE_DECLINED;
+}
+
 }
 
 extern "C" int b200_encode_map2_bf16(void* map, const void* base, long long rows, long long cols, long long ld,
@@ -1029,9 +1400,12 @@
                               int split_k, int accumulate, float alpha, const uint32_t* tile_flags,
                               uint32_t flag_epoch, long long flag_elem_off, int flag_tile_elems,
                               long long flag_bias_off, int force_bn, float* col_stats, const uint32_t* flag_epoch_ptr,
-                              const B200SgdEpilogue* sgd, cudaStream_t stream) {
+                              const B200SgdEpilogue* sgd, const B200BnEpilogue* bn_epi, cudaStream_t stream) {
   using namespace b200;
   if (M <= 0 || N <= 0 || K <= 0) return 0;
+  if (bn_epi != nullptr && (M > 4 * BM || out_fp32 || accumulate || a_mn || split_k > 1 || bias != nullptr || act != 0 ||
+                            alpha != 1.0f || col_stats != nullptr || tile_flags != nullptr || sgd != nullptr))
+    return B200_BN_EPILOGUE_DECLINED;
   if (sgd != nullptr && (!accumulate || !out_fp32 || !a_mn || !b_mn || bias != nullptr || act != 0 || alpha != 1.0f ||
                          col_stats != nullptr || tile_flags != nullptr))
     return B200_SGD_EPILOGUE_DECLINED;
@@ -1086,6 +1460,7 @@
     if (split_k != 1 || cluster_k != 1 || persistent) return B200_SGD_EPILOGUE_DECLINED;
     set_sgd_epilogue(p, *sgd);
   }
+  if (bn_epi != nullptr) return launch_bn<0>(ta, tb, p, *bn_epi, bn, grid, stream);
   if (cluster_k > 1) {
     if (bn == 128) return launch_cfg<128>(ta, tb, p, grid, stream);
     return launch_cfg<64>(ta, tb, p, grid, stream);
@@ -1151,11 +1526,12 @@
 
 extern "C" int b200_conv_igemm_fwd(const void* x, const void* w, void* y, int N, int H, int W, int Cin, int Cout, int KH,
                                    int KW, int stride, int pad, int Ho, int Wo, int cluster_k, int force_bn,
-                                   float* col_stats, cudaStream_t stream) {
+                                   float* col_stats, const B200BnEpilogue* bn_epi, cudaStream_t stream) {
   using namespace b200;
   const long long M = static_cast<long long>(N) * Ho * Wo;
   const int K = KH * KW * Cin;
   if (M <= 0 || Cout <= 0) return 0;
+  if (bn_epi != nullptr && (M > 4 * BM || col_stats != nullptr)) return B200_BN_EPILOGUE_DECLINED;
   if (Cin % 64 != 0 || Cout % 8 != 0 || M > (1ll << 30) || (reinterpret_cast<uintptr_t>(x) & 15) ||
       (reinterpret_cast<uintptr_t>(w) & 15) || (reinterpret_cast<uintptr_t>(y) & 15))
     return -2;
@@ -1181,6 +1557,7 @@
   p.conv_ho = Ho; p.conv_wo = Wo; p.conv_stride = stride; p.conv_pad = pad; p.conv_kw = KW; p.conv_cin = Cin;
   p.conv_taps = KH * KW; p.conv_ncol = Cin;
   dim3 grid((Cout + bn - 1) / bn, static_cast<unsigned>((M + BM - 1) / BM), cluster_k);
+  if (bn_epi != nullptr) return launch_bn<1>(ta, tb, p, *bn_epi, bn, grid, stream);
   if (cluster_k > 1) {
     if (bn == 128) return launch_cfg<128, 1>(ta, tb, p, grid, stream);
     return launch_cfg<64, 1>(ta, tb, p, grid, stream);
@@ -1192,11 +1569,12 @@
 
 extern "C" int b200_conv_igemm_dgrad(const void* dy, const void* w, void* dx, int N, int H, int W, int Cin, int Cout,
                                      int KH, int KW, int pad, int Ho, int Wo, int cluster_k, int force_bn,
-                                     cudaStream_t stream) {
+                                     const B200BnEpilogue* bn_epi, cudaStream_t stream) {
   using namespace b200;
   const long long M = static_cast<long long>(N) * H * W;
   const int K = KH * KW * Cout;
   if (M <= 0 || Cin <= 0) return 0;
+  if (bn_epi != nullptr && M > 4 * BM) return B200_BN_EPILOGUE_DECLINED;
   const int padp = KH - 1 - pad, padq = KW - 1 - pad;
   if (Cout % 64 != 0 || Cin % 64 != 0 || M > (1ll << 30) || padp < 0 || padq < 0 || padp != padq ||
       Ho + 2 * padp - (KH - 1) != H || Wo + 2 * padq - (KW - 1) != W || (reinterpret_cast<uintptr_t>(dy) & 15) ||
@@ -1225,6 +1603,7 @@
   p.conv_ho = H; p.conv_wo = W; p.conv_stride = 1; p.conv_pad = padp; p.conv_kw = KW; p.conv_cin = Cout;
   p.conv_taps = KH * KW; p.conv_ncol = Cin;
   dim3 grid((Cin + bn - 1) / bn, static_cast<unsigned>((M + BM - 1) / BM), cluster_k);
+  if (bn_epi != nullptr) return launch_bn<3>(ta, tb, p, *bn_epi, bn, grid, stream);
   if (cluster_k > 1) {
     if (bn == 128) return launch_cfg<128, 3>(ta, tb, p, grid, stream);
     return launch_cfg<64, 3>(ta, tb, p, grid, stream);
diff --git a/baton_b200/csrc/launch.h b/baton_b200/csrc/launch.h
--- a/baton_b200/csrc/launch.h
+++ b/baton_b200/csrc/launch.h
@@ -15,11 +15,33 @@
 };
 #define B200_SGD_EPILOGUE_DECLINED (-6)
 
+struct B200BnEpilogue {
+  int mode;
+  int relu;
+  float eps, momentum;
+  const float* gamma;
+  const float* beta;
+  float* mean;
+  float* rstd;
+  const void* residual;
+  void* y;
+  float* running_mean;
+  float* running_var;
+  long long* nbt;
+  const void* x;
+  const void* y_in;
+  const void* dy_b;
+  void* dres;
+  float* dgamma;
+  float* dbeta;
+};
+#define B200_BN_EPILOGUE_DECLINED (-7)
+
 int b200_gemm_bf16(const void* a, const void* b, void* d, const float* bias, int M, int N, int K, long long lda,
                    long long ldb, long long ldd, int a_mn, int b_mn, int out_fp32, int act, int split_k, int accumulate,
                    float alpha, const uint32_t* tile_flags, uint32_t flag_epoch, long long flag_elem_off, int flag_tile_elems,
                    long long flag_bias_off, int force_bn, float* col_stats, const uint32_t* flag_epoch_ptr,
-                   const B200SgdEpilogue* sgd, cudaStream_t stream);
+                   const B200SgdEpilogue* sgd, const B200BnEpilogue* bn, cudaStream_t stream);
 int b200_gemm_bf16_batched(const void* a, const void* b, void* d, int M, int N, int K, long long lda, long long ldb,
                            long long ldd, int a_mn, int b_mn, int out_fp32, int act, float alpha, int n_outer,
                            int n_inner, long long a_outer, long long a_inner, long long b_outer, long long b_inner,
@@ -30,9 +52,10 @@
                        float scale, cudaStream_t stream);
 int b200_conv_igemm_fwd(const void* x, const void* w, void* y, int N, int H, int W, int Cin, int Cout, int KH, int KW,
                         int stride, int pad, int Ho, int Wo, int cluster_k, int force_bn, float* col_stats,
-                        cudaStream_t stream);
+                        const B200BnEpilogue* bn, cudaStream_t stream);
 int b200_conv_igemm_dgrad(const void* dy, const void* w, void* dx, int N, int H, int W, int Cin, int Cout, int KH, int KW,
-                          int pad, int Ho, int Wo, int cluster_k, int force_bn, cudaStream_t stream);
+                          int pad, int Ho, int Wo, int cluster_k, int force_bn, const B200BnEpilogue* bn,
+                          cudaStream_t stream);
 int b200_conv_igemm_wgrad(const void* dy, const void* x, float* dw, int N, int H, int W, int Cin, int Cout, int KH, int KW,
                           int stride, int pad, int Ho, int Wo, int split_k, int force_bn, const B200SgdEpilogue* sgd,
                           cudaStream_t stream);
diff --git a/baton_b200/models/resnet.py b/baton_b200/models/resnet.py
--- a/baton_b200/models/resnet.py
+++ b/baton_b200/models/resnet.py
@@ -12,21 +12,31 @@
 def _conv_bn_fwd(conv: "bnn.Conv2d", bn: "bnn.BatchNorm2d", x, residual=None, after_conv=None):
     cc, cb = bnn.Ctx(), bnn.Ctx()
     stats = conv._fusable_stats(x)
+    n, h, w, _ = x.shape
+    k, s, p = conv.kernel_size, conv.stride, conv.padding
+    shape = (n, bnn.F.conv_out_size(h, k, s, p), bnn.F.conv_out_size(w, k, s, p), conv.out_channels)
+    epi = bnn.bn_fwd_epilogue(bn, residual, shape, x.device)
     z = bnn._ConvFn.forward(cc, x, conv.weight, conv._w_bf16(), conv.kernel_size, conv.kernel_size, conv.stride,
-                            conv.padding, None, stats, conv.flags_cfg)
+                            conv.padding, None, stats, conv.flags_cfg, epi)
     if after_conv is not None:
         after_conv()
+    if cc.bn_fused:
+        return bnn._BNFn.fused(cb, z, residual, bn, epi), (cc, cb)
     y = bnn._BNFn.forward(cb, z, residual, bn.weight, bn.bias, bn.running_mean, bn.running_var, bn.num_batches_tracked,
                           bn.eps, bn.momentum, bn.relu, True, bn.workspace, None, stats is not None)
     return y, (cc, cb)
 
 
-def _conv_bn_bwd(ctxs, dy_a, dy_b=None, needs_dx=True):
+def _conv_bn_bwd(ctxs, dy_a, dy_b=None, needs_dx=True, below=None):
     cc, cb = ctxs
     cc.needs_dx = needs_dx
-    out = bnn._BNFn.backward(cb, dy_a, dy_b)
-    dz, dres = out[0], out[1]
-    dx = bnn._ConvFn.backward(cc, dz)[0]
+    if isinstance(dy_a, bnn.BNGrad):
+        dz, dres = dy_a.dz, dy_a.dres
+    else:
+        out = bnn._BNFn.backward(cb, dy_a, dy_b)
+        dz, dres = out[0], out[1]
+    epi = bnn.bn_bwd_epilogue(*below) if below is not None and needs_dx else None
+    dx = bnn._ConvFn.backward(cc, dz, epi)[0]
     return dx, dres
 
 
@@ -182,15 +192,19 @@
         tape.append((ctxs, ds_ctx))
         return out
 
-    def _block_bwd(self, entry, pieces):
+    def _block_bwd(self, entry, pieces, below=None):
         ctxs, ds_ctx = entry
-        d, dres = _conv_bn_bwd(ctxs[-1], pieces[0], pieces[1] if len(pieces) > 1 else None)
+        d, dres = _conv_bn_bwd(ctxs[-1], pieces[0], pieces[1] if len(pieces) > 1 else None, below=(ctxs[-2][1], None))
         dx_ds = None
         if ds_ctx is not None:
             with bnn.BRANCH.fork(dres):
                 dx_ds, _ = _conv_bn_bwd(ds_ctx, dres)
-        for c in reversed(ctxs[:-1]):
-            d, _ = _conv_bn_bwd(c, d)
+        for i in range(len(ctxs) - 2, -1, -1):
+            if i > 0:
+                blw = (ctxs[i - 1][1], None)
+            else:
+                blw = (below, dres) if below is not None and ds_ctx is None else None
+            d, _ = _conv_bn_bwd(ctxs[i], d, below=blw)
         if ds_ctx is not None:
             bnn.BRANCH.join()
             return [d, dx_ds]
@@ -236,7 +250,7 @@
         d = d.reshape(h.shape) if ca is None else bnn._AvgPoolFn.backward(ca, d)
         pieces = [d]
         for bi in range(len(tape) - 1, -1, -1):
-            pieces = self._block_bwd(tape[bi], pieces)
+            pieces = self._block_bwd(tape[bi], pieces, tape[bi - 1][0][-1][1] if bi > 0 else None)
         if fused_stem is not None:
             _stem_bwd(fused_stem, self.bn1, self.maxpool, pieces[0], pieces[1] if len(pieces) > 1 else None)
         else:
diff --git a/baton_b200/ops/functional.py b/baton_b200/ops/functional.py
--- a/baton_b200/ops/functional.py
+++ b/baton_b200/ops/functional.py
@@ -102,6 +102,38 @@
     return out
 
 
+BN_EPILOGUE_MAX_ROWS = 512
+_BN_EPILOGUE_MAX_CLUSTER = 16
+
+
+def bn_epilogue_fusable(M: int, N: int, K: int) -> bool:
+    bn = pick_bn(M, N)
+    if M > BN_EPILOGUE_MAX_ROWS or bn != 64 or N % 8 or K % 8:
+        return False
+    return ((M + 127) // 128) * pick_cluster_k(M, N, K, bn) <= _BN_EPILOGUE_MAX_CLUSTER
+
+
+_BN_KEYS = ("gamma", "beta", "mean", "rstd", "residual", "y", "running_mean", "running_var", "nbt", "x", "y_in", "dy_b",
+            "dres", "dgamma", "dbeta")
+
+
+def _bn_args(bn: dict):
+    return ([bn.get(k) for k in _BN_KEYS],
+            [float(bn["mode"]), float(bool(bn.get("relu"))), float(bn.get("eps", 0.0)), float(bn.get("momentum", 0.0))])
+
+
+def gemm_bn(a: torch.Tensor, b: torch.Tensor, bn: dict, b_mn: bool = False) -> Optional[torch.Tensor]:
+    M, K = a.shape
+    N = b.shape[1] if b_mn else b.shape[0]
+    if not (_tma_ok(a) and _tma_ok(b)) or not bn_epilogue_fusable(M, N, K):
+        return None
+    bnw = pick_bn(M, N)
+    k = pick_cluster_k(M, N, K, bnw)
+    out = torch.empty((M, N), dtype=BF16, device=a.device)
+    ok = load().gemm_bn(a, b, out, M, N, K, _pitch(a), _pitch(b), N, b_mn, -k if k > 1 else 1, bnw, *_bn_args(bn))
+    return out if ok else None
+
+
 def gemm_stats_fusable(M: int, N: int, K: int) -> bool:
     return K % 8 == 0
 
@@ -261,6 +293,23 @@
     return y if ok else None
 
 
+def conv_igemm_fwd_bn(x: torch.Tensor, w2d: torch.Tensor, kh: int, kw: int, stride: int, pad: int,
+                      bn: dict) -> Optional[torch.Tensor]:
+    n, h, w, c = x.shape
+    cout = w2d.shape[0]
+    if c % 64 or w2d.shape[1] != kh * kw * c or not x.is_contiguous() or not w2d.is_contiguous():
+        return None
+    ho, wo = conv_out_size(h, kh, stride, pad), conv_out_size(w, kw, stride, pad)
+    M, K = n * ho * wo, kh * kw * c
+    if not bn_epilogue_fusable(M, cout, K):
+        return None
+    bnw = pick_bn(M, cout)
+    z = torch.empty((M, cout), dtype=BF16, device=x.device)
+    ok = load().conv_igemm_fwd_bn(x, w2d, z, kh, kw, stride, pad, ho, wo, pick_cluster_k(M, cout, K, bnw), bnw,
+                                  *_bn_args(bn))
+    return z if ok else None
+
+
 def conv_igemm_dgrad(dy: torch.Tensor, w2d: torch.Tensor, in_shape, kh: int, kw: int, pad: int) -> Optional[torch.Tensor]:
     n, h, w, c = in_shape
     cout = dy.shape[-1]
@@ -271,6 +320,21 @@
     dx = torch.empty((n, h, w, c), dtype=BF16, device=dy.device)
     ok = load().conv_igemm_dgrad(dy, w2d, dx, kh, kw, pad, pick_cluster_k(M, c, K, bn), bn)
     return dx if ok else None
+
+
+def conv_igemm_dgrad_bn(dy: torch.Tensor, w2d: torch.Tensor, in_shape, kh: int, kw: int, pad: int,
+                        bn: dict) -> Optional[torch.Tensor]:
+    n, h, w, c = in_shape
+    cout = dy.shape[-1]
+    if c % 64 or cout % 64 or w2d.shape[1] != kh * kw * c or not dy.is_contiguous() or not w2d.is_contiguous():
+        return None
+    M, K = n * h * w, kh * kw * cout
+    if not bn_epilogue_fusable(M, c, K):
+        return None
+    bnw = pick_bn(M, c)
+    dz = torch.empty((n, h, w, c), dtype=BF16, device=dy.device)
+    ok = load().conv_igemm_dgrad_bn(dy, w2d, dz, kh, kw, pad, pick_cluster_k(M, c, K, bnw), bnw, *_bn_args(bn))
+    return dz if ok else None
 
 
 def conv_igemm_wgrad_(dy2d: torch.Tensor, x: torch.Tensor, dw2d: torch.Tensor, kh: int, kw: int, stride: int,
diff --git a/baton_b200/ops/nn.py b/baton_b200/ops/nn.py
--- a/baton_b200/ops/nn.py
+++ b/baton_b200/ops/nn.py
@@ -282,23 +282,34 @@
 
 class _ConvFn(torch.autograd.Function):
     @staticmethod
-    def forward(ctx, x, weight, w_bf16, kh, kw, stride, pad, anchor, stats=None, gate=None):
+    def forward(ctx, x, weight, w_bf16, kh, kw, stride, pad, anchor, stats=None, gate=None, bn_epi=None):
         weight = _unwrap(weight)
         n, h, w, c = x.shape
         cout = w_bf16.shape[0]
+        ctx.bn_fused = False
         ctx.center = (h == 1 and w == 1 and kh == kw and kh % 2 == 1 and pad == kh // 2 and c % 8 == 0 and kh > 1)
         if ctx.center:
             col, ho, wo, kp = x.view(n, c), 1, 1, c
             wc = w_bf16.view(cout, kh * kw, c)[:, (kh // 2) * kw + kw // 2, :]
-            y = F.gemm(col, wc, col_stats=stats)
+            y = F.gemm_bn(col, wc, bn_epi) if bn_epi is not None else None
+            ctx.bn_fused = y is not None
+            if y is None:
+                y = F.gemm(col, wc, col_stats=stats)
         else:
             y = None
             ctx.igemm = False
             if kh == 1 and kw == 1 and stride == 1 and pad == 0 and c % 8 == 0:
                 col, ho, wo, kp = x.view(n * h * w, c), h, w, c
+                if bn_epi is not None and gate is None:
+                    y = F.gemm_bn(col, w_bf16, bn_epi)
+                    ctx.bn_fused = y is not None
             elif c % 64 == 0:
                 ho, wo, kp = F.conv_out_size(h, kh, stride, pad), F.conv_out_size(w, kw, stride, pad), kh * kw * c
-                y = F.conv_igemm_fwd(x, w_bf16, kh, kw, stride, pad, col_stats=stats)
+                if bn_epi is not None:
+                    y = F.conv_igemm_fwd_bn(x, w_bf16, kh, kw, stride, pad, bn_epi)
+                    ctx.bn_fused = y is not None
+                if y is None:
+                    y = F.conv_igemm_fwd(x, w_bf16, kh, kw, stride, pad, col_stats=stats)
                 col, ctx.igemm = x, y is not None
             if y is None:
                 if not (kh == 1 and kw == 1 and stride == 1 and pad == 0 and c % 8 == 0):
@@ -315,7 +326,7 @@
         return y.view(n, ho, wo, cout)
 
     @staticmethod
-    def backward(ctx, dy):
+    def backward(ctx, dy, bn_below=None):
         col, w_bf16 = ctx.saved_tensors
         n, h, w, c, kh, kw, stride, pad, ho, wo, kp = ctx.geom
         cout = w_bf16.shape[0]
@@ -342,7 +353,11 @@
             dx = None
             if ctx.needs_dx:
                 wc = w_bf16.view(cout, kh * kw, c)[:, tap, :]
-                dx = F.gemm(dy2, wc, b_mn=True).view(n, 1, 1, c)
+                dz = F.gemm_bn(dy2, wc, bn_below, b_mn=True) if bn_below is not None else None
+                if dz is not None:
+                    dx = BNGrad(dz.view(n, 1, 1, c), bn_below["dres"])
+                else:
+                    dx = F.gemm(dy2, wc, b_mn=True).view(n, 1, 1, c)
             if tgt is not None:
                 WGRAD.run(lambda: _wgrad(lambda sgd: F.gemm(dy2, col, a_mn=True, b_mn=True, out=g2d, accumulate=True,
                                                             sgd=sgd) is not None, g2d, nograd_of=tgt),
@@ -352,11 +367,21 @@
         tok = WGRAD.mark(dy2)
         dx = None
         if ctx.needs_dx:
+            one_by_one = kh == 1 and kw == 1 and stride == 1 and pad == 0 and c % 8 == 0
             if stride == 1 and kh == kw and kh > 1 and kp == k_true and w_bf16.shape[1] == k_true:
-                dx = F.conv_igemm_dgrad(dy2.view(n, ho, wo, cout), w_bf16, (n, h, w, c), kh, kw, pad)
+                if bn_below is not None:
+                    dz = F.conv_igemm_dgrad_bn(dy2.view(n, ho, wo, cout), w_bf16, (n, h, w, c), kh, kw, pad, bn_below)
+                    if dz is not None:
+                        dx = BNGrad(dz, bn_below["dres"])
+                if dx is None:
+                    dx = F.conv_igemm_dgrad(dy2.view(n, ho, wo, cout), w_bf16, (n, h, w, c), kh, kw, pad)
+            elif one_by_one and bn_below is not None:
+                dz = F.gemm_bn(dy2, w_bf16, bn_below, b_mn=True)
+                if dz is not None:
+                    dx = BNGrad(dz.view(n, h, w, c), bn_below["dres"])
             if dx is None:
                 dcol = F.gemm(dy2, w_bf16, b_mn=True)
-                if kh == 1 and kw == 1 and stride == 1 and pad == 0 and c % 8 == 0:
+                if one_by_one:
                     dx = dcol.view(n, h, w, c)
                 else:
                     dx = F.col2im(dcol, (n, h, w, c), kh, kw, stride, pad, ho, wo)
@@ -474,6 +499,44 @@
         if ctx.has_res and dres is None:
             dres = dy
         return dx, dres, gg, gb, None, None, None, None, None, None, None, None, None, None
+
+    @staticmethod
+    def fused(ctx, z, residual, bn, epi):
+        c = z.shape[-1]
+        y = epi["y"]
+        ctx.save_for_backward(z, y, epi["mean"], epi["rstd"])
+        ctx.gamma, ctx.beta, ctx.sums_b = epi["gamma"], epi["beta"], bn.workspace[2 * c:]
+        ctx.relu, ctx.has_res, ctx.rows, ctx.c = bn.relu, residual is not None, z.numel() // c, c
+        return y
+
+
+class BNGrad:
+    __slots__ = ("dz", "dres")
+
+    def __init__(self, dz, dres):
+        self.dz, self.dres = dz, dres
+
+
+def bn_fwd_epilogue(bn: "BatchNorm2d", residual, shape, device) -> Optional[dict]:
+    if not bn.training or bn.workspace is None:
+        return None
+    c = bn.num_features
+    return {"mode": 1, "relu": bn.relu, "eps": bn.eps, "momentum": bn.momentum, "gamma": _unwrap(bn.weight),
+            "beta": _unwrap(bn.bias), "mean": torch.empty(c, dtype=torch.float32, device=device),
+            "rstd": torch.empty(c, dtype=torch.float32, device=device),
+            "residual": residual.contiguous() if residual is not None else None,
+            "y": torch.empty(shape, dtype=BF16, device=device), "running_mean": bn.running_mean,
+            "running_var": bn.running_var, "nbt": bn.num_batches_tracked}
+
+
+def bn_bwd_epilogue(ctx, dy_b=None) -> Optional[dict]:
+    x, y, mean, rstd = ctx.saved_tensors
+    tg, tb = _grad_target(ctx.gamma), _grad_target(ctx.beta)
+    if tg is None or tb is None:
+        return None
+    return {"mode": 2, "relu": ctx.relu, "gamma": ctx.gamma, "mean": mean, "rstd": rstd, "x": x, "y_in": y,
+            "dy_b": dy_b.contiguous() if dy_b is not None else None,
+            "dres": torch.empty_like(x) if ctx.has_res else None, "dgamma": tg, "dbeta": tb}
 
 
 class BatchNorm2d(nn.Module):
```

Result: faster. 196,500, median of 6 (+1.2%).
